# mandt-lab/shallow-ntc

Measured on AMD Instinct MI355X. Metric: decode Mpixels/s + (bpp, PSNR) on Kodak, two_layer_syn, higher is better.
Workload: dtype f32

## Files before the change

include/sntc.h:

```cpp
#ifndef SNTC_H_
#define SNTC_H_

#include <stddef.h>
#include <stdint.h>

#ifdef __cplusplus
extern "C" {
#endif

#define SNTC_VERSION 100

enum {
  SNTC_OK = 0,
  SNTC_ERR_BAD_SHAPE = 1,
  SNTC_ERR_UNSUPPORTED = 2,
  SNTC_ERR_HIP = 3,
  SNTC_ERR_NONFINITE = 4,
  SNTC_ERR_NO_DEVICE = 5
};

const char* sntc_last_error(void);
int sntc_version(void);
int sntc_device_count(void);
int sntc_device_arch(int device, char* buf, size_t buflen);

enum {
  SNTC_CONV2D = 0,
  SNTC_CONV2D_TRANSPOSE = 1,
  SNTC_SIGNAL_DOWN = 2,
  SNTC_SIGNAL_UP = 3
};
enum {
  SNTC_ACT_NONE = 0, SNTC_ACT_RELU = 1, SNTC_ACT_LEAKY_RELU = 2 , SNTC_ACT_SIGMOID = 3
};
enum {
  SNTC_PRO_NONE = 0, SNTC_PRO_ABS = 1, SNTC_PRO_SQUARE = 2
};
enum {
  SNTC_EPI_STORE = 0,
  SNTC_EPI_ADD = 1,
  SNTC_EPI_GATE = 2,
  SNTC_EPI_RES_DIV = 3,
  SNTC_EPI_RES_MUL = 4,
  SNTC_EPI_RES_DIV_SQRT = 5,
  SNTC_EPI_RES_MUL_SQRT = 6,
  SNTC_EPI_MASK_RELU = 7,
  SNTC_EPI_MASK_LEAKY = 8
};

typedef struct sntc_conv_desc {
  int32_t kind;
  int32_t kh, kw;
  int32_t stride;
  int32_t cin, cout;
  int32_t act;
  int32_t prologue;
  int32_t epilogue;
  int32_t reserved[7];
} sntc_conv_desc;

typedef struct sntc_conv_plan sntc_conv_plan;

int sntc_conv_plan_create(const sntc_conv_desc* desc, const float* weight, const float* bias,
                          void* stream, sntc_conv_plan** plan);
void sntc_conv_plan_destroy(sntc_conv_plan* plan);
int sntc_conv_plan_update(sntc_conv_plan* plan, const float* weight, const float* bias, void* stream);
typedef struct sntc_plan_group sntc_plan_group;
int sntc_plan_group_create(sntc_conv_plan* const* plans, const float* const* weights, const float* const* biases, int count,
                           void* stream, sntc_plan_group** group);
int sntc_plan_group_update(const sntc_plan_group* group, void* stream);
void sntc_plan_group_destroy(sntc_plan_group* group);
int sntc_conv_out_shape(const sntc_conv_plan* plan, int h, int w, int* ho, int* wo);
int64_t sntc_conv_flops(const sntc_conv_plan* plan, int n, int h, int w);
int sntc_conv_forward(const sntc_conv_plan* plan, const float* x, int n, int h, int w, float* y,
                      const float* res, const float* aux, void* workspace, size_t workspace_bytes, void* stream);
int64_t sntc_conv_workspace_bytes(const sntc_conv_plan* plan, int n, int h, int w);
int sntc_conv_fusable(const sntc_conv_plan* first, const sntc_conv_plan* second);
int64_t sntc_conv_fused_workspace_bytes(const sntc_conv_plan* first, int n, int h, int w);
int sntc_conv_forward_fused(const sntc_conv_plan* first, const sntc_conv_plan* second, const float* x, int n, int h, int w, float* y,
                            const float* res, const float* aux, void* workspace, size_t workspace_bytes, void* stream);
typedef struct sntc_resblock_plan sntc_resblock_plan;
int sntc_resblock_supported(int c);
int sntc_resblock_plan_create(int c, const float* w0, const float* b0, const float* w1, const float* b1,
                              const float* w2, const float* b2, int precision, void* stream, sntc_resblock_plan** plan);
int sntc_resblock_plan_update(sntc_resblock_plan* plan, const float* w0, const float* b0, const float* w1, const float* b1,
                              const float* w2, const float* b2, void* stream);
void sntc_resblock_plan_destroy(sntc_resblock_plan* plan);
int64_t sntc_resblock_flops(const sntc_resblock_plan* plan, int n, int h, int w);
int sntc_resblock_forward(const sntc_resblock_plan* plan, const float* x, int n, int h, int w, float* y, void* stream);
int sntc_resblock_plan_set_workgroups(sntc_resblock_plan* plan, int max_workgroups);
typedef struct sntc_rgbconv_plan sntc_rgbconv_plan;
int sntc_rgbconv_supported(int kind, int k, int stride, int cin, int cout, int act);
int sntc_rgbconv_plan_create(int kind, int k, int stride, int cin, int cout, const float* w, const float* bias, int act,
                             void* stream, sntc_rgbconv_plan** plan);
int sntc_rgbconv_plan_update(sntc_rgbconv_plan* plan, const float* w, const float* bias, void* stream);
void sntc_rgbconv_plan_destroy(sntc_rgbconv_plan* plan);
int64_t sntc_rgbconv_flops(const sntc_rgbconv_plan* plan, int n, int h, int w);
int sntc_rgbconv_forward(const sntc_rgbconv_plan* plan, const float* x, int n, int h, int w, float* y, void* stream);
int sntc_rgbconv_plan_set_workgroups(sntc_rgbconv_plan* plan, int max_workgroups);
typedef struct sntc_upsmall_plan sntc_upsmall_plan;
int sntc_upsmall_supported(int kind, int k, int stride, int cin, int cout);
int sntc_upsmall_plan_create(int kind, int k, int stride, int cin, int cout, const float* w, const float* bias, void* stream,
                             sntc_upsmall_plan** plan);
int sntc_upsmall_plan_update(sntc_upsmall_plan* plan, const float* w, const float* bias, void* stream);
void sntc_upsmall_plan_destroy(sntc_upsmall_plan* plan);
int64_t sntc_upsmall_flops(const sntc_upsmall_plan* plan, int n, int h, int w);
int sntc_upsmall_forward(const sntc_upsmall_plan* plan, const float* x, int n, int h, int w, float* y, void* stream);
typedef struct sntc_syn_plan sntc_syn_plan;
typedef struct sntc_syn_batch {
  const float* y_hat;
  float* hidden;
  int32_t n, h, w;
  int32_t reserved;
} sntc_syn_batch;
int sntc_syn_supported(int k, int stride, int cin, int ch, int has_res);
int sntc_syn_plan_create(int k, int stride, int cin, int ch, int has_res, int act_kind, const float* w1, const float* b1,
                         const float* beta, const float* gamma, void* stream, sntc_syn_plan** plan);
int sntc_syn_plan_update(sntc_syn_plan* plan, const float* w1, const float* b1, const float* beta, const float* gamma, void* stream);
void sntc_syn_plan_destroy(sntc_syn_plan* plan);
int64_t sntc_syn_flops(const sntc_syn_plan* plan, int64_t latent_pixels);
int64_t sntc_syn_workspace_bytes(const sntc_syn_plan* plan);
int sntc_syn_forward(const sntc_syn_plan* plan, const sntc_syn_batch* batches, int nbatches, void* workspace, size_t workspace_bytes,
                     void* stream);
int sntc_syn_plan_set_workgroups(sntc_syn_plan* plan, int max_workgroups);
int sntc_syn_plan_units(const sntc_syn_plan* plan, int* out, int capacity);
int sntc_syn_describe(int k, int stride, int cin, int ch, int has_res, int* out, int capacity);
int sntc_syn_selfcheck(int k, int stride, int cin, int ch, int has_res, int h, int w, unsigned seed, double* max_err);
int sntc_conv_plan_set_tile(sntc_conv_plan* plan, int variant);
int sntc_conv_plan_set_schedule(sntc_conv_plan* plan, int flags);
int sntc_split3(const float* x, int64_t npix, int c, void* out, void* stream);
int sntc_dequant_split3(const int32_t* symbols, const float* hyper, int64_t npix, int c, void* out, float* y_hat,
                        void* stream);
int sntc_conv_status(int* flags, void* stream);
int sntc_conv_status_inject(int flags, void* stream);
int sntc_conv_set_stream_k(int enabled);
int sntc_conv_get_stream_k(void);
int sntc_conv_launch_info(const sntc_conv_plan* plan, int n, int h, int w, int* variant, int* nblocks);
int sntc_conv_launch_order(const sntc_conv_plan* plan, int n, int h, int w, int* column_major);
int64_t sntc_conv_tune_workspace_bytes(const sntc_conv_plan* plan, int n, int h, int w);
int sntc_conv_plan_tune(sntc_conv_plan* plan, const float* x, int n, int h, int w, float* y, const float* res,
                        const float* aux, void* workspace, size_t workspace_bytes, int reps, int* variant, int* stream_k,
                        void* stream);
int sntc_conv_plan_candidates(const sntc_conv_plan* plan, int n, int h, int w, int* variants, int* stream_k, int capacity);
int sntc_conv_plan_set_choice(sntc_conv_plan* plan, int n, int h, int w, int variant, int stream_k);
int sntc_conv_plan_clear_tuning(sntc_conv_plan* plan);
int sntc_conv_plan_drop_choice(sntc_conv_plan* plan, int n, int h, int w, int ncols);

int sntc_conv_columns_supported(const sntc_conv_plan* plan, int ncols);
int sntc_conv_forward_columns(const sntc_conv_plan* plan, const float* x, int n, int h, int w, float* y, const float* res,
                              const float* aux, void* workspace, size_t workspace_bytes, void* stream, int ncols);
int64_t sntc_conv_columns_flops(const sntc_conv_plan* plan, int n, int h, int w, int ncols);
int64_t sntc_conv_columns_workspace_bytes(const sntc_conv_plan* plan, int n, int h, int w, int ncols);
int sntc_conv_columns_launch_info(const sntc_conv_plan* plan, int n, int h, int w, int ncols, int* variant, int* nblocks,
                                  int* column_major);
int64_t sntc_conv_columns_tune_workspace_bytes(const sntc_conv_plan* plan, int n, int h, int w, int ncols);
int sntc_conv_columns_tune(sntc_conv_plan* plan, const float* x, int n, int h, int w, int ncols, float* y, void* workspace,
                           size_t workspace_bytes, int reps, int* variant, int* stream_k, void* stream);
int sntc_conv_columns_candidates(const sntc_conv_plan* plan, int n, int h, int w, int ncols, int* variants, int* stream_k,
                                 int capacity);
int sntc_conv_columns_set_choice(sntc_conv_plan* plan, int n, int h, int w, int ncols, int variant, int stream_k);

int sntc_gdn_small(const float* x, int64_t npix, int c, const float* beta, const float* gamma,
                   int inverse, int alpha, int epsilon_is_half, float* y, void* stream);

int sntc_two_layer_tail(const float* t, int n, int hh, int wh, int ch, int has_res, int act_kind,
                        const float* beta, const float* gamma, const float* w2, const float* b2,
                        int k2, int s2, int cout, float* x_hat, void* stream);
int sntc_two_layer_tail_pixels(const float* t, int n, int hh, int wh, int ch, int has_res, int act_kind,
                               const float* beta, const float* gamma, const float* w2, const float* b2, int k2, int s2,
                               int cout, int h, int w, const float* ref, uint8_t* pixels, uint64_t* sse, void* stream);

int sntc_pad_reflect(const float* x, int n, int h, int w, int c, int hp, int wp, float* y, void* stream);
int sntc_pad_zero(const float* x, int n, int h, int w, int c, int top, int left, int hp, int wp, float* y, void* stream);
int sntc_crop(const float* x, int n, int hp, int wp, int c, int h, int w, float* y, void* stream);
int sntc_depth_to_space(const float* x, int n, int h, int w, int c, int block, float* y, void* stream);
int sntc_concat_channels(const float* a, int ca, const float* b, int cb, int64_t npix, float* y, void* stream);
int sntc_pixels_sse(const float* x, const float* x_hat, int n, int h, int w, int c, int hs, int ws,
                    uint8_t* pixels_out, unsigned long long* sse_out, void* stream);
int sntc_block_sse(const float* x, const uint8_t* pixels, int n, int h, int w, int c, int block, uint32_t* out, void* stream);
int sntc_float_sse(const float* x, const float* x_hat, int n, int h, int w, int c, int hs, int ws,
                   double* sse_out, void* stream);

typedef struct sntc_prior sntc_prior;
int sntc_prior_create(int channels, int nlayers, const int* widths, const float* matrices,
                      const float* biases, const float* factors, void* stream, sntc_prior** prior);
void sntc_prior_destroy(sntc_prior* prior);

int sntc_entropy_factorized(const sntc_prior* prior, const float* z, int n, int64_t hw, float* z_hat,
                            double* bits, int values_only, void* stream);

int sntc_entropy_scale_normal(const float* y, const float* hyper, int n, int64_t hw, int c,
                              float* y_hat, int32_t* symbols, double* bits, int values_only,
                              void* stream);
int sntc_dequant_scale_normal(const int32_t* symbols, const float* hyper, int n, int64_t hw, int c,
                              float* y_hat, void* stream);
int sntc_dequant_mean(const int32_t* symbols, const float* mu, int n, int64_t hw, int c, int mu_stride, float* y_hat,
                      void* stream);

int64_t sntc_rans_cap_words(int64_t elems_per_image, int segments);
int sntc_rans_encode(const int32_t* values, const uint16_t* table_ids, int nimages, int64_t elems_per_image, int segments,
                     int lanes, const uint16_t* cdf, const uint32_t* meta, int ntables, int total_entries, int64_t cap_words,
                     uint16_t* scratch, int32_t* len_words, void* stream);
int sntc_rans_compact(const uint16_t* scratch, int64_t cap_words, const int32_t* len_words, const int64_t* offsets,
                      int nstreams, uint16_t* payload, void* stream);
int64_t sntc_rans_lut_budget(int ntables, int total_entries);
int sntc_rans_decode(const uint16_t* payload, const int64_t* offsets, const uint16_t* table_ids, int nimages,
                     int64_t elems_per_image, int segments, int lanes, const uint16_t* cdf, const uint32_t* meta, int ntables,
                     int total_entries, const uint32_t* dec, const uint16_t* lut, const uint32_t* lut_meta, int lut_entries,
                     int32_t* values, int32_t* bad_streams, void* stream);
int sntc_rans_encode_channels(const float* y, int nimages, int64_t elems_per_image, int channels, int segments, int lanes,
                              const uint16_t* cdf, const uint32_t* meta, int total_entries, int64_t cap_words, uint16_t* scratch,
                              int32_t* len_words, float* y_hat, void* stream);
int sntc_rans_decode_channels(const uint16_t* payload, const int64_t* offsets, int nimages, int64_t elems_per_image, int channels,
                              int segments, int lanes, const uint16_t* cdf, const uint32_t* meta, int total_entries,
                              const uint32_t* dec, const uint16_t* lut, const uint32_t* lut_meta, int lut_entries, float* y_hat,
                              int32_t* bad_streams, void* stream);
int sntc_rans_cost(const int32_t* values, const uint16_t* table_ids, int nimages, int64_t elems_per_image, const uint32_t* meta,
                   int ntables, int total_entries, const uint32_t* cost_q, uint64_t* cost, void* stream);
int sntc_scale_table_ids(const float* hyper, int64_t npix, int c, uint16_t* table_ids, void* stream);
int sntc_channel_table_ids(int64_t npix, int c, uint16_t* table_ids, void* stream);
int sntc_round_to_int(const float* x, int64_t total, int32_t* out, void* stream);
int sntc_int_to_float(const int32_t* x, int64_t total, float* out, void* stream);

int sntc_step_symbols(const float* y, const float* mu, int n, int64_t hw, int c, int mu_stride, const uint16_t* base_ids,
                      const float* inv_step, const int32_t* shift, int32_t* symbols, uint16_t* table_ids, void* stream);
int sntc_step_table_ids(const uint16_t* base_ids, int n, int64_t elems_per_image, const int32_t* shift, uint16_t* table_ids,
                        void* stream);
int sntc_dequant_step(const int32_t* symbols, const float* mu, int n, int64_t hw, int c, int mu_stride, const float* step,
                      float* y_hat, void* stream);
int sntc_step_ladder_cost(const float* y, const float* mu, int n, int64_t hw, int c, int mu_stride, const uint16_t* base_ids,
                          const float* inv_step, const int32_t* shift, int nsteps, const uint32_t* meta, int ntables,
                          int total_entries, const uint32_t* cost_q, uint64_t* cost, void* stream);

int sntc_step_map_symbols(const float* y, const float* mu, int n, int64_t hw, int c, int mu_stride, const uint16_t* base_ids,
                          const int8_t* kmap, const float* lut, int32_t* symbols, uint16_t* table_ids, void* stream);
int sntc_step_map_table_ids(const uint16_t* base_ids, int n, int64_t hw, int c, const int8_t* kmap, uint16_t* table_ids,
                            void* stream);
int sntc_dequant_step_map(const int32_t* symbols, const float* mu, int n, int64_t hw, int c, int mu_stride, const int8_t* kmap,
                          const float* lut, float* y_hat, void* stream);
int sntc_step_map_ladder_cost(const float* y, const float* mu, int n, int64_t hw, int c, int mu_stride, const uint16_t* base_ids,
                              const int8_t* offsets, const float* lut, const int32_t* base, int nsteps, const uint32_t* meta,
                              int ntables, int total_entries, const uint32_t* cost_q, uint64_t* cost, void* stream);

int sntc_step_ladder_dequant(const float* y, const float* mu, int n, int64_t hw, int c, int mu_stride, const float* inv_step,
                             const float* step, int nsteps, float* y_hat, void* stream);
int sntc_step_map_ladder_dequant(const float* y, const float* mu, int n, int64_t hw, int c, int mu_stride, const int8_t* offsets,
                                 const float* lut, const int32_t* base, int nsteps, float* y_hat, void* stream);

int sntc_ssim_scale(const float* a, const float* b, int n, int h, int w, int c, float max_val, double* ssim_sum,
                    double* cs_sum, void* stream);
int sntc_avgpool2_symmetric(const float* x, int n, int h, int w, int c, float* y, void* stream);
int sntc_pixels_float(const float* x_hat, int n, int h, int w, int c, int hs, int ws, float* out, void* stream);

int sntc_msssim_inputs(const float* x, const float* x_hat, int n, int h, int w, int c, int hs, int ws, float* a, float* b,
                       double* sse, void* stream);
int sntc_msssim_finish(const double* sums, const double* counts, const double* weights, int scales, int n, int c, double weight,
                       double* q, float* coef, void* stream);
int sntc_ssim_scale_grad(const float* a, const float* b, int n, int h, int w, int c, float max_val, const float* coef, int use_lum,
                         const float* g_coarse, int hs, int ws, float out_scale, float* g, void* stream);
int sntc_avgpool2_symmetric_grad(const float* g_coarse, int n, int h, int w, int c, float* g_fine, void* stream);

int sntc_sga_factorized_fwd(const sntc_prior* prior, const float* z_loc, int n, int64_t hw, float tau,
                            const float* noise, uint64_t seed, uint64_t step, float* z_tilde, float* sprime,
                            float* dbits_dz, double* bits, void* stream);
int sntc_sga_normal_fwd(const float* y_loc, const float* hyper, int n, int64_t hw, int c, float tau,
                        const float* noise, uint64_t seed, uint64_t step, float* y_tilde, float* sprime,
                        float* dbits_dv, float* dbits_draw, double* bits, void* stream);
int sntc_sga_normal_bwd(const float* g_ytilde, const float* sprime, const float* dbits_dv, const float* dbits_draw,
                        float weight, int64_t npix, int c, float* g_yloc, float* g_hyper, void* stream);
int sntc_sga_normal_step_fwd(const float* y_loc, const float* hyper, int n, int64_t hw, int c, float tau, const float* noise,
                             uint64_t seed, uint64_t step, const float* quant_step, const float* inv_step, const int32_t* shift,
                             float* y_tilde, float* sprime, float* dbits_dv, float* dbits_draw, double* bits, void* stream);
int sntc_sga_normal_step_bwd(const float* g_ytilde, const float* sprime, const float* dbits_dv, const float* dbits_draw,
                             float weight, int n, int64_t hw, int c, const float* quant_step, const float* inv_step,
                             const float* dweight, float* g_yloc, float* g_hyper, void* stream);
int sntc_sga_normal_step_map_fwd(const float* y_loc, const float* hyper, int n, int64_t hw, int c, float tau, const float* noise,
                                 uint64_t seed, uint64_t step, const int8_t* kmap, const float* lut, float* y_tilde, float* sprime,
                                 float* dbits_dv, float* dbits_draw, double* bits, void* stream);
int sntc_sga_normal_step_map_bwd(const float* g_ytilde, const float* sprime, const float* dbits_dv, const float* dbits_draw,
                                 float weight, int n, int64_t hw, int c, const int8_t* kmap, const float* lut, float* g_yloc,
                                 float* g_hyper, void* stream);
int sntc_uq_sample(const float* loc, const float* offset, int64_t npix, int c, int offset_stride, int mode, float param,
                   const float* noise, uint64_t seed, uint64_t step, float* out, void* stream);
int sntc_sga_chain(const float* g, const float* dbits, const float* sprime, float weight, int64_t total, float* out,
                   void* stream);
int sntc_distortion_grad(const float* x, const float* x_hat, int n, int h, int w, int c, int hs, int ws, float scale,
                         float* g_xhat, double* sse, void* stream);
int sntc_distortion_grad_weighted(const float* x, const float* x_hat, int n, int h, int w, int c, int hs, int ws, float scale,
                                  const float* weights, int hb, int wb, int block, float* g_xhat, double* sse, double* wsse,
                                  void* stream);
int sntc_two_layer_out_adjoint(const float* g_xhat, int n, int hh, int wh, int ch, const float* w2, int k2, int s2, int cout,
                               float* g_h, void* stream);
int sntc_two_layer_tail_bwd(const float* t, const float* g_h, int64_t npix, int ch, int has_res, int act_kind,
                            const float* beta, const float* gamma, int cp, float* g_t, float* abs_x, float* g_x,
                            void* stream);
int sntc_adam_step(float* param, const float* grad, float* m, float* v, int64_t n, float lr, float beta1, float beta2,
                   float eps, int64_t t, float grad_scale, void* stream);

int64_t sntc_conv_wgrad_workspace_bytes(int kind, int kh, int kw, int stride, int cin, int cout, int n, int h, int w);
int sntc_conv_wgrad(int kind, int kh, int kw, int stride, int cin, int cout, const float* x, const float* g_out, int n,
                    int h, int w, float* dw, int accumulate, void* workspace, int64_t workspace_bytes, void* stream);
int64_t sntc_bias_grad_workspace_bytes(int64_t npix, int c);
int sntc_bias_grad(const float* g, int64_t npix, int c, float* db, int accumulate, void* workspace, int64_t workspace_bytes,
                   void* stream);
int sntc_act_backward(const float* g, const float* y, int64_t total, int act, float* g_pre, void* stream);
int sntc_gate_forward(const float* x, const float* t, const float* s, int64_t total, float* out, void* stream);
int sntc_gate_backward(const float* g, const float* t, const float* s, int64_t total, float* g_t, float* g_spre, void* stream);
int sntc_axpy(float* a, const float* b, float alpha, int64_t total, void* stream);
int sntc_noise_add(const float* x, int64_t total, const float* noise, uint64_t seed, uint64_t step, float* out, void* stream);
int sntc_sumsq(const float* x, int64_t total, double* out, void* stream);
int sntc_two_layer_hidden(const float* t, int64_t npix, int ch, int has_res, int act_kind, const float* beta,
                          const float* gamma, float* h, void* stream);
int sntc_gdn_reparam_forward(const float* raw, int64_t total, float bound, float pedestal, float* eff, void* stream);
int sntc_gdn_reparam_backward(const float* raw, const float* g_eff, int64_t total, float bound, float* g_raw, void* stream);
int sntc_noisy_normal(const float* y_tilde, const float* hyper, int n, int64_t hw, int c, float* dbits_dv,
                      float* dbits_draw, double* bits, void* stream);
int sntc_noisy_factorized(const sntc_prior* prior, const float* z_tilde, int n, int64_t hw, float* dbits_dz,
                          float* grad_record, double* bits, void* stream);
int sntc_prior_record_floats(const sntc_prior* prior);
int sntc_prior_update(sntc_prior* prior, const float* matrices, const float* biases, const float* factors, void* stream);
int sntc_prior_param_grad(const sntc_prior* prior, const float* matrices, const float* factors, const float* grad_record,
                          float weight, float* g_matrices, float* g_biases, float* g_factors, void* stream);

int sntc_gdn_apply(const float* x, const float* norm, int64_t total, int inverse, float* y, void* stream);
int sntc_gdn_backward_prep(const float* g, const float* x, const float* norm, int64_t total, int inverse, float* q, float* abs_x,
                           void* stream);
int sntc_gdn_backward_finish(const float* g, const float* x, const float* norm, const float* t, int64_t total, int inverse,
                             float* dx, void* stream);
int sntc_small_matmul(const float* a, const float* b, int rows, int k, int64_t cols, int transpose_a, float* out, void* stream);
int sntc_transpose_last2(const float* src, int taps, int a, int b, float* dst, void* stream);

#ifdef __cplusplus
}
#endif
#endif
```

shallow-ntc_amd/_capi.py:

```python
from __future__ import annotations

import ctypes as C
import os
from pathlib import Path

_PKG = Path(__file__).resolve().parent
LIB_PATH = Path(os.environ.get("SNTC_LIB", _PKG / "lib" / "libsntc_hip.so"))

OK, ERR_BAD_SHAPE, ERR_UNSUPPORTED, ERR_HIP, ERR_NONFINITE, ERR_NO_DEVICE = range(6)

CONV2D, CONV2D_TRANSPOSE, SIGNAL_DOWN, SIGNAL_UP = range(4)
ACT_NONE, ACT_RELU, ACT_LEAKY_RELU, ACT_SIGMOID = range(4)
PRO_NONE, PRO_ABS, PRO_SQUARE = range(3)
EPI_STORE, EPI_ADD, EPI_GATE, EPI_RES_DIV, EPI_RES_MUL, EPI_RES_DIV_SQRT, EPI_RES_MUL_SQRT, EPI_MASK_RELU, EPI_MASK_LEAKY = range(9)


class SntcError(RuntimeError):
    def __init__(self, code, msg):
        super().__init__(f"sntc error {code}: {msg}")
        self.code = code


class NonFiniteError(SntcError, ValueError):
    """Mirrors tf.debugging.check_numerics' InvalidArgumentError (reference mshyper/models.py:308-309,356)."""


class ConvDesc(C.Structure):
    _fields_ = [("kind", C.c_int32), ("kh", C.c_int32), ("kw", C.c_int32), ("stride", C.c_int32),
                ("cin", C.c_int32), ("cout", C.c_int32), ("act", C.c_int32), ("prologue", C.c_int32),
                ("epilogue", C.c_int32), ("reserved", C.c_int32 * 7)]


class SynBatch(C.Structure):
    _fields_ = [("y_hat", C.c_void_p), ("hidden", C.c_void_p), ("n", C.c_int32), ("h", C.c_int32), ("w", C.c_int32),
                ("reserved", C.c_int32)]


_P = C.c_void_p
SIGNATURES = {
    "sntc_last_error": (C.c_char_p, []),
    "sntc_version": (C.c_int, []),
    "sntc_device_count": (C.c_int, []),
    "sntc_device_arch": (C.c_int, [C.c_int, C.c_char_p, C.c_size_t]),
    "sntc_conv_plan_create": (C.c_int, [C.POINTER(ConvDesc), _P, _P, _P, C.POINTER(_P)]),
    "sntc_conv_plan_destroy": (None, [_P]),
    "sntc_conv_plan_update": (C.c_int, [_P, _P, _P, _P]),
    "sntc_plan_group_create": (C.c_int, [_P, _P, _P, C.c_int, _P, _P]),
    "sntc_plan_group_update": (C.c_int, [_P, _P]),
    "sntc_plan_group_destroy": (None, [_P]),
    "sntc_conv_out_shape": (C.c_int, [_P, C.c_int, C.c_int, C.POINTER(C.c_int), C.POINTER(C.c_int)]),
    "sntc_conv_flops": (C.c_int64, [_P, C.c_int, C.c_int, C.c_int]),
    "sntc_conv_forward": (C.c_int, [_P, _P, C.c_int, C.c_int, C.c_int, _P, _P, _P, _P, C.c_size_t, _P]),
    "sntc_conv_workspace_bytes": (C.c_int64, [_P, C.c_int, C.c_int, C.c_int]),
    "sntc_conv_fusable": (C.c_int, [_P, _P]),
    "sntc_conv_fused_workspace_bytes": (C.c_int64, [_P, C.c_int, C.c_int, C.c_int]),
    "sntc_conv_forward_fused": (C.c_int, [_P, _P, _P, C.c_int, C.c_int, C.c_int, _P, _P, _P, _P, C.c_size_t, _P]),
    "sntc_resblock_supported": (C.c_int, [C.c_int]),
    "sntc_resblock_plan_create": (C.c_int, [C.c_int, _P, _P, _P, _P, _P, _P, C.c_int, _P, C.POINTER(_P)]),
    "sntc_resblock_plan_update": (C.c_int, [_P, _P, _P, _P, _P, _P, _P, _P]),
    "sntc_resblock_plan_destroy": (None, [_P]),
    "sntc_resblock_flops": (C.c_int64, [_P, C.c_int, C.c_int, C.c_int]),
    "sntc_resblock_forward": (C.c_int, [_P, _P, C.c_int, C.c_int, C.c_int, _P, _P]),
    "sntc_resblock_plan_set_workgroups": (C.c_int, [_P, C.c_int]),
    "sntc_upsmall_supported": (C.c_int, [C.c_int, C.c_int, C.c_int, C.c_int, C.c_int]),
    "sntc_upsmall_plan_create": (C.c_int, [C.c_int, C.c_int, C.c_int, C.c_int, C.c_int, _P, _P, _P, C.POINTER(_P)]),
    "sntc_upsmall_plan_update": (C.c_int, [_P, _P, _P, _P]),
    "sntc_upsmall_plan_destroy": (None, [_P]),
    "sntc_upsmall_flops": (C.c_int64, [_P, C.c_int, C.c_int, C.c_int]),
    "sntc_upsmall_forward": (C.c_int, [_P, _P, C.c_int, C.c_int, C.c_int, _P, _P]),
    "sntc_rgbconv_supported": (C.c_int, [C.c_int, C.c_int, C.c_int, C.c_int, C.c_int, C.c_int]),
    "sntc_rgbconv_plan_create": (C.c_int, [C.c_int, C.c_int, C.c_int, C.c_int, C.c_int, _P, _P, C.c_int, _P, C.POINTER(_P)]),
    "sntc_rgbconv_plan_update": (C.c_int, [_P, _P, _P, _P]),
    "sntc_rgbconv_plan_destroy": (None, [_P]),
    "sntc_rgbconv_flops": (C.c_int64, [_P, C.c_int, C.c_int, C.c_int]),
    "sntc_rgbconv_forward": (C.c_int, [_P, _P, C.c_int, C.c_int, C.c_int, _P, _P]),
    "sntc_rgbconv_plan_set_workgroups": (C.c_int, [_P, C.c_int]),
    "sntc_syn_supported": (C.c_int, [C.c_int, C.c_int, C.c_int, C.c_int, C.c_int]),
    "sntc_syn_plan_create": (C.c_int, [C.c_int, C.c_int, C.c_int, C.c_int, C.c_int, C.c_int, _P, _P, _P, _P, _P, C.POINTER(_P)]),
    "sntc_syn_plan_update": (C.c_int, [_P, _P, _P, _P, _P, _P]),
    "sntc_syn_plan_destroy": (None, [_P]),
    "sntc_syn_flops": (C.c_int64, [_P, C.c_int64]),
    "sntc_syn_workspace_bytes": (C.c_int64, [_P]),
    "sntc_syn_forward": (C.c_int, [_P, _P, C.c_int, _P, C.c_size_t, _P]),
    "sntc_syn_plan_set_workgroups": (C.c_int, [_P, C.c_int]),
    "sntc_syn_plan_units": (C.c_int, [_P, C.POINTER(C.c_int), C.c_int]),
    "sntc_syn_describe": (C.c_int, [C.c_int, C.c_int, C.c_int, C.c_int, C.c_int, C.POINTER(C.c_int), C.c_int]),
    "sntc_syn_selfcheck": (C.c_int, [C.c_int, C.c_int, C.c_int, C.c_int, C.c_int, C.c_int, C.c_int, C.c_uint, C.POINTER(C.c_double)]),
    "sntc_conv_plan_set_tile": (C.c_int, [C.c_void_p, C.c_int]),
    "sntc_conv_plan_set_schedule": (C.c_int, [C.c_void_p, C.c_int]),
    "sntc_split3": (C.c_int, [_P, C.c_int64, C.c_int, _P, _P]),
    "sntc_dequant_split3": (C.c_int, [_P, _P, C.c_int64, C.c_int, _P, _P, _P]),
    "sntc_conv_status": (C.c_int, [C.POINTER(C.c_int), _P]),
    "sntc_conv_status_inject": (C.c_int, [C.c_int, _P]),
    "sntc_conv_set_stream_k": (C.c_int, [C.c_int]),
    "sntc_conv_get_stream_k": (C.c_int, []),
    "sntc_conv_launch_info": (C.c_int, [_P, C.c_int, C.c_int, C.c_int, C.POINTER(C.c_int), C.POINTER(C.c_int)]),
    "sntc_conv_launch_order": (C.c_int, [_P, C.c_int, C.c_int, C.c_int, C.POINTER(C.c_int)]),
    "sntc_conv_tune_workspace_bytes": (C.c_int64, [_P, C.c_int, C.c_int, C.c_int]),
    "sntc_conv_plan_tune": (C.c_int, [_P, _P, C.c_int, C.c_int, C.c_int, _P, _P, _P, _P, C.c_size_t, C.c_int, C.POINTER(C.c_int),
                                      C.POINTER(C.c_int), _P]),
    "sntc_conv_plan_clear_tuning": (C.c_int, [_P]),
    "sntc_conv_plan_candidates": (C.c_int, [_P, C.c_int, C.c_int, C.c_int, C.POINTER(C.c_int), C.POINTER(C.c_int), C.c_int]),
    "sntc_conv_plan_set_choice": (C.c_int, [_P, C.c_int, C.c_int, C.c_int, C.c_int, C.c_int]),
    "sntc_conv_plan_drop_choice": (C.c_int, [_P, C.c_int, C.c_int, C.c_int, C.c_int]),
    "sntc_conv_columns_supported": (C.c_int, [_P, C.c_int]),
    "sntc_conv_forward_columns": (C.c_int, [_P, _P, C.c_int, C.c_int, C.c_int, _P, _P, _P, _P, C.c_size_t, _P, C.c_int]),
    "sntc_conv_columns_flops": (C.c_int64, [_P, C.c_int, C.c_int, C.c_int, C.c_int]),
    "sntc_conv_columns_workspace_bytes": (C.c_int64, [_P, C.c_int, C.c_int, C.c_int, C.c_int]),
    "sntc_conv_columns_launch_info": (C.c_int, [_P, C.c_int, C.c_int, C.c_int, C.c_int, C.POINTER(C.c_int), C.POINTER(C.c_int),
                                                C.POINTER(C.c_int)]),
    "sntc_conv_columns_tune_workspace_bytes": (C.c_int64, [_P, C.c_int, C.c_int, C.c_int, C.c_int]),
    "sntc_conv_columns_tune": (C.c_int, [_P, _P, C.c_int, C.c_int, C.c_int, C.c_int, _P, _P, C.c_size_t, C.c_int, C.POINTER(C.c_int),
                                         C.POINTER(C.c_int), _P]),
    "sntc_conv_columns_candidates": (C.c_int, [_P, C.c_int, C.c_int, C.c_int, C.c_int, C.POINTER(C.c_int), C.POINTER(C.c_int), C.c_int]),
    "sntc_conv_columns_set_choice": (C.c_int, [_P, C.c_int, C.c_int, C.c_int, C.c_int, C.c_int, C.c_int]),
    "sntc_gdn_small": (C.c_int, [_P, C.c_int64, C.c_int, _P, _P, C.c_int, C.c_int, C.c_int, _P, _P]),
    "sntc_two_layer_tail": (C.c_int, [_P, C.c_int, C.c_int, C.c_int, C.c_int, C.c_int, C.c_int, _P, _P, _P, _P,
                                      C.c_int, C.c_int, C.c_int, _P, _P]),
    "sntc_two_layer_tail_pixels": (C.c_int, [_P, C.c_int, C.c_int, C.c_int, C.c_int, C.c_int, C.c_int, _P, _P, _P, _P,
                                             C.c_int, C.c_int, C.c_int, C.c_int, C.c_int, _P, _P, _P, _P]),
    "sntc_pad_reflect": (C.c_int, [_P, C.c_int, C.c_int, C.c_int, C.c_int, C.c_int, C.c_int, _P, _P]),
    "sntc_pad_zero": (C.c_int, [_P, C.c_int, C.c_int, C.c_int, C.c_int, C.c_int, C.c_int, C.c_int, C.c_int, _P, _P]),
    "sntc_crop": (C.c_int, [_P, C.c_int, C.c_int, C.c_int, C.c_int, C.c_int, C.c_int, _P, _P]),
    "sntc_depth_to_space": (C.c_int, [_P, C.c_int, C.c_int, C.c_int, C.c_int, C.c_int, _P, _P]),
    "sntc_concat_channels": (C.c_int, [_P, C.c_int, _P, C.c_int, C.c_int64, _P, _P]),
    "sntc_pixels_sse": (C.c_int, [_P, _P, C.c_int, C.c_int, C.c_int, C.c_int, C.c_int, C.c_int, _P, _P, _P]),
    "sntc_float_sse": (C.c_int, [_P, _P, C.c_int, C.c_int, C.c_int, C.c_int, C.c_int, C.c_int, _P, _P]),
    "sntc_prior_create": (C.c_int, [C.c_int, C.c_int, C.POINTER(C.c_int), C.POINTER(C.c_float),
                                    C.POINTER(C.c_float), C.POINTER(C.c_float), _P, C.POINTER(_P)]),
    "sntc_prior_destroy": (None, [_P]),
    "sntc_entropy_factorized": (C.c_int, [_P, _P, C.c_int, C.c_int64, _P, _P, C.c_int, _P]),
    "sntc_entropy_scale_normal": (C.c_int, [_P, _P, C.c_int, C.c_int64, C.c_int, _P, _P, _P, C.c_int, _P]),
    "sntc_dequant_scale_normal": (C.c_int, [_P, _P, C.c_int, C.c_int64, C.c_int, _P, _P]),
    "sntc_dequant_mean": (C.c_int, [_P, _P, C.c_int, C.c_int64, C.c_int, C.c_int, _P, _P]),
    "sntc_rans_cap_words": (C.c_int64, [C.c_int64, C.c_int]),
    "sntc_rans_encode": (C.c_int, [_P, _P, C.c_int, C.c_int64, C.c_int, C.c_int, _P, _P, C.c_int, C.c_int, C.c_int64, _P, _P, _P]),
    "sntc_rans_compact": (C.c_int, [_P, C.c_int64, _P, _P, C.c_int, _P, _P]),
    "sntc_rans_lut_budget": (C.c_int64, [C.c_int, C.c_int]),
    "sntc_rans_decode": (C.c_int, [_P, _P, _P, C.c_int, C.c_int64, C.c_int, C.c_int, _P, _P, C.c_int, C.c_int, _P, _P, _P, C.c_int, _P, _P, _P]),
    "sntc_rans_encode_channels": (C.c_int, [_P, C.c_int, C.c_int64, C.c_int, C.c_int, C.c_int, _P, _P, C.c_int, C.c_int64, _P, _P, _P, _P]),
    "sntc_rans_decode_channels": (C.c_int, [_P, _P, C.c_int, C.c_int64, C.c_int, C.c_int, C.c_int, _P, _P, C.c_int, _P, _P, _P, C.c_int, _P, _P, _P]),
    "sntc_rans_cost": (C.c_int, [_P, _P, C.c_int, C.c_int64, _P, C.c_int, C.c_int, _P, _P, _P]),
    "sntc_scale_table_ids": (C.c_int, [_P, C.c_int64, C.c_int, _P, _P]),
    "sntc_channel_table_ids": (C.c_int, [C.c_int64, C.c_int, _P, _P]),
    "sntc_round_to_int": (C.c_int, [_P, C.c_int64, _P, _P]),
    "sntc_int_to_float": (C.c_int, [_P, C.c_int64, _P, _P]),
    "sntc_step_symbols": (C.c_int, [_P, _P, C.c_int, C.c_int64, C.c_int, C.c_int, _P, _P, _P, _P, _P, _P]),
    "sntc_step_table_ids": (C.c_int, [_P, C.c_int, C.c_int64, _P, _P, _P]),
    "sntc_dequant_step": (C.c_int, [_P, _P, C.c_int, C.c_int64, C.c_int, C.c_int, _P, _P, _P]),
    "sntc_step_ladder_cost": (C.c_int, [_P, _P, C.c_int, C.c_int64, C.c_int, C.c_int, _P, _P, _P, C.c_int, _P, C.c_int, C.c_int,
                                        _P, _P, _P]),
    "sntc_step_map_symbols": (C.c_int, [_P, _P, C.c_int, C.c_int64, C.c_int, C.c_int, _P, _P, _P, _P, _P, _P]),
    "sntc_step_map_table_ids": (C.c_int, [_P, C.c_int, C.c_int64, C.c_int, _P, _P, _P]),
    "sntc_dequant_step_map": (C.c_int, [_P, _P, C.c_int, C.c_int64, C.c_int, C.c_int, _P, _P, _P, _P]),
    "sntc_step_map_ladder_cost": (C.c_int, [_P, _P, C.c_int, C.c_int64, C.c_int, C.c_int, _P, _P, _P, _P, C.c_int, _P, C.c_int,
                                            C.c_int, _P, _P, _P]),
    "sntc_step_ladder_dequant": (C.c_int, [_P, _P, C.c_int, C.c_int64, C.c_int, C.c_int, _P, _P, C.c_int, _P, _P]),
    "sntc_step_map_ladder_dequant": (C.c_int, [_P, _P, C.c_int, C.c_int64, C.c_int, C.c_int, _P, _P, _P, C.c_int, _P, _P]),
    "sntc_ssim_scale": (C.c_int, [_P, _P, C.c_int, C.c_int, C.c_int, C.c_int, C.c_float, _P, _P, _P]),
    "sntc_avgpool2_symmetric": (C.c_int, [_P, C.c_int, C.c_int, C.c_int, C.c_int, _P, _P]),
    "sntc_pixels_float": (C.c_int, [_P, C.c_int, C.c_int, C.c_int, C.c_int, C.c_int, C.c_int, _P, _P]),
    "sntc_msssim_inputs": (C.c_int, [_P, _P, C.c_int, C.c_int, C.c_int, C.c_int, C.c_int, C.c_int, _P, _P, _P, _P]),
    "sntc_msssim_finish": (C.c_int, [_P, C.POINTER(C.c_double), C.POINTER(C.c_double), C.c_int, C.c_int, C.c_int, C.c_double,
                                     _P, _P, _P]),
    "sntc_ssim_scale_grad": (C.c_int, [_P, _P, C.c_int, C.c_int, C.c_int, C.c_int, C.c_float, _P, C.c_int, _P, C.c_int, C.c_int,
                                       C.c_float, _P, _P]),
    "sntc_avgpool2_symmetric_grad": (C.c_int, [_P, C.c_int, C.c_int, C.c_int, C.c_int, _P, _P]),
    "sntc_sga_factorized_fwd": (C.c_int, [_P, _P, C.c_int, C.c_int64, C.c_float, _P, C.c_uint64, C.c_uint64, _P, _P, _P, _P, _P]),
    "sntc_sga_normal_fwd": (C.c_int, [_P, _P, C.c_int, C.c_int64, C.c_int, C.c_float, _P, C.c_uint64, C.c_uint64, _P, _P, _P,
                                      _P, _P, _P]),
    "sntc_sga_normal_bwd": (C.c_int, [_P, _P, _P, _P, C.c_float, C.c_int64, C.c_int, _P, _P, _P]),
    "sntc_sga_normal_step_fwd": (C.c_int, [_P, _P, C.c_int, C.c_int64, C.c_int, C.c_float, _P, C.c_uint64, C.c_uint64, _P, _P, _P,
                                           _P, _P, _P, _P, _P, _P]),
    "sntc_sga_normal_step_bwd": (C.c_int, [_P, _P, _P, _P, C.c_float, C.c_int, C.c_int64, C.c_int, _P, _P, _P, _P, _P, _P]),
    "sntc_uq_sample": (C.c_int, [_P, _P, C.c_int64, C.c_int, C.c_int, C.c_int, C.c_float, _P, C.c_uint64, C.c_uint64, _P, _P]),
    "sntc_sga_chain": (C.c_int, [_P, _P, _P, C.c_float, C.c_int64, _P, _P]),
    "sntc_sga_normal_step_map_fwd": (C.c_int, [_P, _P, C.c_int, C.c_int64, C.c_int, C.c_float, _P, C.c_uint64, C.c_uint64, _P, _P, _P,
                                               _P, _P, _P, _P, _P]),
    "sntc_sga_normal_step_map_bwd": (C.c_int, [_P, _P, _P, _P, C.c_float, C.c_int, C.c_int64, C.c_int, _P, _P, _P, _P, _P]),
    "sntc_distortion_grad_weighted": (C.c_int, [_P, _P, C.c_int, C.c_int, C.c_int, C.c_int, C.c_int, C.c_int, C.c_float, _P, C.c_int,
                                                C.c_int, C.c_int, _P, _P, _P, _P]),
    "sntc_block_sse": (C.c_int, [_P, _P, C.c_int, C.c_int, C.c_int, C.c_int, C.c_int, _P, _P]),
    "sntc_distortion_grad": (C.c_int, [_P, _P, C.c_int, C.c_int, C.c_int, C.c_int, C.c_int, C.c_int, C.c_float, _P, _P, _P]),
    "sntc_two_layer_tail_bwd": (C.c_int, [_P, _P, C.c_int64, C.c_int, C.c_int, C.c_int, _P, _P, C.c_int, _P, _P, _P, _P]),
    "sntc_two_layer_out_adjoint": (C.c_int, [_P, C.c_int, C.c_int, C.c_int, C.c_int, _P, C.c_int, C.c_int, C.c_int, _P, _P]),
    "sntc_adam_step": (C.c_int, [_P, _P, _P, _P, C.c_int64, C.c_float, C.c_float, C.c_float, C.c_float, C.c_int64, C.c_float, _P]),
    "sntc_conv_wgrad_workspace_bytes": (C.c_int64, [C.c_int] * 9),
    "sntc_conv_wgrad": (C.c_int, [C.c_int] * 6 + [_P, _P, C.c_int, C.c_int, C.c_int, _P, C.c_int, _P, C.c_int64, _P]),
    "sntc_bias_grad_workspace_bytes": (C.c_int64, [C.c_int64, C.c_int]),
    "sntc_bias_grad": (C.c_int, [_P, C.c_int64, C.c_int, _P, C.c_int, _P, C.c_int64, _P]),
    "sntc_act_backward": (C.c_int, [_P, _P, C.c_int64, C.c_int, _P, _P]),
    "sntc_gate_forward": (C.c_int, [_P, _P, _P, C.c_int64, _P, _P]),
    "sntc_gate_backward": (C.c_int, [_P, _P, _P, C.c_int64, _P, _P, _P]),
    "sntc_axpy": (C.c_int, [_P, _P, C.c_float, C.c_int64, _P]),
    "sntc_noise_add": (C.c_int, [_P, C.c_int64, _P, C.c_uint64, C.c_uint64, _P, _P]),
    "sntc_sumsq": (C.c_int, [_P, C.c_int64, _P, _P]),
    "sntc_two_layer_hidden": (C.c_int, [_P, C.c_int64, C.c_int, C.c_int, C.c_int, _P, _P, _P, _P]),
    "sntc_gdn_reparam_forward": (C.c_int, [_P, C.c_int64, C.c_float, C.c_float, _P, _P]),
    "sntc_gdn_reparam_backward": (C.c_int, [_P, _P, C.c_int64, C.c_float, _P, _P]),
    "sntc_noisy_normal": (C.c_int, [_P, _P, C.c_int, C.c_int64, C.c_int, _P, _P, _P, _P]),
    "sntc_noisy_factorized": (C.c_int, [_P, _P, C.c_int, C.c_int64, _P, _P, _P, _P]),
    "sntc_gdn_apply": (C.c_int, [_P, _P, C.c_int64, C.c_int, _P, _P]),
    "sntc_gdn_backward_prep": (C.c_int, [_P, _P, _P, C.c_int64, C.c_int, _P, _P, _P]),
    "sntc_gdn_backward_finish": (C.c_int, [_P, _P, _P, _P, C.c_int64, C.c_int, _P, _P]),
    "sntc_small_matmul": (C.c_int, [_P, _P, C.c_int, C.c_int, C.c_int64, C.c_int, _P, _P]),
    "sntc_transpose_last2": (C.c_int, [_P, C.c_int, C.c_int, C.c_int, _P, _P]),
    "sntc_prior_record_floats": (C.c_int, [_P]),
    "sntc_prior_update": (C.c_int, [_P, _P, _P, _P, _P]),
    "sntc_prior_param_grad": (C.c_int, [_P, _P, _P, _P, C.c_float, _P, _P, _P, _P]),
}

_lib = None


def load():
    global _lib
    if _lib is not None:
        return _lib
    if not LIB_PATH.exists():
        raise ImportError(
            f"{LIB_PATH} is missing: build it with `python -c 'import __graft_entry__ as g; g.build()'` "
            f"or `make -C shallow-ntc_amd/csrc`.  There is no CPU fallback for the hot path.")
    import torch
    lib = C.CDLL(str(LIB_PATH))
    for name, (res, args) in SIGNATURES.items():
        fn = getattr(lib, name)
        fn.restype = res
        fn.argtypes = args
    _lib = lib
    if os.environ.get("SNTC_STATIC_SCHEDULES", "") not in ("", "0"):
        lib.sntc_conv_set_stream_k(0)
    return lib


def last_error() -> str:
    return load().sntc_last_error().decode("utf-8", "replace")


def check(rc: int):
    if rc != OK:
        msg = last_error()
        raise (NonFiniteError if rc == ERR_NONFINITE else SntcError)(rc, msg)


def call(name, *args):
    check(getattr(load(), name)(*args))


def device_count() -> int:
    return load().sntc_device_count()


def require_gpu():
    if device_count() < 1:
        raise SntcError(ERR_NO_DEVICE, "no HIP device visible: the shallow-ntc hot path only runs on MI355X (gfx950)")


def device_arch(device=0) -> str:
    buf = C.create_string_buffer(256)
    check(load().sntc_device_arch(device, buf, 256))
    return buf.value.decode()
```

shallow-ntc_amd/csrc/conv_plan.hip:

```cpp
#include <algorithm>
#include <cstdio>
#include <cstdlib>
#include <array>
#include <atomic>
#include <map>
#include <mutex>
#include <cstdlib>
#include <vector>
#include "sntc_internal.h"

namespace sntc {

struct PackDesc {
  const float* w;
  float* wp;
  const int* taps;
  const unsigned* cols;
  int T, Cin, Cout, K, Ncol, kw, s, pt, pl, phase_mode, slab_major, out_major, bf3, rowpack;
};

__device__ __forceinline__ void pack_element(const PackDesc& d, size_t idx) {
  const int col = (int)(idx / d.K);
  const int k = (int)(idx - (size_t)col * d.K);
  float v = 0.0f;
// ... 174 lines not shown
  const int k = d.kh, s = d.stride;
  struct HostGrp { std::vector<int> taps; std::vector<unsigned> cols; int q0y = 0, q0x = 0; bool uniform = true; };
  std::vector<HostGrp> groups;
  auto enc = [](int oyo, int oxo, int ch) { return ((unsigned)(oyo + 128) << 24) | ((unsigned)(oxo + 128) << 16) | (unsigned)ch; };

  if (!p->phase_mode) {
    HostGrp hg;
    for (int ky = 0; ky < d.kh; ++ky)
      for (int kx = 0; kx < (p->rowpack ? 1 : d.kw); ++kx) hg.taps.push_back((ky << 16) | kx);
    for (int ch = 0; ch < d.cout; ++ch) hg.cols.push_back(enc(0, 0, ch));
    groups.push_back(std::move(hg));
  } else {
    auto classes = [&](int kk, std::vector<std::pair<int, std::vector<int>>>& out) {
      for (int phi = 0; phi < s; ++phi) {
        const int cnt = (kk - phi + s - 1) / s;
        if (cnt <= 0) return false;
        bool found = false;
        for (auto& c : out)
          if (c.first == cnt) { c.second.push_back(phi); found = true; }
        if (!found) out.push_back({cnt, {phi}});
      }
      std::sort(out.begin(), out.end(), [](const auto& a, const auto& b) { return a.first > b.first; });
      return true;
    };
    std::vector<std::pair<int, std::vector<int>>> cy, cx;
    if (!classes(d.kh, cy) || !classes(d.kw, cx))
      return fail(SNTC_ERR_UNSUPPORTED, "transposed convolution with kernel < stride is not supported");
    for (auto& a : cy)
      for (auto& b : cx) {
        HostGrp hg;
        for (int jy = 0; jy < a.first; ++jy)
          for (int jx = 0; jx < b.first; ++jx) hg.taps.push_back((jy << 16) | jx);
        for (int py : a.second)
          for (int px : b.second)
            for (int ch = 0; ch < d.cout; ++ch) hg.cols.push_back(enc(py - p->pt, px - p->pl, ch));
        auto q0 = [&](int phi, int pad) { return phi < pad ? 1 : 0; };
        hg.q0y = q0(a.second[0], p->pt);
        hg.q0x = q0(b.second[0], p->pl);
        for (int py : a.second) hg.uniform &= q0(py, p->pt) == hg.q0y;
        for (int px : b.second) hg.uniform &= q0(px, p->pl) == hg.q0x;
        groups.push_back(std::move(hg));
      }
    std::stable_sort(groups.begin(), groups.end(),
                     [](const HostGrp& a, const HostGrp& b) { return a.taps.size() > b.taps.size(); });
  }
  if ((int)groups.size() > kMaxGroups) return fail(SNTC_ERR_UNSUPPORTED, "too many phase groups");
  p->ngroups = (int)groups.size();
  p->exact_grid = p->phase_mode && p->pt < s && p->pl < s;
  for (auto& hg : groups) p->exact_grid = p->exact_grid && hg.uniform;
  for (int gi = 0; gi < p->ngroups; ++gi) {
    auto& hg = groups[gi];
    auto& G = p->g[gi];
    if (p->exact_grid) { G.q0y = hg.q0y; G.q0x = hg.q0x; }
    G.T = (int)hg.taps.size();
    G.Ncol = (int)hg.cols.size();
    G.tw = 1;
    for (int t = 0; t < G.T; ++t) G.tw = std::max(G.tw, (hg.taps[t] & 0xffff) + 1);
    for (int t = 0; t < G.T; ++t)
      if (hg.taps[t] != (((t / G.tw) << 16) | (t % G.tw))) return fail(SNTC_ERR_UNSUPPORTED, "tap table is not a dense row-major grid");
    G.K = p->rowpack ? G.T * kStage : ((G.T * d.cin + kStage - 1) / kStage) * kStage;
    if ((int64_t)G.Ncol * G.K * 4 >= (1LL << 31)) return fail(SNTC_ERR_UNSUPPORTED, "packed weights of one phase group must be < 2 GiB");
    SNTC_HIP(hipMalloc(&G.taps, sizeof(int) * std::max(1, G.T)));
    SNTC_HIP(hipMalloc(&G.cols, sizeof(unsigned) * G.Ncol));
    SNTC_HIP(hipMalloc(&G.wp, (p->bf3 ? 6 : sizeof(float)) * (size_t)G.Ncol * std::max(kStage, G.K)));
    SNTC_HIP(hipMemcpyAsync(G.taps, hg.taps.data(), sizeof(int) * G.T, hipMemcpyHostToDevice, stream));
    SNTC_HIP(hipMemcpyAsync(G.cols, hg.cols.data(), sizeof(unsigned) * G.Ncol, hipMemcpyHostToDevice, stream));
    SNTC_HIP(hipStreamSynchronize(stream));
    const size_t total = (size_t)G.Ncol * G.K;
    const int blocks = (int)std::min<size_t>((total + 255) / 256, 4096);
    if (total > 0)
      hipLaunchKernelGGL(pack_weights_kernel, dim3(blocks), dim3(256), 0, stream, weight, G.wp, G.taps, G.cols,
                         G.T, d.cin, d.cout, G.K, G.Ncol, d.kind, d.kw, s, p->pt, p->pl, p->phase_mode ? 1 : 0, p->vec ? 1 : 0, p->out_major ? 1 : 0, p->bf3 ? 1 : 0, p->rowpack ? 1 : 0);
    SNTC_HIP(hipGetLastError());
  }
  if (bias) {
    SNTC_HIP(hipMalloc(&p->bias, sizeof(float) * d.cout));
    SNTC_HIP(hipMemcpyAsync(p->bias, bias, sizeof(float) * d.cout, hipMemcpyDeviceToDevice, stream));
  }
  (void)k;
  return pack_fused_second(p, stream);
}

extern "C" int sntc_conv_plan_create(const sntc_conv_desc* desc, const float* weight, const float* bias,
                                     void* stream, sntc_conv_plan** plan) {
  if (!desc || !weight || !plan) return fail(SNTC_ERR_BAD_SHAPE, "sntc_conv_plan_create: null argument");
  const sntc_conv_desc& d = *desc;
  if (d.kind < SNTC_CONV2D || d.kind > SNTC_SIGNAL_UP) return fail(SNTC_ERR_UNSUPPORTED, "unknown conv kind");
  if (d.kh < 1 || d.kw < 1 || d.kh > 64 || d.kw > 64 || d.stride < 1 || d.stride > 64 || d.cin < 1 || d.cout < 1 ||
      d.cout > 65535)
    return fail(SNTC_ERR_BAD_SHAPE, "sntc_conv_plan_create: bad kernel / stride / channel sizes");
  if (d.act < SNTC_ACT_NONE || d.act > SNTC_ACT_SIGMOID || d.prologue < 0 || d.prologue > SNTC_PRO_SQUARE ||
      d.epilogue < 0 || d.epilogue > SNTC_EPI_MASK_LEAKY)
    return fail(SNTC_ERR_UNSUPPORTED, "unknown activation / prologue / epilogue");
  int rc = gg_init();
  if (rc) return rc;
  auto* p = new sntc_conv_plan();
  p->d = d;
  SNTC_HIP(hipGetDevice(&p->device));
  p->up = (d.kind == SNTC_CONV2D_TRANSPOSE || d.kind == SNTC_SIGNAL_UP);
  p->phase_mode = p->up && d.stride > 1;
  if (d.kind == SNTC_CONV2D_TRANSPOSE) {
    p->pt = std::max(d.kh - d.stride, 0) / 2;
    p->pl = std::max(d.kw - d.stride, 0) / 2;
  } else if (d.kind == SNTC_SIGNAL_UP) {
    p->pt = (d.kh - 1) / 2;
    p->pl = (d.kw - 1) / 2;
  } else if (d.kind == SNTC_SIGNAL_DOWN) {
    p->pt = d.kh / 2;
    p->pl = d.kw / 2;
  }
  p->rowpack = d.reserved[2] == 1;
  if (p->rowpack && (d.kind != SNTC_CONV2D || d.kw * d.cin > kStage || d.prologue != SNTC_PRO_NONE || d.reserved[1] != 0)) {
    delete p;
    return fail(SNTC_ERR_UNSUPPORTED, "row-packed plans: Keras Conv2D with kw * Cin <= 16 (the RGB first layer), fp32, no prologue");
  }
  p->vec = p->rowpack || (d.cin % kStage) == 0;
  p->out_major = (d.kind == SNTC_CONV2D_TRANSPOSE) != (d.reserved[0] != 0);
  p->bf3 = d.reserved[1] != 0;
  p->s3 = d.reserved[1] == 2;
  if (p->bf3 && (!p->vec || d.prologue != SNTC_PRO_NONE)) {
    delete p;
    return fail(SNTC_ERR_UNSUPPORTED, "bf16 x 3 plans need Cin % 16 == 0 and no prologue");
  }
  if (p->s3 && ((d.cout & 3) || (d.epilogue != SNTC_EPI_STORE && d.epilogue != SNTC_EPI_ADD && d.epilogue != SNTC_EPI_GATE &&
                                d.epilogue != SNTC_EPI_MASK_RELU && d.epilogue != SNTC_EPI_MASK_LEAKY))) {
    delete p;
    return fail(SNTC_ERR_UNSUPPORTED, "pre-split bf16 x 3 plans need Cout % 4 == 0 and a store / add / gate / mask epilogue");
  }
  rc = build_plan(p, weight, bias, (hipStream_t)stream);
  if (rc) {
    sntc_conv_plan_destroy(p);
    return rc;
  }
  *plan = p;
  return SNTC_OK;
}

extern "C" int sntc_conv_plan_update(sntc_conv_plan* p, const float* weight, const float* bias, void* stream) {
  if (!p || !weight) return fail(SNTC_ERR_BAD_SHAPE, "sntc_conv_plan_update: null argument");
  if ((bias != nullptr) != (p->bias != nullptr)) return fail(SNTC_ERR_BAD_SHAPE, "sntc_conv_plan_update: bias presence differs from the plan");
  hipStream_t s = (hipStream_t)stream;
  const sntc_conv_desc& d = p->d;
  for (int gi = 0; gi < p->ngroups; ++gi) {
    auto& G = p->g[gi];
    const size_t total = (size_t)G.Ncol * G.K;
    const int blocks = (int)std::min<size_t>((total + 255) / 256, 4096);
    if (total > 0)
      hipLaunchKernelGGL(pack_weights_kernel, dim3(blocks), dim3(256), 0, s, weight, G.wp, G.taps, G.cols, G.T, d.cin, d.cout, G.K,
                         G.Ncol, d.kind, d.kw, d.stride, p->pt, p->pl, p->phase_mode ? 1 : 0, p->vec ? 1 : 0, p->out_major ? 1 : 0, p->bf3 ? 1 : 0, p->rowpack ? 1 : 0);
    SNTC_HIP(hipGetLastError());
  }
  if (bias) SNTC_HIP(hipMemcpyAsync(p->bias, bias, sizeof(float) * d.cout, hipMemcpyDeviceToDevice, s));
  return pack_fused_second(p, s);
}

struct sntc_plan_group {
  PackJob* jobs = nullptr;
  int* blk_job = nullptr;
  long long* blk_first = nullptr;
  int nblocks = 0;
  int nblocks2 = 0;
};

extern "C" void sntc_plan_group_destroy(sntc_plan_group* g) {
  if (!g) return;
  if (g->jobs) (void)hipFree(g->jobs);
  if (g->blk_job) (void)hipFree(g->blk_job);
  if (g->blk_first) (void)hipFree(g->blk_first);
  delete g;
}

extern "C" int sntc_plan_group_create(sntc_conv_plan* const* plans, const float* const* weights, const float* const* biases,
                                      int count, void* stream, sntc_plan_group** out) {
  if (!plans || !weights || !biases || !out || count < 1) return fail(SNTC_ERR_BAD_SHAPE, "sntc_plan_group_create: null argument");
  std::vector<PackJob> jobs, jobs2;
  for (int i = 0; i < count; ++i) {
    sntc_conv_plan* p = plans[i];
    if (!p || !weights[i]) return fail(SNTC_ERR_BAD_SHAPE, "sntc_plan_group_create: null plan or weight array");
    if ((biases[i] != nullptr) != (p->bias != nullptr))
      return fail(SNTC_ERR_BAD_SHAPE, "sntc_plan_group_create: bias presence differs from the plan");
    const sntc_conv_desc& d = p->d;
    for (int gi = 0; gi < p->ngroups; ++gi) {
      auto& G = p->g[gi];
      PackJob j{};
      j.d = PackDesc{weights[i], G.wp, G.taps, G.cols, G.T, d.cin, d.cout, G.K, G.Ncol, d.kw, d.stride, p->pt, p->pl,
                     p->phase_mode ? 1 : 0, p->vec ? 1 : 0, p->out_major ? 1 : 0, p->bf3 ? 1 : 0, p->rowpack ? 1 : 0};
      j.kind = 0;
      if ((size_t)G.Ncol * G.K > 0) jobs.push_back(j);
    }
    if (biases[i]) {
      PackJob j{};
      j.d.w = biases[i]; j.d.wp = p->bias; j.d.Ncol = d.cout;
      j.kind = 1;
      jobs.push_back(j);
    }
    if (fusable_second(p) && p->w2f) {
      PackJob j{};
      j.d.w = p->g[0].wp; j.d.wp = p->w2f; j.d.K = p->g[0].K; j.d.Ncol = p->g[0].Ncol;
      j.kind = 2;
      jobs2.push_back(j);
    }
  }
  std::vector<int> blk_job;
  std::vector<long long> blk_first;
  auto add_blocks = [&](const std::vector<PackJob>& js, int base) {
    for (size_t j = 0; j < js.size(); ++j) {
      const size_t total = js[j].kind == 0 ? (size_t)js[j].d.Ncol * js[j].d.K : js[j].kind == 1 ? (size_t)js[j].d.Ncol : (size_t)(2 * 3 * 12 * 64 * 4);
      for (size_t f = 0; f < total; f += kPackChunk) { blk_job.push_back(base + (int)j); blk_first.push_back((long long)f); }
    }
  };
  add_blocks(jobs, 0);
  const int nb1 = (int)blk_job.size();
  add_blocks(jobs2, (int)jobs.size());
  const int nb2 = (int)blk_job.size() - nb1;
  jobs.insert(jobs.end(), jobs2.begin(), jobs2.end());
  auto* g = new sntc_plan_group();
  g->nblocks = nb1;
  g->nblocks2 = nb2;
  hipStream_t s = (hipStream_t)stream;
  hipError_t e = hipMalloc(&g->jobs, sizeof(PackJob) * jobs.size());
  if (e == hipSuccess) e = hipMalloc(&g->blk_job, sizeof(int) * blk_job.size());
  if (e == hipSuccess) e = hipMalloc(&g->blk_first, sizeof(long long) * blk_first.size());
  if (e == hipSuccess) e = hipMemcpyAsync(g->jobs, jobs.data(), sizeof(PackJob) * jobs.size(), hipMemcpyHostToDevice, s);
  if (e == hipSuccess) e = hipMemcpyAsync(g->blk_job, blk_job.data(), sizeof(int) * blk_job.size(), hipMemcpyHostToDevice, s);
  if (e == hipSuccess) e = hipMemcpyAsync(g->blk_first, blk_first.data(), sizeof(long long) * blk_first.size(), hipMemcpyHostToDevice, s);
  if (e == hipSuccess) e = hipStreamSynchronize(s);
  if (e != hipSuccess) { sntc_plan_group_destroy(g); return hip_fail(e, "sntc_plan_group_create"); }
  *out = g;
  return SNTC_OK;
}

extern "C" int sntc_plan_group_update(const sntc_plan_group* g, void* stream) {
  if (!g) return fail(SNTC_ERR_BAD_SHAPE, "sntc_plan_group_update: null group");
  hipStream_t s = (hipStream_t)stream;
  if (g->nblocks > 0) hipLaunchKernelGGL(pack_group_kernel, dim3(g->nblocks), dim3(256), 0, s, g->jobs, g->blk_job, g->blk_first);
  if (g->nblocks2 > 0)
    hipLaunchKernelGGL(pack_group_kernel, dim3(g->nblocks2), dim3(256), 0, s, g->jobs, g->blk_job + g->nblocks, g->blk_first + g->nblocks);
  SNTC_HIP(hipGetLastError());
  return SNTC_OK;
}

struct Geo {
  int Ho, Wo, Qh, Qw, sA, tstep, offy, offx, sO;
};

static int geometry(const sntc_conv_plan* p, int h, int w, Geo* g) {
  const sntc_conv_desc& d = p->d;
  const int s = d.stride;
  if (h < 1 || w < 1) return fail(SNTC_ERR_BAD_SHAPE, "empty image");
  if (p->rowpack) {
    if (h < d.kh || w < d.kw) return fail(SNTC_ERR_BAD_SHAPE, "row-packed plan: padded input smaller than the kernel");
    const int ho = (h - d.kh) / s + 1, wo = (w - d.kw) / s + 1;
    *g = Geo{ho, wo, ho, wo, s, 1, 0, 0, 1};
    return SNTC_OK;
  }
  if (!p->up) {
    g->Ho = (h + s - 1) / s;
    g->Wo = (w + s - 1) / s;
    int pt, pl;
    if (d.kind == SNTC_CONV2D) {
      pt = std::max((g->Ho - 1) * s + d.kh - h, 0) / 2;
      pl = std::max((g->Wo - 1) * s + d.kw - w, 0) / 2;
    } else {
      pt = p->pt;
      pl = p->pl;
    }
    *g = Geo{g->Ho, g->Wo, g->Ho, g->Wo, s, 1, -pt, -pl, 1};
  } else if (!p->phase_mode) {
    *g = Geo{h, w, h, w, 1, -1, p->pt, p->pl, 1};
  } else {
    const int ho = h * s, wo = w * s;
    if (p->exact_grid)
      *g = Geo{ho, wo, h, w, 1, -1, 0, 0, s};
    else
      *g = Geo{ho, wo, (ho - 1 + p->pt) / s + 1, (wo - 1 + p->pl) / s + 1, 1, -1, 0, 0, s};
  }
  return SNTC_OK;
}

extern "C" int sntc_conv_out_shape(const sntc_conv_plan* p, int h, int w, int* ho, int* wo) {
  if (!p || !ho || !wo) return fail(SNTC_ERR_BAD_SHAPE, "sntc_conv_out_shape: null argument");
  Geo g;
  int rc = geometry(p, h, w, &g);
  if (rc) return rc;
  *ho = g.Ho;
  *wo = g.Wo;
  return SNTC_OK;
}

static int64_t conv_flops(const sntc_conv_plan* p, int n, int h, int w, int ncols) {
  if (!p) return 0;
  Geo g;
  if (geometry(p, h, w, &g)) return 0;
  const sntc_conv_desc& d = p->d;
  const int64_t px = p->up ? (int64_t)h * w : (int64_t)g.Ho * g.Wo;
  return 2 * (int64_t)n * px * d.kh * d.kw * d.cin * (ncols > 0 ? ncols : d.cout);
}

extern "C" int64_t sntc_conv_flops(const sntc_conv_plan* p, int n, int h, int w) { return conv_flops(p, n, h, w, 0); }

struct Sched {
  const GGInstance* inst = nullptr;
  int ksplit = 1;
  bool sk = false;
  int workers = 0;
  int64_t units = 0;
  int64_t blocks = 0;
};

static int max_steps(const sntc_conv_plan* p) {
  int s = 0;
  for (int gi = 0; gi < p->ngroups; ++gi) s = std::max(s, p->g[gi].K / kStage);
  return s;
}

static int pick_ksplit(const sntc_conv_plan* p, const Geo& g) {
  int steps_min = 1 << 30, steps_max = 0;
  int64_t bpi = 0;
  const int64_t mt = ((int64_t)g.Qh * g.Qw + 127) / 128;
  for (int gi = 0; gi < p->ngroups; ++gi) {
    const int steps = p->g[gi].K / 32;
    steps_min = std::min(steps_min, steps);
    steps_max = std::max(steps_max, steps);
    bpi += mt * ((p->g[gi].Ncol + 63) / 64);
  }
#ifndef SNTC_KSPLIT_BPI_MAX
#define SNTC_KSPLIT_BPI_MAX 32
#endif
  if (steps_max < 64 || bpi > SNTC_KSPLIT_BPI_MAX) return 1;
  const int want = (int)((128 + bpi - 1) / bpi);
  return std::max(1, std::min({8, want, std::max(1, steps_min / 8)}));
}

static const char* columns_error(const sntc_conv_plan* p, int ncols) {
  if (!p) return "null plan";
  if (p->ngroups != 1 || p->phase_mode) return "column-limited launches: single-group plans whose columns are the output channels";
  if (p->bf3 || p->s3 || p->rowpack) return "column-limited launches: plain fp32 plans only (not bf16 x 3, not row-packed)";
  if (p->d.epilogue != SNTC_EPI_STORE) return "column-limited launches: plain store epilogue only";
  if (ncols <= 0 || ncols > p->d.cout || (ncols & 3)) return "column-limited launches: 0 < ncols <= cout and ncols % 4 == 0";
  return nullptr;
}

static inline int launch_cols(const sntc_conv_plan* p, int gi, int ncols) { return ncols > 0 ? ncols : p->g[gi].Ncol; }

struct Work {
  int ntm = 0;
  int ntn[kMaxGroups] = {};
  int tile0[kMaxGroups] = {};
  long long unit0[kMaxGroups] = {};
  int tps = 0;
  long long ups = 0;
  int64_t tiles = 0, units = 0;
  double padded_macs = 0;
};

static Work work_of(const sntc_conv_plan* p, const GGInstance& inst, int64_t M, int ncols) {
  Work wk;
  const int bm = inst.bm, bn = inst.bn;
  wk.ntm = (int)((M + bm - 1) / bm);
  for (int gi = 0; gi < p->ngroups; ++gi) {
    const int steps = p->g[gi].K / kStage;
    wk.ntn[gi] = (launch_cols(p, gi, ncols) + bn - 1) / bn;
    wk.tile0[gi] = wk.tps;
    wk.unit0[gi] = wk.ups;
    wk.tps += wk.ntn[gi];
    wk.ups += (long long)wk.ntn[gi] * steps;
    wk.padded_macs += (double)p->g[gi].K * (double)((int64_t)wk.ntn[gi] * bn) * (double)((int64_t)wk.ntm * bm);
  }
  wk.tiles = (int64_t)wk.tps * wk.ntm;
  wk.units = (int64_t)wk.ups * wk.ntm;
  return wk;
}

constexpr int kDeepBlocksPerCU = 2;
constexpr double kDeepCost = 0.6;

static std::atomic<int> g_stream_k_enabled{1};

static Sched schedule_s3(const sntc_conv_plan* p, const Geo& g, int64_t n, const TuneChoice* force) {
  Sched best;
  const int64_t M = n * g.Qh * g.Qw;
  const int msteps = max_steps(p);
  double best_cost = 1e300;
  for (int v : {11, 12, 13}) {
    if (p->tile >= 11 && v != p->tile) continue;
    if (force && v != force->variant) continue;
    const GGInstance* inst = gg_find(v, kLoadVec, kStageDma, kFormPresplit);
    if (!inst) continue;
    const int cus = std::max(8, gg_resident(*inst));
    const Work wk = work_of(p, *inst, M, 0);
    const int64_t tiles = wk.tiles, units = wk.units;
    const double macs = wk.padded_macs;
    Sched s;
    s.inst = inst;
    s.ksplit = 1;
    s.units = units;
    const int64_t fit = msteps > 0 ? units / msteps : 0;
    const int workers = (int)(std::min<int64_t>(cus, fit) & ~7LL);
    const bool can_sk = g_stream_k_enabled.load(std::memory_order_relaxed) && units < (1LL << 31) && workers >= 8 && 2 * workers >= cus;
    s.sk = force ? (force->sk != 0 && can_sk) : (can_sk && !p->no_stream_k && (units >= 64 * tiles || p->force_stream_k));
    s.workers = s.sk ? workers : 0;
    s.blocks = s.sk ? workers : tiles;
    double cost = macs;
    if (s.sk) {
      cost *= (double)cus / workers;
    } else {
      const double rounds = (double)tiles / cus;
      cost *= rounds < 1.0 ? 1.0 / rounds : std::ceil(rounds) / rounds;
    }
    cost /= (v == 11 ? 1.0 : v == 13 ? 0.97 : 0.92);
    if (cost < best_cost) { best_cost = cost; best = s; }
  }
  bool halo = best.inst && !p->no_halo && g.sA == 1;
  for (int gi = 0; halo && gi < p->ngroups; ++gi) {
    const int th = p->g[gi].T / p->g[gi].tw;
    halo = p->g[gi].T <= 32 && best.inst->bm + (th - 1) * g.Qw + p->g[gi].tw - 1 + (p->g[gi].T > 1 ? 1 : 0) <= bf3p_patch_rows_max();
  }
  if (halo) best.inst = gg_find(best.inst->variant, kLoadVec, kStageDma, kFormPresplitHalo);
  return best;
}

static const GGInstance* column_major(const sntc_conv_plan* p, const Sched& sc, int ncols) {
  const GGInstance* strip = sc.inst;
  if (!sc.sk || strip->load != kLoadVec || strip->stage != kStageRing || strip->form != kFormPlain || p->ngroups != 1 || p->colm == 0 ||
      (p->colm != 1 && (size_t)launch_cols(p, 0, ncols) * p->g[0].K * sizeof(float) <= ((size_t)4 << 20)))
    return nullptr;
  const GGInstance* twin = gg_find(strip->variant, kLoadVec, kStageRing, kFormColm);
  return twin && gg_resident(*twin) >= gg_resident(*strip) ? twin : nullptr;
}

static Sched schedule(const sntc_conv_plan* p, const Geo& g, int64_t n, bool fused = false, const TuneChoice* force = nullptr,
                      int ncols = 0) {
  if (p->s3) return schedule_s3(p, g, n, force);
  Sched best;
  const int64_t M = n * g.Qh * g.Qw;
  const int ksplit = fused ? 1 : pick_ksplit(p, g);
  const int msteps = max_steps(p);
  const bool pro = p->d.prologue != SNTC_PRO_NONE;
  const GGLoad load = !p->vec ? kLoadGather : pro ? kLoadVecPro : kLoadVec;
  const GGForm form = fused ? kFormFuse2 : p->bf3 ? kFormBf3 : kFormPlain;
  double best_cost = 1e300;
  for (int v = 1; v <= kNumVariants; ++v) {
    if (!fused && p->tile != 0 && v != p->tile) continue;
    if (p->tile == 0 && (v == 6 || v == 7 || v == 10)) continue;
    if (force && v != force->variant) continue;
    const GGInstance* ring = gg_find(v, load, kStageRing, form);
    if (!ring) continue;
    const GGInstance* dma = !fused && plan_dma(p) ? gg_find(v, load, kStageDma, kFormPlain) : nullptr;
    const Work wk = work_of(p, *ring, M, ncols);
    const int64_t tiles = wk.tiles, units = wk.units;
    const double macs = wk.padded_macs;
    Sched s;
    s.inst = dma ? dma : ring;
    const int resident = std::max(1, gg_resident(*s.inst));
    s.ksplit = ksplit;
    s.units = units;
    const int64_t fit = msteps > 0 ? units / msteps : 0;
    const int workers = (int)(std::min<int64_t>(resident, fit) & ~7LL);
    const bool short_tiles = (units < 64 * tiles || tiles * ksplit >= 4 * (int64_t)resident) && !p->force_stream_k;
    const bool can_sk = ksplit == 1 && g_stream_k_enabled.load(std::memory_order_relaxed) && units < (1LL << 31) && workers >= 8 &&
                        2 * workers >= resident;
    s.sk = force ? (force->sk != 0 && can_sk) : (can_sk && !p->no_stream_k && !short_tiles);
    s.workers = s.sk ? workers : 0;
    s.blocks = s.sk ? workers : tiles * ksplit;
    double cost = macs;
    const bool deep_ok = !fused && !s.sk && p->dma != 0 && p->vec && !p->rowpack && !pro && !p->bf3 &&
                         tiles * ksplit <= (int64_t)kDeepBlocksPerCU * gg_num_cus();
    const GGInstance* deep = deep_ok ? gg_find(v, kLoadVec, kStageDeep, kFormPlain) : nullptr;
    if (deep) s.inst = deep;
    if (s.sk) {
      cost *= (double)resident / workers;
    } else if (deep) {
      cost *= std::max(1.0, (double)gg_num_cus() / (double)(tiles * ksplit)) * kDeepCost;
    } else {
      const double rounds = (double)(tiles * ksplit) / resident;
      cost *= rounds < 1.0 ? 1.0 / rounds : std::ceil(rounds) / rounds;
      if (tiles * ksplit < 768) cost *= 1.0 + 0.5 * (double)(768 - tiles * ksplit) / 768.0;
    }
    static const double kRate[kNumVariants + 1] = {0, 0.86, 0.93, 1.00, 1.00, 0.97, 0.90, 0.85, 0.90, 1.02, 0.40};
    cost /= kRate[v];
#ifdef SNTC_DIAG
    if (getenv("SNTC_SCHED_DBG"))
      fprintf(stderr, "[sched] M=%lld v=%d sk=%d workers=%d blocks=%lld tiles=%lld units=%lld resident=%d deep=%d cost=%.4g (macs %.4g)\n", (long long)M, v,
              (int)s.sk, s.workers, (long long)s.blocks, (long long)tiles, (long long)units, resident, deep ? 1 : 0, cost, macs);
#endif
    if (cost < best_cost) { best_cost = cost; best = s; }
  }
  if (const GGInstance* twin = column_major(p, best, ncols)) best.inst = twin;
  return best;
}

static Sched plan_schedule(const sntc_conv_plan* p, const Geo& g, int n, int h, int w, bool fused = false, int ncols = 0) {
  if (!fused && p->tile == 0 && !p->no_stream_k && !p->force_stream_k) {
    TuneChoice c;
    bool have = false;
    {
      std::lock_guard<std::mutex> lk(p->tune_mu);
      auto it = p->tuned.find({n, h, w, ncols});
      if (it != p->tuned.end()) { c = it->second; have = true; }
    }
    if (have && c.sk != 0 && !g_stream_k_enabled.load(std::memory_order_relaxed)) have = false;
    if (have) {
      const Sched s = schedule(p, g, n, false, &c, ncols);
      if (s.inst) return s;
    }
  }
  return schedule(p, g, n, fused, nullptr, ncols);
}

static int64_t workspace_floats(const sntc_conv_plan* p, int64_t M, const Sched& s, int ncols = 0) {
  if (s.sk)
    return (int64_t)s.workers * (int64_t)s.inst->slab_floats + s.workers;
  if (s.ksplit <= 1) return 0;
  int64_t cols = 0;
  for (int gi = 0; gi < p->ngroups; ++gi) cols += launch_cols(p, gi, ncols);
  return (int64_t)s.ksplit * M * cols;
}

static int64_t conv_workspace_bytes(const sntc_conv_plan* p, int n, int h, int w, int ncols) {
  if (!p) return 0;
  Geo g;
  if (geometry(p, h, w, &g)) return 0;
  return 4 * workspace_floats(p, (int64_t)n * g.Qh * g.Qw, plan_schedule(p, g, n, h, w, false, ncols), ncols);
}

extern "C" int64_t sntc_conv_workspace_bytes(const sntc_conv_plan* p, int n, int h, int w) { return conv_workspace_bytes(p, n, h, w, 0); }

static int conv_launch_info(const sntc_conv_plan* p, int n, int h, int w, int ncols, int* variant, int* nblocks, int* column_major_out) {
  Geo g;
  int rc = geometry(p, h, w, &g);
  if (rc) return rc;
  const Sched s = plan_schedule(p, g, n, h, w, false, ncols);
  if (variant) *variant = s.inst ? s.inst->variant : 0;
  if (nblocks) *nblocks = (int)s.blocks;
  if (column_major_out) *column_major_out = s.inst && s.inst->form == kFormColm ? 1 : 0;
  return SNTC_OK;
}

extern "C" int sntc_conv_launch_order(const sntc_conv_plan* p, int n, int h, int w, int* column_major_out) {
  if (!p || !column_major_out) return fail(SNTC_ERR_BAD_SHAPE, "sntc_conv_launch_order: null argument");
  return conv_launch_info(p, n, h, w, 0, nullptr, nullptr, column_major_out);
}

extern "C" int sntc_conv_launch_info(const sntc_conv_plan* p, int n, int h, int w, int* variant, int* nblocks) {
  if (!p || !variant || !nblocks) return fail(SNTC_ERR_BAD_SHAPE, "sntc_conv_launch_info: null argument");
  return conv_launch_info(p, n, h, w, 0, variant, nblocks, nullptr);
}

static int conv_forward_impl(const sntc_conv_plan* p, const sntc_conv_plan* p2, const float* x, int n, int h, int w, float* y,
                             const float* res, const float* aux, void* workspace, size_t workspace_bytes, void* stream,
                             const TuneChoice* force = nullptr, int ncols = 0) {
  if (!p || !x || !y) return fail(SNTC_ERR_BAD_SHAPE, "sntc_conv_forward: null argument");
  if (ncols != 0) {
    if (const char* why = columns_error(p, ncols)) return fail(SNTC_ERR_UNSUPPORTED, why);
    if (p2) return fail(SNTC_ERR_UNSUPPORTED, "column-limited launches: not the fused pair");
  }
  if (n < 1) return fail(SNTC_ERR_BAD_SHAPE, "sntc_conv_forward: empty batch");
  const sntc_conv_desc& d = p->d;
  const int epilogue = p2 ? p2->d.epilogue : d.epilogue;
  if (epilogue != SNTC_EPI_STORE && !res) return fail(SNTC_ERR_BAD_SHAPE, "epilogue needs `res`");
  if (epilogue == SNTC_EPI_GATE && !aux) return fail(SNTC_ERR_BAD_SHAPE, "gate epilogue needs `aux`");
  Geo g;
  int rc = geometry(p, h, w, &g);
  if (rc) return rc;
  const int64_t M = (int64_t)n * g.Qh * g.Qw;
  const int64_t x_bytes = (int64_t)n * h * w * d.cin * (p->s3 ? 6 : 4);
  if (M > 0x7fffffffLL || x_bytes >= (1LL << 31))
    return fail(SNTC_ERR_BAD_SHAPE, "sntc_conv_forward: input tensor must be < 2 GiB (32-bit buffer offsets); split the batch");
  if (p2 && M * p2->d.cout >= (1LL << 32)) return fail(SNTC_ERR_BAD_SHAPE, "sntc_conv_forward_fused: output too large; split the batch");
  const Sched sc = force ? schedule(p, g, n, false, force, ncols) : plan_schedule(p, g, n, h, w, p2 != nullptr, ncols);
  if (!sc.inst) return fail(SNTC_ERR_UNSUPPORTED, "sntc_conv_forward: no compiled instance for this plan and tile variant");
  const int64_t ws_floats = workspace_floats(p, M, sc, ncols);
  if (ws_floats > 0 && (!workspace || workspace_bytes < (size_t)ws_floats * 4))
    return fail(SNTC_ERR_BAD_SHAPE, "sntc_conv_forward: this call needs sntc_conv_workspace_bytes() of workspace "
                                    "(split-K slabs / stream-K hand-off)");
  const GGInstance& inst = *sc.inst;
  const Work wk = work_of(p, inst, M, ncols);
  if (sc.sk && wk.units != sc.units) return fail(SNTC_ERR_HIP, "sntc_conv_forward: schedule and launch disagree about the work units");
  GGArgs a{};
  a.ksplit = sc.ksplit;
  a.slab = static_cast<float*>(workspace);
  a.x = x; a.y = y; a.bias = p->bias; a.res = res; a.aux = aux;
  a.x_bytes = (unsigned)x_bytes;
  a.N = n; a.H = h; a.W = w; a.Cin = d.cin;
  a.Qh = g.Qh; a.Qw = g.Qw; a.M = (int)M;
  a.Ho = g.Ho; a.Wo = g.Wo; a.Cout = ncols > 0 ? ncols : d.cout;
  a.sA = g.sA; a.tstep = g.tstep; a.offy = g.offy; a.offx = g.offx; a.sO = g.sO;
  a.act = d.act; a.epi = epilogue; a.pro = d.prologue;
  a.ntm = wk.ntm;
  a.ngroups = p->ngroups;
  if (p2) { a.w2f = p2->w2f; a.bias2 = p2->bias; a.Cout2 = p2->d.cout; }
  a.status = gg_status_word();
  if (!a.status) return fail(SNTC_ERR_HIP, "sntc_conv_forward: the device tables of the current device are not initialised");
  a.sk = sc.sk ? 1 : 0;
  a.nworkers = sc.workers;
  a.units = wk.units;
  if (sc.sk) {
    a.sk_slab = static_cast<float*>(workspace);
    a.sk_flags = reinterpret_cast<int*>(a.sk_slab + (size_t)sc.workers * inst.slab_floats);
    a.slab = nullptr;
    if (int zrc = zero_async(a.sk_flags, sizeof(int) * sc.workers, (hipStream_t)stream)) return zrc;
  }
  int nb = 0;
  size_t slab_off = 0;
  for (int gi = 0; gi < p->ngroups; ++gi) {
    GGGroup& G = a.g[gi];
    G.wp = p->g[gi].wp; G.taps = p->g[gi].taps; G.cols = reinterpret_cast<const int*>(p->g[gi].cols);
    G.T = p->g[gi].T; G.K = p->g[gi].K; G.Ncol = launch_cols(p, gi, ncols); G.tw = p->g[gi].tw;
    G.ntn = wk.ntn[gi];
    G.steps = G.K / kStage;
    G.blk0 = nb;
    G.tile0 = wk.tile0[gi];
    G.unit0 = wk.unit0[gi];
    nb += G.ntn * a.ntm * sc.ksplit;
    G.slab_off = slab_off;
    G.q0y = p->g[gi].q0y; G.q0x = p->g[gi].q0x;
    slab_off += (size_t)sc.ksplit * M * G.Ncol;
  }
  a.tps = wk.tps;
  a.ups = (int)wk.ups;
  if (p->s3) a.order = p->dma == 0 ? 0 : 1;
  rc = gg_launch(inst, a, sc.sk ? sc.workers : nb, (hipStream_t)stream);
  if (rc || sc.sk || sc.ksplit <= 1) return rc;
  return gg_reduce_launch(a, (hipStream_t)stream);
}

extern "C" int sntc_conv_forward(const sntc_conv_plan* p, const float* x, int n, int h, int w, float* y,
                                 const float* res, const float* aux, void* workspace, size_t workspace_bytes,
                                 void* stream) {
  return conv_forward_impl(p, nullptr, x, n, h, w, y, res, aux, workspace, workspace_bytes, stream);
}

static void tune_candidates(const sntc_conv_plan* p, const Geo& g, int n, std::vector<std::pair<TuneChoice, Sched>>* out, int ncols = 0) {
  for (int v = 1; v <= kMaxVariant; ++v) {
    if (!base_instance(p, v)) continue;
    for (int sk = 1; sk >= 0; --sk) {
      TuneChoice c;
      c.variant = v;
      c.sk = sk;
      const Sched s = schedule(p, g, n, false, &c, ncols);
      if (!s.inst || s.inst->variant != v || (sk && !s.sk)) continue;
      out->push_back({c, s});
    }
  }
}

static int64_t conv_tune_workspace_bytes(const sntc_conv_plan* p, int n, int h, int w, int ncols) {
  if (!p) return 0;
  Geo g;
  if (geometry(p, h, w, &g)) return 0;
  std::vector<std::pair<TuneChoice, Sched>> cand;
  tune_candidates(p, g, n, &cand, ncols);
  int64_t m = 0;
  for (auto& c : cand) m = std::max(m, workspace_floats(p, (int64_t)n * g.Qh * g.Qw, c.second, ncols));
  return 4 * m;
}

extern "C" int64_t sntc_conv_tune_workspace_bytes(const sntc_conv_plan* p, int n, int h, int w) {
  return conv_tune_workspace_bytes(p, n, h, w, 0);
}

static int conv_plan_tune(sntc_conv_plan* p, const float* x, int n, int h, int w, int ncols, float* y, const float* res,
                          const float* aux, void* workspace, size_t workspace_bytes, int reps, int* variant,
                          int* stream_k, void* stream) {
  if (!p || !x || !y) return fail(SNTC_ERR_BAD_SHAPE, "sntc_conv_plan_tune: null argument");
  if (ncols != 0)
    if (const char* why = columns_error(p, ncols)) return fail(SNTC_ERR_UNSUPPORTED, why);
  Geo g;
  int rc = geometry(p, h, w, &g);
  if (rc) return rc;
  reps = std::max(1, std::min(reps, 100));
  std::vector<std::pair<TuneChoice, Sched>> cand;
  tune_candidates(p, g, n, &cand, ncols);
  if (cand.empty()) return fail(SNTC_ERR_UNSUPPORTED, "sntc_conv_plan_tune: no candidate");
  hipEvent_t e0, e1;
  SNTC_HIP(hipEventCreate(&e0));
  SNTC_HIP(hipEventCreate(&e1));
  float best_ms = 1e30f;
  TuneChoice best;
  for (auto& c : cand) {
    if ((size_t)(4 * workspace_floats(p, (int64_t)n * g.Qh * g.Qw, c.second, ncols)) > workspace_bytes) continue;
    rc = conv_forward_impl(p, nullptr, x, n, h, w, y, res, aux, workspace, workspace_bytes, stream, &c.first, ncols);
    if (rc) break;
    (void)hipEventRecord(e0, (hipStream_t)stream);
    for (int r = 0; r < reps && !rc; ++r)
      rc = conv_forward_impl(p, nullptr, x, n, h, w, y, res, aux, workspace, workspace_bytes, stream, &c.first, ncols);
    (void)hipEventRecord(e1, (hipStream_t)stream);
    if (rc) break;
    float ms = 0.f;
    if (hipEventSynchronize(e1) != hipSuccess || hipEventElapsedTime(&ms, e0, e1) != hipSuccess) { rc = fail(SNTC_ERR_HIP, "sntc_conv_plan_tune: timing failed"); break; }
    if (ms < best_ms) { best_ms = ms; best = c.first; }
  }
  (void)hipEventDestroy(e0);
  (void)hipEventDestroy(e1);
  if (rc) return rc;
  if (best.variant == 0) return fail(SNTC_ERR_BAD_SHAPE, "sntc_conv_plan_tune: workspace smaller than sntc_conv_tune_workspace_bytes()");
  {
    std::lock_guard<std::mutex> lk(p->tune_mu);
    p->tuned[{n, h, w, ncols}] = best;
  }
  if (variant) *variant = best.variant;
  if (stream_k) *stream_k = best.sk;
  return SNTC_OK;
}

extern "C" int sntc_conv_plan_tune(sntc_conv_plan* p, const float* x, int n, int h, int w, float* y, const float* res,
                                   const float* aux, void* workspace, size_t workspace_bytes, int reps, int* variant,
                                   int* stream_k, void* stream) {
  return conv_plan_tune(p, x, n, h, w, 0, y, res, aux, workspace, workspace_bytes, reps, variant, stream_k, stream);
}

static int conv_plan_set_choice(sntc_conv_plan* p, int n, int h, int w, int ncols, int variant, int stream_k) {
  if (!p) return fail(SNTC_ERR_BAD_SHAPE, "sntc_conv_plan_set_choice: null plan");
  if (ncols != 0)
    if (const char* why = columns_error(p, ncols)) return fail(SNTC_ERR_UNSUPPORTED, why);
  Geo g;
  int rc = geometry(p, h, w, &g);
  if (rc) return rc;
  TuneChoice c;
  c.variant = variant;
  c.sk = stream_k ? 1 : 0;
  const Sched s = schedule(p, g, n, false, &c, ncols);
  if (!s.inst || s.inst->variant != variant || (stream_k && !s.sk))
    return fail(SNTC_ERR_UNSUPPORTED, "sntc_conv_plan_set_choice: not a candidate of this plan for this call shape");
  std::lock_guard<std::mutex> lk(p->tune_mu);
  p->tuned[{n, h, w, ncols}] = c;
  return SNTC_OK;
}

extern "C" int sntc_conv_plan_set_choice(sntc_conv_plan* p, int n, int h, int w, int variant, int stream_k) {
  return conv_plan_set_choice(p, n, h, w, 0, variant, stream_k);
}

static int conv_plan_candidates(const sntc_conv_plan* p, int n, int h, int w, int ncols, int* variants, int* stream_k, int capacity) {
  if (!p || !variants || !stream_k || capacity < 1) return fail(SNTC_ERR_BAD_SHAPE, "sntc_conv_plan_candidates: bad argument");
  if (ncols != 0 && columns_error(p, ncols)) { (void)fail(SNTC_ERR_UNSUPPORTED, columns_error(p, ncols)); return -1; }
  Geo g;
  if (geometry(p, h, w, &g)) return -1;
  std::vector<std::pair<TuneChoice, Sched>> cand;
  tune_candidates(p, g, n, &cand, ncols);
  int k = 0;
  for (auto& c : cand)
    if (k < capacity) { variants[k] = c.first.variant; stream_k[k] = c.first.sk; ++k; }
  return k;
}

extern "C" int sntc_conv_plan_candidates(const sntc_conv_plan* p, int n, int h, int w, int* variants, int* stream_k, int capacity) {
  return conv_plan_candidates(p, n, h, w, 0, variants, stream_k, capacity);
}

extern "C" int sntc_conv_columns_supported(const sntc_conv_plan* p, int ncols) { return columns_error(p, ncols) ? 0 : 1; }

extern "C" int sntc_conv_forward_columns(const sntc_conv_plan* p, const float* x, int n, int h, int w, float* y, const float* res,
                                         const float* aux, void* workspace, size_t workspace_bytes, void* stream, int ncols) {
  if (const char* why = columns_error(p, ncols)) return fail(SNTC_ERR_UNSUPPORTED, why);
  return conv_forward_impl(p, nullptr, x, n, h, w, y, res, aux, workspace, workspace_bytes, stream, nullptr, ncols);
}

extern "C" int64_t sntc_conv_columns_flops(const sntc_conv_plan* p, int n, int h, int w, int ncols) {
  return columns_error(p, ncols) ? 0 : conv_flops(p, n, h, w, ncols);
}

extern "C" int64_t sntc_conv_columns_workspace_bytes(const sntc_conv_plan* p, int n, int h, int w, int ncols) {
  return columns_error(p, ncols) ? 0 : conv_workspace_bytes(p, n, h, w, ncols);
}

extern "C" int sntc_conv_columns_launch_info(const sntc_conv_plan* p, int n, int h, int w, int ncols, int* variant, int* nblocks,
                                             int* column_major_out) {
  if (const char* why = columns_error(p, ncols)) return fail(SNTC_ERR_UNSUPPORTED, why);
  return conv_launch_info(p, n, h, w, ncols, variant, nblocks, column_major_out);
}

extern "C" int64_t sntc_conv_columns_tune_workspace_bytes(const sntc_conv_plan* p, int n, int h, int w, int ncols) {
  return columns_error(p, ncols) ? 0 : conv_tune_workspace_bytes(p, n, h, w, ncols);
}

extern "C" int sntc_conv_columns_tune(sntc_conv_plan* p, const float* x, int n, int h, int w, int ncols, float* y, void* workspace,
                                      size_t workspace_bytes, int reps, int* variant, int* stream_k, void* stream) {
  if (const char* why = columns_error(p, ncols)) return fail(SNTC_ERR_UNSUPPORTED, why);
  return conv_plan_tune(p, x, n, h, w, ncols, y, nullptr, nullptr, workspace, workspace_bytes, reps, variant, stream_k, stream);
}

extern "C" int sntc_conv_columns_candidates(const sntc_conv_plan* p, int n, int h, int w, int ncols, int* variants, int* stream_k,
                                            int capacity) {
  if (columns_error(p, ncols)) { (void)fail(SNTC_ERR_UNSUPPORTED, columns_error(p, ncols)); return -1; }
  return conv_plan_candidates(p, n, h, w, ncols, variants, stream_k, capacity);
}

extern "C" int sntc_conv_columns_set_choice(sntc_conv_plan* p, int n, int h, int w, int ncols, int variant, int stream_k) {
  if (const char* why = columns_error(p, ncols)) return fail(SNTC_ERR_UNSUPPORTED, why);
  return conv_plan_set_choice(p, n, h, w, ncols, variant, stream_k);
}

extern "C" int sntc_conv_plan_drop_choice(sntc_conv_plan* p, int n, int h, int w, int ncols) {
  if (!p) return fail(SNTC_ERR_BAD_SHAPE, "sntc_conv_plan_drop_choice: null plan");
  std::lock_guard<std::mutex> lk(p->tune_mu);
  p->tuned.erase({n, h, w, ncols});
  return SNTC_OK;
}

extern "C" int sntc_conv_plan_clear_tuning(sntc_conv_plan* p) {
  if (!p) return fail(SNTC_ERR_BAD_SHAPE, "sntc_conv_plan_clear_tuning: null plan");
  std::lock_guard<std::mutex> lk(p->tune_mu);
  p->tuned.clear();
  return SNTC_OK;
}

static const char* fused_pair_error(const sntc_conv_plan* p, const sntc_conv_plan* p2) {
  if (!p || !p2) return "null plan";
  const sntc_conv_desc& a = p->d;
  if (p->up || p2->up || p->bf3 || p2->bf3) return "forward convolutions in fp32 only";
  if (!p->vec || a.cout != 96 || a.stride != 1 || a.prologue != SNTC_PRO_NONE || a.epilogue != SNTC_EPI_STORE || p->ngroups != 1)
    return "first plan: stride-1 convolution with Cin % 16 == 0 and 96 output channels, plain store";
  if (!fusable_second(p2) || !p2->w2f) return "second plan: 1x1 convolution 96 -> 192 without activation";
  return nullptr;
}

extern "C" int sntc_conv_fusable(const sntc_conv_plan* p, const sntc_conv_plan* p2) { return fused_pair_error(p, p2) ? 0 : 1; }

extern "C" int64_t sntc_conv_fused_workspace_bytes(const sntc_conv_plan* p, int n, int h, int w) {
  if (!p) return 0;
  Geo g;
  if (geometry(p, h, w, &g)) return 0;
  return 4 * workspace_floats(p, (int64_t)n * g.Qh * g.Qw, schedule(p, g, n, true));
}

extern "C" int sntc_conv_forward_fused(const sntc_conv_plan* p, const sntc_conv_plan* p2, const float* x, int n, int h, int w, float* y,
                                       const float* res, const float* aux, void* workspace, size_t workspace_bytes,
                                       void* stream) {
  if (const char* why = fused_pair_error(p, p2)) return fail(SNTC_ERR_UNSUPPORTED, why);
  return conv_forward_impl(p, p2, x, n, h, w, y, res, aux, workspace, workspace_bytes, stream);
}

extern "C" int sntc_conv_set_stream_k(int enabled) {
  g_stream_k_enabled.store(enabled ? 1 : 0, std::memory_order_relaxed);
  return SNTC_OK;
}

extern "C" int sntc_conv_get_stream_k(void) { return g_stream_k_enabled.load(std::memory_order_relaxed); }

__global__ void status_exchange_kernel(int* word, int* out) { *out = atomicExch(word, 0); }
__global__ void status_or_kernel(int* word, int flags) { atomicOr(word, flags); }

extern "C" int sntc_conv_status(int* flags, void* stream) {
  if (!flags) return fail(SNTC_ERR_BAD_SHAPE, "sntc_conv_status: null argument");
  int rc = gg_init();
  if (rc) return rc;
  int* word = gg_status_word();
  hipStream_t s = (hipStream_t)stream;
  hipLaunchKernelGGL(status_exchange_kernel, dim3(1), dim3(1), 0, s, word, word + 1);
  SNTC_HIP(hipGetLastError());
  SNTC_HIP(hipMemcpyAsync(flags, word + 1, sizeof(int), hipMemcpyDeviceToHost, s));
  SNTC_HIP(hipStreamSynchronize(s));
  return SNTC_OK;
}

extern "C" int sntc_conv_status_inject(int flags, void* stream) {
  int rc = gg_init();
  if (rc) return rc;
  hipLaunchKernelGGL(status_or_kernel, dim3(1), dim3(1), 0, (hipStream_t)stream, gg_status_word(), flags);
  SNTC_HIP(hipGetLastError());
  return SNTC_OK;
}
```

shallow-ntc_amd/csrc/gather_gemm.hip:

```cpp
#include "gather_gemm_kernel.h"

namespace sntc {

#define SNTC_GG_DECL_VEC(TM, TN, WM, WN) extern template __global__ void gg_kernel<TM, TN, WM, WN, true, false>(const GGArgs);
#define SNTC_GG_DECL_PRO(TM, TN, WM, WN)                                                   \
  extern template __global__ void gg_kernel<TM, TN, WM, WN, true, true>(const GGArgs);    \
  extern template __global__ void gg_kernel<TM, TN, WM, WN, false, true>(const GGArgs);
#define SNTC_GG_DECL_DMA(TM, TN, WM, WN) extern template __global__ void gg_kernel<TM, TN, WM, WN, true, false, false, true>(const GGArgs);
SNTC_GG_SHAPES(SNTC_GG_DECL_VEC)
SNTC_GG_SHAPES(SNTC_GG_DECL_PRO)
SNTC_GG_DMA_SHAPES(SNTC_GG_DECL_DMA)
extern template __global__ void gg_kernel<1, 1, 2, 2, true, false, false, true, kDeepRing>(const GGArgs);
extern template __global__ void gg_kernel<1, 3, 4, 1, true, false, false, false, 0, true>(const GGArgs);
extern template __global__ void gg_kernel<2, 2, 2, 2, true, false, false, false, 0, false, true>(const GGArgs);
extern template __global__ void gg_kernel<1, 2, 4, 1, true, false, true>(const GGArgs);
extern template __global__ void gg_kernel<1, 4, 4, 1, true, false, true>(const GGArgs);

__global__ void __launch_bounds__(256) gg_reduce_kernel(const GGArgs a) {
  const GGGroup G = a.g[blockIdx.y];
  const size_t total = (size_t)a.M * G.Ncol;
  const int per = a.Qh * a.Qw;
  for (size_t i = blockIdx.x * (size_t)blockDim.x + threadIdx.x; i < total; i += (size_t)gridDim.x * blockDim.x) {
    const int m = (int)(i / G.Ncol);
    const int col = (int)(i - (size_t)m * G.Ncol);
    float v = 0.0f;
    for (int sp = 0; sp < a.ksplit; ++sp) v += a.slab[G.slab_off + (size_t)sp * total + i];
    const unsigned ce = G.cols[col];
    const int ch = ce & 0xffff;
    const int n = m / per;
    const int rem = m - n * per;
    const int qy = rem / a.Qw + G.q0y, qx = rem - (rem / a.Qw) * a.Qw + G.q0x;
    const int oy = qy * a.sO + (int)((ce >> 24) & 0xff) - 128;
    const int ox = qx * a.sO + (int)((ce >> 16) & 0xff) - 128;
    if ((unsigned)oy >= (unsigned)a.Ho || (unsigned)ox >= (unsigned)a.Wo) continue;
    const size_t idx = (((size_t)n * a.Ho + oy) * a.Wo + ox) * a.Cout + ch;
    v = apply_act(v + (a.bias ? a.bias[ch] : 0.0f), a.act);
    a.y[idx] = apply_epilogue1(v, a.epi, a.res, a.aux, idx);
  }
}

int gg_reduce_launch(const GGArgs& args, hipStream_t stream) {
  size_t most = 0;
  for (int gi = 0; gi < args.ngroups; ++gi) most = std::max(most, (size_t)args.M * args.g[gi].Ncol);
  int blocks = (int)std::min<size_t>((most + 255) / 256, 2048);
  hipLaunchKernelGGL(gg_reduce_kernel, dim3(blocks, args.ngroups), dim3(256), 0, stream, args);
  hipError_t e = hipGetLastError();
  if (e != hipSuccess) return hip_fail(e, "split-K reduce launch");
  return SNTC_OK;
}

static GGInstance row(int v, GGLoad load, GGStage stage, GGForm form, int TM, int TN, int WM, int WN, const void* fn) {
  GGInstance r{v, load, stage, form, 32 * TM * WM, 32 * TN * WN, 64 * WM * WN, 0, (size_t)TM * TN * 16 * 64 * WM * WN, fn};
  const size_t rinfo = 2 * r.bm * sizeof(int4);
  if (form == kFormPresplitHalo)
    r.lds = (size_t)2 * kBf3PatchRounds * 512 * 16 + (size_t)(v == 12 ? kBf3DeepRing : 3) * r.bn * 96 + rinfo;
  else if (form == kFormBf3 || form == kFormPresplit)
    r.lds = (size_t)3 * (r.bm + r.bn) * 96 + rinfo;
  else
    r.lds = (size_t)(stage == kStageDeep ? kDeepRing : stage == kStageDma ? 4 : 3) * (r.bm + r.bn) * kStage * sizeof(float) + rinfo;
  return r;
}

#define GG(v, load, stage, form, TM, TN, WM, WN, ...) \
  row(v, load, stage, form, TM, TN, WM, WN, reinterpret_cast<const void*>(&gg_kernel<TM, TN, WM, WN, __VA_ARGS__>))
#define GG_LOADERS(v, TM, TN, WM, WN)                                        \
  GG(v, kLoadVec, kStageRing, kFormPlain, TM, TN, WM, WN, true, false),      \
  GG(v, kLoadVecPro, kStageRing, kFormPlain, TM, TN, WM, WN, true, true),    \
  GG(v, kLoadGather, kStageRing, kFormPlain, TM, TN, WM, WN, false, true)
#define GG_DMA(v, TM, TN, WM, WN) GG(v, kLoadVec, kStageDma, kFormPlain, TM, TN, WM, WN, true, false, false, true)
#define BF3P(v, TN, form) row(v, kLoadVec, kStageDma, form, 2, TN, 4, 2, bf3p_kernel(v, form == kFormPresplitHalo))

static const GGInstance kInstances[] = {
    GG_LOADERS(1, 1, 1, 4, 1), GG_LOADERS(2, 1, 2, 4, 1), GG_LOADERS(3, 1, 3, 4, 1), GG_LOADERS(4, 1, 4, 4, 1), GG_LOADERS(5, 1, 5, 4, 1),
    GG_LOADERS(6, 1, 6, 4, 1), GG_LOADERS(7, 1, 7, 4, 1), GG_LOADERS(8, 1, 1, 2, 2), GG_LOADERS(9, 2, 2, 2, 2), GG_LOADERS(10, 2, 4, 4, 1),
    GG_DMA(1, 1, 1, 4, 1), GG_DMA(2, 1, 2, 4, 1), GG_DMA(3, 1, 3, 4, 1), GG_DMA(4, 1, 4, 4, 1), GG_DMA(5, 1, 5, 4, 1),
    GG_DMA(8, 1, 1, 2, 2), GG_DMA(9, 2, 2, 2, 2),
    GG(8, kLoadVec, kStageDeep, kFormPlain, 1, 1, 2, 2, true, false, false, true, kDeepRing),
    GG(3, kLoadVec, kStageRing, kFormFuse2, 1, 3, 4, 1, true, false, false, false, 0, true),
    GG(9, kLoadVec, kStageRing, kFormColm, 2, 2, 2, 2, true, false, false, false, 0, false, true),
    GG(2, kLoadVec, kStageRing, kFormBf3, 1, 2, 4, 1, true, false, true),
    GG(4, kLoadVec, kStageRing, kFormBf3, 1, 4, 4, 1, true, false, true),
    BF3P(11, 4, kFormPresplit), BF3P(11, 4, kFormPresplitHalo), BF3P(12, 2, kFormPresplit), BF3P(12, 2, kFormPresplitHalo),
    BF3P(13, 3, kFormPresplit), BF3P(13, 3, kFormPresplitHalo),
};
#undef GG
#undef GG_LOADERS
#undef GG_DMA
#undef BF3P
constexpr int kNumInstances = sizeof(kInstances) / sizeof(kInstances[0]);

const GGInstance* gg_find(int variant, GGLoad load, GGStage stage, GGForm form) {
  for (const GGInstance& r : kInstances)
    if (r.variant == variant && r.load == load && r.stage == stage && r.form == form) return &r;
  return nullptr;
}

static bool presplit(const GGInstance& r) { return r.form == kFormPresplit || r.form == kFormPresplitHalo; }

constexpr int kMaxDevices = 16;
struct DeviceTables {
  std::once_flag once;
  int rc = SNTC_OK;
  int num_cus = 0;
  int resident[kNumInstances] = {};
  int* status = nullptr;
};
static DeviceTables g_dev[kMaxDevices];

static int fill_tables(DeviceTables& T, int dev) {
  hipDeviceProp_t prop;
  SNTC_HIP(hipGetDeviceProperties(&prop, dev));
  T.num_cus = prop.multiProcessorCount;
  for (int i = 0; i < kNumInstances; ++i) {
    const GGInstance& r = kInstances[i];
    SNTC_HIP(hipFuncSetAttribute(r.fn, hipFuncAttributeMaxDynamicSharedMemorySize, (int)r.lds));
    if (presplit(r)) {
      T.resident[i] = T.num_cus;
      continue;
    }
    int per_cu = 0;
    SNTC_HIP(hipOccupancyMaxActiveBlocksPerMultiprocessor(&per_cu, r.fn, r.threads, r.lds));
    per_cu = std::max(1, std::min({per_cu, 8, (int)(163840 / r.lds)}));
    T.resident[i] = per_cu * T.num_cus;
  }
  SNTC_HIP(hipMalloc(&T.status, 2 * sizeof(int)));
  SNTC_HIP(hipMemset(T.status, 0, 2 * sizeof(int)));
  return SNTC_OK;
}

static DeviceTables* current_tables() {
  int dev = 0;
  if (hipGetDevice(&dev) != hipSuccess || dev < 0 || dev >= kMaxDevices) return nullptr;
  DeviceTables& T = g_dev[dev];
  std::call_once(T.once, [&] { T.rc = fill_tables(T, dev); });
  return T.rc == SNTC_OK ? &T : nullptr;
}

int gg_init() {
  int dev = 0;
  SNTC_HIP(hipGetDevice(&dev));
  if (dev < 0 || dev >= kMaxDevices) return fail(SNTC_ERR_UNSUPPORTED, "device index beyond the residency tables");
  DeviceTables& T = g_dev[dev];
  std::call_once(T.once, [&] { T.rc = fill_tables(T, dev); });
  return T.rc;
}

int gg_resident(const GGInstance& inst) {
  const DeviceTables* T = current_tables();
  return T ? T->resident[&inst - kInstances] : 0;
}

int gg_num_cus() {
  const DeviceTables* T = current_tables();
  return T ? T->num_cus : 0;
}

int* gg_status_word() {
  const DeviceTables* T = current_tables();
  return T ? T->status : nullptr;
}

int gg_launch(const GGInstance& inst, const GGArgs& args, int nblocks, hipStream_t stream) {
  GGArgs a = args;
  a.dma = inst.stage;
  a.bf3 = inst.form == kFormBf3 || presplit(inst) ? 1 : 0;
  a.halo = inst.form == kFormPresplitHalo ? 1 : 0;
  if (!presplit(inst)) a.order = inst.form == kFormColm ? 0 : 1;
#ifdef SNTC_DIAG
  if (const char* e = getenv("SNTC_GG_DBG")) a.dbg = atoi(e);
#endif
  void* params[] = {&a};
  hipError_t e = hipLaunchKernel(inst.fn, dim3(nblocks), dim3(inst.threads), params, inst.lds, stream);
  if (e != hipSuccess) return hip_fail(e, "gather-GEMM launch");
  return SNTC_OK;
}

}
```

shallow-ntc_amd/csrc/gather_gemm_kernel.h:

```cpp
#pragma once
#include <algorithm>
#include <cstdlib>
#include <mutex>
#include <type_traits>
#include "sntc_internal.h"

namespace sntc {

typedef float f32x4 __attribute__((ext_vector_type(4)));
typedef float f32x16 __attribute__((ext_vector_type(16)));
typedef unsigned u32x4 __attribute__((ext_vector_type(4)));

constexpr unsigned kOutOfRange = 0x80000000u;
constexpr int kSpinLimit = 1 << 22;

__device__ __forceinline__ float apply_act(float v, int act) {
  switch (act) {
    case SNTC_ACT_RELU: return fmaxf(v, 0.0f);
    case SNTC_ACT_LEAKY_RELU: return v >= 0.0f ? v : 0.2f * v;
    case SNTC_ACT_SIGMOID: return 1.0f / (1.0f + expf(-v));
    default: return v;
  }
}

template <int HI, int LO, class F>
__device__ __forceinline__ bool first_of_desc(F&& f) {
  if constexpr (HI < LO) {
    return false;
  } else {
    if (f(std::integral_constant<int, HI>{})) return true;
    return first_of_desc<HI - 1, LO>(f);
  }
}

__device__ __forceinline__ f32x4 buf_load(__amdgpu_buffer_rsrc_t rsrc, unsigned voff, unsigned soff) {
  const u32x4 v = __builtin_amdgcn_raw_buffer_load_b128(rsrc, (int)voff, (int)soff, 0);
  return __builtin_bit_cast(f32x4, v);
}

__device__ __forceinline__ void buf_store(__amdgpu_buffer_rsrc_t rsrc, f32x4 v, unsigned voff, unsigned soff) {
  __builtin_amdgcn_raw_buffer_store_b128(__builtin_bit_cast(u32x4, v), rsrc, (int)voff, (int)soff, 0);
}

__device__ __forceinline__ float buf_load1(__amdgpu_buffer_rsrc_t rsrc, unsigned voff) {
  return __builtin_bit_cast(float, __builtin_amdgcn_raw_buffer_load_b32(rsrc, (int)voff, 0, 0));
}

__device__ __forceinline__ f32x4 apply_epilogue(f32x4 v, int epi, const f32x4 rs, const float* aux, size_t idx) {
  switch (epi) {
    case SNTC_EPI_ADD: return v + rs;
    case SNTC_EPI_GATE: return rs + *reinterpret_cast<const f32x4*>(aux + idx) * v;
    case SNTC_EPI_RES_DIV: return rs / v;
    case SNTC_EPI_RES_MUL: return rs * v;
    case SNTC_EPI_RES_DIV_SQRT:
#pragma unroll
      for (int e = 0; e < 4; ++e) v[e] = rs[e] / sqrtf(v[e]);
      return v;
    case SNTC_EPI_RES_MUL_SQRT:
#pragma unroll
      for (int e = 0; e < 4; ++e) v[e] = rs[e] * sqrtf(v[e]);
      return v;
    case SNTC_EPI_MASK_RELU:
#pragma unroll
      for (int e = 0; e < 4; ++e) v[e] = rs[e] > 0.0f ? v[e] : 0.0f;
      return v;
    case SNTC_EPI_MASK_LEAKY:
#pragma unroll
      for (int e = 0; e < 4; ++e) v[e] = rs[e] >= 0.0f ? v[e] : 0.2f * v[e];
      return v;
    default: return v;
  }
}

__device__ __forceinline__ float apply_epilogue1(float v, int epi, const float* res, const float* aux, size_t idx) {
  switch (epi) {
    case SNTC_EPI_ADD: return v + res[idx];
    case SNTC_EPI_GATE: return res[idx] + aux[idx] * v;
    case SNTC_EPI_RES_DIV: return res[idx] / v;
    case SNTC_EPI_RES_MUL: return res[idx] * v;
    case SNTC_EPI_RES_DIV_SQRT: return res[idx] / sqrtf(v);
    case SNTC_EPI_RES_MUL_SQRT: return res[idx] * sqrtf(v);
    case SNTC_EPI_MASK_RELU: return res[idx] > 0.0f ? v : 0.0f;
    case SNTC_EPI_MASK_LEAKY: return res[idx] >= 0.0f ? v : 0.2f * v;
    default: return v;
  }
}

typedef const GGArgs __attribute__((address_space(4))) KArgs;
__device__ __forceinline__ KArgs& fresh_args() {
  KArgs* kp = (KArgs*)__builtin_amdgcn_kernarg_segment_ptr();
  asm volatile("" : "+s"(kp));
  return *kp;
}

struct Piece {
  int gi, mt, nt, k0, k1;
  int consume;
  int publish;
  int split;
};

constexpr int gg_waves(int tiles) { return tiles == 1 ? 4 : (tiles <= 3 ? 3 : 2); }

typedef __bf16 bf16x8 __attribute__((ext_vector_type(8)));
typedef __bf16 bf16x4 __attribute__((ext_vector_type(4)));

__device__ __forceinline__ void split3(float x, __bf16* hi, __bf16* mid, __bf16* lo) {
  const __bf16 h = (__bf16)x;
  const float r1 = x - (float)h;
  const __bf16 m = (__bf16)r1;
  const float r2 = r1 - (float)m;
  *hi = h; *mid = m; *lo = (__bf16)r2;
}

template <int TM, int TN, int WM, int WN, bool VEC, bool PRO, bool BF3 = false, bool DMA = false, int DEEP = 0, bool FUSE2 = false,
          bool COLM = false>
__global__ void __launch_bounds__(256, FUSE2 ? 2 : gg_waves(TM * TN)) gg_kernel(const GGArgs a) {
  static_assert(!BF3 || (VEC && !PRO), "the bf16 x 3 experiment covers the vector path without prologue");
  static_assert(!DMA || (VEC && !PRO && !BF3), "direct-to-LDS staging: vector path, no prologue (nothing can touch the data on the way)");
  static_assert(!FUSE2 || (TM == 1 && TN == 3 && WM == 4 && WN == 1 && VEC && !PRO && !BF3 && !DMA),
                "FUSE2: 3x3 (N = 96) -> 1x1 (96 -> 192) of a ResidualBlock, the 128 x 96 register-staged instance only");
  static_assert(DEEP == 0 || (DMA && (DEEP & (DEEP - 1)) == 0 && DEEP >= 4), "DEEP: ring slots of the direct-to-LDS pipeline, a power of two");
  constexpr int RING = DMA ? (DEEP ? DEEP : 4) : 3;
  constexpr int BM = WM * TM * 32;
  constexpr int BN = WN * TN * 32;
  constexpr int SLOT = BF3 ? (BM + BN) * 24 : (BM + BN) * kStage;
  constexpr int A_CH = BM / 64;
  constexpr int B_CH = BF3 ? (BN * 6 + 255) / 256 : (BN + 63) / 64;
  constexpr int A_SC = BM / 16;
  constexpr int EPW = 32 * (TN >= 2 ? 64 : 32);
  constexpr bool DBUF = !BF3 && TM * TN <= 8 && TN <= 5;
  constexpr bool RBUF = DBUF && TM * TN <= 3 && !FUSE2;
  static_assert(RING * SLOT >= 4 * EPW + (DMA ? SLOT : 0), "epilogue staging (and one prefetched stage) must fit in the stage ring");
  extern __shared__ __attribute__((aligned(16))) char smem[];
  float* ring = reinterpret_cast<float*>(smem);
  int4* rinfo_all = reinterpret_cast<int4*>(ring + RING * SLOT);

  const int tid = threadIdx.x;
  const int lane = tid & 63;
  const int wave = tid >> 6;
  const int wm = wave / WN;
  const int wn = wave % WN;
  const int l31 = lane & 31;
  const int h = lane >> 5;

  int sk_head_t = -1, sk_head_k1 = 0;
  int sk_tail_t = -1, sk_tail_k0 = 0;
  int sk_cur = 0, sk_last = -1;
  int sk_phase = 0;
  int wl = 0;
  if (a.sk) {
    const int w = blockIdx.x;
    wl = (w & 7) * (a.nworkers >> 3) + (w >> 3);
    const int u_lo = (int)(a.units * wl / a.nworkers);
    const int u_hi = (int)(a.units * (wl + 1) / a.nworkers);
    auto locate = [&](int u, int* t, int* k, int* steps) {
      if constexpr (COLM) {
        const int st = a.g[0].steps;
        const int per = a.ntm * st;
        const int nt = u / per;
        const int r2 = u - nt * per;
        const int mt = r2 / st;
        *t = nt * a.ntm + mt;
        *k = r2 - mt * st;
        *steps = st;
      } else {
        const int mt = u / a.ups;
        const int r = u - mt * a.ups;
        int gi = 0;
#pragma unroll
        for (int i = 1; i < kMaxGroups; ++i)
          if (i < a.ngroups && r >= (int)a.g[i].unit0) gi = i;
        const int r2 = r - (int)a.g[gi].unit0;
        const int nt = r2 / a.g[gi].steps;
        *t = mt * a.tps + a.g[gi].tile0 + nt;
        *k = r2 - nt * a.g[gi].steps;
        *steps = a.g[gi].steps;
      }
    };
    if (u_hi > u_lo) {
      int tF, kF, sF, tL, kL, sL;
      locate(u_lo, &tF, &kF, &sF);
      locate(u_hi - 1, &tL, &kL, &sL);
      sk_cur = tF;
      sk_last = tL;
      if (kF > 0) { sk_tail_t = tF; sk_tail_k0 = kF; sk_cur = tF + 1; }
      if (kL + 1 < sL) { sk_head_t = tL; sk_head_k1 = kL + 1; sk_last = tL - 1; }
    } else {
      sk_phase = 3;
    }
  }

  auto tile_of = [&](int t, Piece* p) {
    KArgs& a = fresh_args();
    if constexpr (COLM) {
      const int nt = t / a.ntm;
      p->gi = 0;
      p->mt = t - nt * a.ntm;
      p->nt = nt;
    } else {
      const int mt = t / a.tps;
      const int r = t - mt * a.tps;
      int gi = 0;
#pragma unroll
      for (int i = 1; i < kMaxGroups; ++i)
        if (i < a.ngroups && r >= a.g[i].tile0) gi = i;
      p->gi = gi;
      p->mt = mt;
      p->nt = r - a.g[gi].tile0;
    }
  };

  auto next_piece = [&](Piece* p) -> bool {
    KArgs& a = fresh_args();
    if (!a.sk) return false;
    if (sk_phase == 0) {
      sk_phase = 1;
      if (sk_head_t >= 0) {
        tile_of(sk_head_t, p);
        p->k0 = 0; p->k1 = sk_head_k1; p->consume = -1; p->publish = 1; p->split = 0;
        return true;
      }
    }
    if (sk_phase == 1) {
      if (sk_cur <= sk_last) {
        tile_of(sk_cur++, p);
        p->k0 = 0; p->k1 = a.g[p->gi].steps; p->consume = -1; p->publish = 0; p->split = 0;
        return true;
      }
      sk_phase = 2;
    }
    if (sk_phase == 2) {
      sk_phase = 3;
      if (sk_tail_t >= 0) {
        tile_of(sk_tail_t, p);
        p->k0 = sk_tail_k0; p->k1 = a.g[p->gi].steps; p->consume = wl - 1; p->publish = 0; p->split = 0;
        return true;
      }
    }
    return false;
  };

  Piece P;
  bool have;
  if (a.sk) {
    have = next_piece(&P);
  } else {
    int gi = 0;
#pragma unroll
    for (int i = 1; i < kMaxGroups; ++i)
      if (i < a.ngroups && (int)blockIdx.x >= a.g[i].blk0) gi = i;
    const int lb0 = blockIdx.x - a.g[gi].blk0;
    const int split = lb0 % a.ksplit;
    const int lb = lb0 / a.ksplit;
    const int ntn = a.g[gi].ntn;
    const int full = a.ntm & ~7;
    if (lb < full * ntn) {
      const int l = lb >> 3;
      P.mt = (l / ntn) * 8 + (lb & 7);
      P.nt = l % ntn;
    } else {
      const int r = lb - full * ntn, rem = a.ntm - full;
      P.mt = full + r % rem;
      P.nt = r / rem;
    }
    const int steps = a.g[gi].steps;
    P.gi = gi;
    P.k0 = (int)(((long long)split * steps) / a.ksplit);
    P.k1 = (int)(((long long)(split + 1) * steps) / a.ksplit);
    P.consume = -1; P.publish = 0; P.split = split;
    have = true;
  }
  if (!have) return;

  const __amdgpu_buffer_rsrc_t xs =
      __builtin_amdgcn_make_buffer_rsrc(const_cast<float*>(a.x), 0, (int)a.x_bytes, 0x00020000);
  const int r0 = tid >> 2;
  const int c = DMA ? ((tid & 3) ^ ((r0 >> 2) & 3)) : (tid & 3);
  const int wsw = (c ^ ((r0 >> 2) & 3)) << 2;
  const int kk = tid & 15;
  const int rs = tid >> 4;
  const int gsw = (((kk >> 2) ^ ((rs >> 2) & 3)) << 2) + (kk & 3);
  constexpr int NROW = VEC ? A_CH : A_SC;

  int a_iy0[NROW], a_ix0[NROW];
  unsigned a_img[NROW];
  unsigned a_off[NROW];
  unsigned b_off[B_CH];
  int ld_stage = 0, ld_t = 0, ld_cc = 0;
  int ld_ty = 0, ld_tx = 0;
  int g_t = 0, g_ch = 0, g_ty = 0, g_tx = 0;
  int g_T = a.g[P.gi].T, g_tw = a.g[P.gi].tw;
  __amdgpu_buffer_rsrc_t ws =
      __builtin_amdgcn_make_buffer_rsrc(const_cast<float*>(a.g[P.gi].wp), 0, a.g[P.gi].Ncol * a.g[P.gi].K * (BF3 ? 6 : 4), 0x00020000);
  int m0 = 0, n0 = 0;

  auto set_tap = [&](int ty, int tx) {
#pragma unroll
    for (int i = 0; i < NROW; ++i) {
      const int iy = a_iy0[i] + ty * a.tstep;
      const int ix = a_ix0[i] + tx * a.tstep;
      const bool ok = (unsigned)iy < (unsigned)a.H && (unsigned)ix < (unsigned)a.W;
      const unsigned pix = ((unsigned)(iy * a.W + ix) * (unsigned)a.Cin * 4u) & 0x7fffffffu;
      a_off[i] = (a_img[i] + pix) | (ok ? 0u : kOutOfRange);
    }
  };

  auto write_rinfo = [&](const Piece& p, int rb) {
    KArgs& a = fresh_args();
    int4* rinfo = rinfo_all + rb * BM;
    const int mbase = p.mt * BM;
    const int q0y = a.g[p.gi].q0y, q0x = a.g[p.gi].q0x;
    for (int r = tid; r < BM; r += 256) {
      const int m = mbase + r;
      int4 ri = make_int4(0, 0, 0, 0);
      if (m < a.M) {
        const int per = a.Qh * a.Qw;
        const int n = m / per;
        const int rem = m - n * per;
        const int qy = rem / a.Qw;
        ri = make_int4(n, qy + q0y, rem - qy * a.Qw + q0x, 1);
      }
      rinfo[r] = ri;
    }
  };

  auto init_loader = [&](const Piece& p, int rb) {
    KArgs& a = fresh_args();
    const int4* rinfo = rinfo_all + rb * BM;
    const auto& G = a.g[p.gi];
    g_T = G.T;
    g_tw = G.tw;
    ws = __builtin_amdgcn_make_buffer_rsrc(const_cast<float*>(G.wp), 0, G.Ncol * G.K * (BF3 ? 6 : 4), 0x00020000);
    m0 = p.mt * BM;
    n0 = p.nt * BN;
#pragma unroll
    for (int i = 0; i < NROW; ++i) {
      const int4 ri = rinfo[VEC ? r0 + 64 * i : rs + 16 * i];
      a_iy0[i] = ri.y * a.sA + a.offy;
      a_ix0[i] = ri.z * a.sA + a.offx;
      a_img[i] = ri.w ? (unsigned)ri.x * (unsigned)(a.H * a.W) * (unsigned)a.Cin * 4u + (VEC ? (unsigned)c * 16u : 0u)
                      : kOutOfRange;
    }
#pragma unroll
    for (int i = 0; i < B_CH; ++i) {
      if (BF3) {
        const int q = tid + 256 * i;
        const int brow = min(n0 + q / 6, G.Ncol - 1);
        b_off[i] = (unsigned)brow * (unsigned)(G.K / kStage) * 96u + (unsigned)(q % 6) * 16u;
      } else {
        const int brow = min(n0 + r0 + 64 * i, G.Ncol - 1);
        b_off[i] = (unsigned)brow * (unsigned)G.K * 4u + (unsigned)c * 16u;
      }
    }
    ld_stage = p.k0;
    if (VEC) {
      ld_cc = p.k0 / g_T;
      ld_t = p.k0 - ld_cc * g_T;
      ld_ty = ld_t / g_tw;
      ld_tx = ld_t - ld_ty * g_tw;
      set_tap(ld_ty, ld_tx);
    } else {
      const int k = p.k0 * kStage + kk;
      g_t = k / a.Cin;
      g_ch = k - g_t * a.Cin;
      g_ty = g_t / g_tw;
      g_tx = g_t - g_ty * g_tw;
    }
  };

  struct Regs {
    f32x4 a[VEC ? A_CH : 1];
    float s[VEC ? 1 : A_SC];
    f32x4 b[B_CH];
  };

  auto advance_stage = [&]() {
    ++ld_stage;
    if (VEC) {
      const int row_end = (ld_tx + 1 == g_tw) ? 1 : 0;
      const int tap_end = (ld_t + 1 == g_T) ? 1 : 0;
      ld_tx = row_end ? 0 : ld_tx + 1;
      ld_ty = tap_end ? 0 : ld_ty + row_end;
      ld_t = tap_end ? 0 : ld_t + 1;
      ld_cc += tap_end;
      set_tap(ld_ty, ld_tx);
    }
  };

  auto load_regs = [&](Regs& R) {
    if (VEC) {
      const unsigned soff = (unsigned)ld_cc * 64u;
#pragma unroll
      for (int i = 0; i < A_CH; ++i) R.a[i] = buf_load(xs, a_off[i], soff);
    } else {
      const bool kok = g_t < g_T;
      const int ty = g_ty * a.tstep, tx = g_tx * a.tstep;
#pragma unroll
      for (int i = 0; i < A_SC; ++i) {
        const int iy = a_iy0[i] + ty;
        const int ix = a_ix0[i] + tx;
        const bool ok = kok && (unsigned)iy < (unsigned)a.H && (unsigned)ix < (unsigned)a.W && !(a_img[i] & kOutOfRange);
        const unsigned off = a_img[i] + ((unsigned)(iy * a.W + ix) * (unsigned)a.Cin + (unsigned)g_ch) * 4u;
        R.s[i] = buf_load1(xs, ok ? off : kOutOfRange);
      }
      g_ch += kStage;
      while (g_ch >= a.Cin) {
        g_ch -= a.Cin;
        ++g_t;
        if (++g_tx == g_tw) { g_tx = 0; ++g_ty; }
      }
    }
    const unsigned wsoff = (unsigned)ld_stage * (BF3 ? 96u : 64u);
#pragma unroll
    for (int i = 0; i < B_CH; ++i)
      if (BF3 ? ((BN * 6) % 256 == 0 || tid + 256 * i < BN * 6) : (BN % 64 == 0 || r0 + 64 * i < BN))
        R.b[i] = buf_load(ws, b_off[i], wsoff);
    advance_stage();
  };

  const int my_nb = [&]() {
    int nb = 0;
#pragma unroll
    for (int i = 0; i < B_CH; ++i) nb += ((tid >> 6) * 16 + 64 * i < BN) ? 1 : 0;
    return nb;
  }();
  const int wave_u = __builtin_amdgcn_readfirstlane(tid >> 6);
  auto dma_stage = [&](int slot) {
    typedef __attribute__((address_space(3))) void lds_void;
    float* Ab = ring + __builtin_amdgcn_readfirstlane(slot) * SLOT + wave_u * 16 * kStage;
    const unsigned soff = (unsigned)__builtin_amdgcn_readfirstlane(ld_cc) * 64u;
#pragma unroll
    for (int i = 0; i < A_CH; ++i)
      __builtin_amdgcn_raw_ptr_buffer_load_lds(xs, (lds_void*)(Ab + 64 * i * kStage), 16, (int)a_off[i], (int)soff, 0, 0);
    float* Bb = Ab + BM * kStage;
    const unsigned wsoff = (unsigned)__builtin_amdgcn_readfirstlane(ld_stage) * 64u;
#pragma unroll
    for (int i = 0; i < B_CH; ++i)
      if (BN % 64 == 0 || wave_u * 16 + 64 * i < BN)
        __builtin_amdgcn_raw_ptr_buffer_load_lds(ws, (lds_void*)(Bb + 64 * i * kStage), 16, (int)b_off[i], (int)wsoff, 0, 0);
    advance_stage();
  };
  auto dma_wait = [&](auto K) {
    constexpr int k = decltype(K)::value < 0 ? 0 : decltype(K)::value;
    if (k == 0) {
      asm volatile("s_waitcnt vmcnt(0)" ::: "memory");
    } else if (my_nb == B_CH) {
      asm volatile("s_waitcnt vmcnt(%0)" ::"n"(k * (A_CH + B_CH)) : "memory");
    } else {
      asm volatile("s_waitcnt vmcnt(%0)" ::"n"(k * (A_CH + B_CH - 1)) : "memory");
    }
  };
  auto write_lds = [&](const Regs& R, int slot) {
    float* Ab = ring + slot * SLOT;
    if (BF3) {
      char* Ap = reinterpret_cast<char*>(Ab);
      char* Bp = Ap + 3 * BM * 32;
#pragma unroll
      for (int i = 0; i < A_CH; ++i) {
        const int r = r0 + 64 * i;
        bf16x4 hi, mid, lo;
#pragma unroll
        for (int e = 0; e < 4; ++e) {
          __bf16 x0, x1, x2;
          split3(R.a[i][e], &x0, &x1, &x2);
          hi[e] = x0; mid[e] = x1; lo[e] = x2;
        }
        const int off = r * 32 + (((c >> 1) ^ ((r >> 3) & 1)) << 4) + ((c & 1) << 3);
        *reinterpret_cast<bf16x4*>(Ap + off) = hi;
        *reinterpret_cast<bf16x4*>(Ap + BM * 32 + off) = mid;
        *reinterpret_cast<bf16x4*>(Ap + 2 * BM * 32 + off) = lo;
      }
#pragma unroll
      for (int i = 0; i < B_CH; ++i) {
        const int q = tid + 256 * i;
        if ((BN * 6) % 256 == 0 || q < BN * 6) {
          const int r = q / 6, part = q % 6, plane = part >> 1, half = part & 1;
          *reinterpret_cast<f32x4*>(Bp + plane * BN * 32 + r * 32 + ((half ^ ((r >> 3) & 1)) << 4)) = R.b[i];
        }
      }
      return;
    }
    float* Bb = Ab + BM * kStage;
    if (VEC) {
#pragma unroll
      for (int i = 0; i < A_CH; ++i) {
        f32x4 v = R.a[i];
        if (PRO) {
          if (a.pro == SNTC_PRO_ABS) {
            v[0] = fabsf(v[0]); v[1] = fabsf(v[1]); v[2] = fabsf(v[2]); v[3] = fabsf(v[3]);
          } else if (a.pro == SNTC_PRO_SQUARE) {
            v = v * v;
          }
        }
        *reinterpret_cast<f32x4*>(Ab + (r0 + 64 * i) * kStage + wsw) = v;
      }
    } else {
#pragma unroll
      for (int i = 0; i < A_SC; ++i) {
        float v = R.s[i];
        if (PRO) {
          if (a.pro == SNTC_PRO_ABS) v = fabsf(v);
          else if (a.pro == SNTC_PRO_SQUARE) v = v * v;
        }
        Ab[(rs + 16 * i) * kStage + gsw] = v;
      }
    }
#pragma unroll
    for (int i = 0; i < B_CH; ++i)
      if (BN % 64 == 0 || r0 + 64 * i < BN)
        *reinterpret_cast<f32x4*>(Bb + (r0 + 64 * i) * kStage + wsw) = R.b[i];
  };

  const int swz = (l31 >> 2) & 3;
  const int fa_row = (wm * TM * 32 + l31) * kStage;
  const int fb_row = (BM + wn * TN * 32 + l31) * kStage;
  const int foff0 = ((0 + h) ^ swz) << 2, foff1 = ((2 + h) ^ swz) << 2;

  struct Frag {
    f32x4 a[TM];
    f32x4 b[TN];
  };
  auto read_frag = [&](Frag& F, int slot, int g) {
    const float* base = ring + slot * SLOT;
    const int off = g ? foff1 : foff0;
#pragma unroll
    for (int i = 0; i < TM; ++i) F.a[i] = *reinterpret_cast<const f32x4*>(base + fa_row + i * 32 * kStage + off);
#pragma unroll
    for (int j = 0; j < TN; ++j) F.b[j] = *reinterpret_cast<const f32x4*>(base + fb_row + j * 32 * kStage + off);
  };

  struct Frag3 {
    bf16x8 a[BF3 ? 3 : 1][TM];
    bf16x8 b[BF3 ? 3 : 1][TN];
  };
  auto read_frag3 = [&](Frag3& F, int slot) {
    const char* base = reinterpret_cast<const char*>(ring + slot * SLOT);
    const int hoff = (h ^ ((l31 >> 3) & 1)) << 4;
#pragma unroll
    for (int p = 0; p < (BF3 ? 3 : 1); ++p) {
#pragma unroll
      for (int i = 0; i < TM; ++i)
        F.a[p][i] = *reinterpret_cast<const bf16x8*>(base + p * BM * 32 + (wm * TM * 32 + i * 32 + l31) * 32 + hoff);
#pragma unroll
      for (int j = 0; j < TN; ++j)
        F.b[p][j] = *reinterpret_cast<const bf16x8*>(base + 3 * BM * 32 + p * BN * 32 + (wn * TN * 32 + j * 32 + l31) * 32 + hoff);
    }
  };

  f32x16 acc[TM][TN];
  auto mfma3 = [&](const Frag3& F) {
    constexpr int PA[6] = {2, 0, 1, 1, 0, 0};
    constexpr int PB[6] = {0, 2, 1, 0, 1, 0};
#pragma unroll
    for (int t = 0; t < (BF3 ? 6 : 0); ++t)
#pragma unroll
      for (int i = 0; i < TM; ++i)
#pragma unroll
        for (int j = 0; j < TN; ++j)
          acc[i][j] = __builtin_amdgcn_mfma_f32_32x32x16_bf16(F.a[BF3 ? PA[t] : 0][i], F.b[BF3 ? PB[t] : 0][j], acc[i][j], 0, 0, 0);
  };
  auto mfma_group = [&](const Frag& F) {
    if (SNTC_DBG(a, 64)) return;
#pragma unroll
    for (int e = 0; e < 4; ++e)
#pragma unroll
      for (int i = 0; i < TM; ++i)
#pragma unroll
        for (int j = 0; j < TN; ++j)
          acc[i][j] = FUSE2 ? __builtin_amdgcn_mfma_f32_32x32x2f32(F.b[j][e], F.a[i][e], acc[i][j], 0, 0, 0)
                            : __builtin_amdgcn_mfma_f32_32x32x2f32(F.a[i][e], F.b[j][e], acc[i][j], 0, 0, 0);
  };

  int rb = 0;
  Regs R0, R1;
  write_rinfo(P, rb);
  __syncthreads();
  init_loader(P, rb);
  int dma_issued = 0;
  if (DMA) {
    const int n = P.k1 - P.k0;
    for (; dma_issued < RING - 1 && dma_issued < n; ++dma_issued) dma_stage(dma_issued);
  } else {
    const int n = P.k1 - P.k0;
    if (n > 0) load_regs(R0);
    if (RBUF && n > 1) load_regs(R1);
  }

  while (true) {
    const int n = P.k1 - P.k0;
    if (P.consume >= 0) {
      if (tid == 0) {
        int spins = 0;
        while (__hip_atomic_load(a.sk_flags + P.consume, __ATOMIC_RELAXED, __HIP_MEMORY_SCOPE_AGENT) == 0) {
          __builtin_amdgcn_s_sleep(8);
          if (++spins > kSpinLimit) {
            __hip_atomic_fetch_or(fresh_args().status, 1, __ATOMIC_RELAXED, __HIP_MEMORY_SCOPE_AGENT);
            break;
          }
        }
        __builtin_amdgcn_fence(__ATOMIC_ACQUIRE, "agent");
        asm volatile("s_waitcnt vmcnt(0)" ::: "memory");
      }
      __syncthreads();
      const __amdgpu_buffer_rsrc_t sr = __builtin_amdgcn_make_buffer_rsrc(
          a.sk_slab + (size_t)P.consume * (TM * TN * 16 * 256), 0, TM * TN * 16 * 256 * 4, 0x00020000);
#pragma unroll
      for (int i = 0; i < TM; ++i)
#pragma unroll
        for (int j = 0; j < TN; ++j)
#pragma unroll
          for (int q = 0; q < 4; ++q) {
            const f32x4 v = buf_load(sr, (unsigned)tid * 16u, (unsigned)((i * TN + j) * 4 + q) * 4096u);
            acc[i][j][4 * q] = v[0]; acc[i][j][4 * q + 1] = v[1]; acc[i][j][4 * q + 2] = v[2]; acc[i][j][4 * q + 3] = v[3];
          }
    } else {
#pragma unroll
      for (int i = 0; i < TM; ++i)
#pragma unroll
        for (int j = 0; j < TN; ++j)
#pragma unroll
          for (int e = 0; e < 16; ++e) acc[i][j][e] = 0.0f;
    }

    Frag F0, F1;
    if (DMA) {
      for (; dma_issued < RING - 1 && dma_issued < n; ++dma_issued) dma_stage(dma_issued);
      using Yes = std::integral_constant<bool, true>;
      using No = std::integral_constant<bool, false>;
      auto wait_first = [&](auto I) {
        constexpr int i = decltype(I)::value;
        if constexpr (i > 2) {
          if (n >= i) { dma_wait(std::integral_constant<int, i - 2>{}); return true; }
        }
        return false;
      };
      if (!first_of_desc<RING - 1, 3>(wait_first)) dma_wait(std::integral_constant<int, 0>{});
      __builtin_amdgcn_s_barrier();
      __builtin_amdgcn_sched_barrier(0);
      if (n > 0) read_frag(F0, 0, 0);
      auto dstep = [&](int j, auto LD, auto PF, auto REM) {
        if (decltype(LD)::value) dma_stage((j + RING - 1) & (RING - 1));
        read_frag(F1, j & (RING - 1), 1);
        mfma_group(F0);
        if (decltype(PF)::value) read_frag(F0, (j + 1) & (RING - 1), 0);
        mfma_group(F1);
        if (decltype(LD)::value) {
          constexpr int NW = A_CH + B_CH, NR = TM + TN, NM = 4 * TM * TN;
          __builtin_amdgcn_sched_group_barrier(0x008, 1, 0);
          __builtin_amdgcn_sched_group_barrier(0x020, NW, 0);
          __builtin_amdgcn_sched_group_barrier(0x008, 1, 0);
          __builtin_amdgcn_sched_group_barrier(0x100, NR, 0);
          __builtin_amdgcn_sched_group_barrier(0x008, NM - 2, 0);
          __builtin_amdgcn_sched_group_barrier(0x008, 1, 0);
          __builtin_amdgcn_sched_group_barrier(0x100, NR, 0);
          __builtin_amdgcn_sched_group_barrier(0x008, NM - 1, 0);
        }
        __builtin_amdgcn_sched_barrier(0);
        if constexpr (decltype(LD)::value) dma_wait(std::integral_constant<int, RING - 3>{});
        else dma_wait(std::integral_constant<int, decltype(REM)::value - 3>{});
        asm volatile("s_waitcnt lgkmcnt(0)" ::: "memory");
        __builtin_amdgcn_s_barrier();
        __builtin_amdgcn_sched_barrier(0);
      };
      int j = 0;
      for (; j + RING - 1 < n; ++j) dstep(j, Yes{}, Yes{}, std::integral_constant<int, -1>{});
      auto tail = [&](auto REM) {
        constexpr int rem = decltype(REM)::value;
        if (n - j == rem) {
          if constexpr (rem > 1) dstep(j, No{}, Yes{}, REM);
          else dstep(j, No{}, No{}, REM);
          ++j;
        }
      };
      first_of_desc<RING - 1, 1>([&](auto REM) { tail(REM); return false; });
      dma_issued = 0;
    } else {
    int s_cur = 0, s_n1 = 1, s_n2 = 2;
    if (n > 0) write_lds(R0, 0);
    if (RBUF) {
      if (n > 1) write_lds(R1, 1);
    } else if (n > 1) {
      load_regs(R0);
      write_lds(R0, 1);
    }
    if (n > 2) load_regs(R0);
    __syncthreads();
    if (DBUF && n > 0) read_frag(F0, 0, 0);

    auto step = [&](auto WR, auto LD, auto PF) {
      if (decltype(WR)::value && !SNTC_DBG(a, 2)) write_lds(R0, s_n2);
      if (decltype(LD)::value && !SNTC_DBG(a, 1)) load_regs(R0);
      if (BF3) {
        Frag3 F3;
        read_frag3(F3, s_cur);
        mfma3(F3);
      } else if (DBUF) {
        if (!SNTC_DBG(a, 8)) read_frag(F1, s_cur, 1);
        mfma_group(F0);
        if (decltype(PF)::value && !SNTC_DBG(a, 8)) read_frag(F0, s_n1, 0);
        mfma_group(F1);
      } else {
        read_frag(F0, s_cur, 0);
        mfma_group(F0);
        read_frag(F0, s_cur, 1);
        mfma_group(F0);
      }
      if (DBUF && VEC && decltype(WR)::value && decltype(LD)::value && decltype(PF)::value) {
        constexpr int NW = A_CH + B_CH, NR = TM + TN, NM = 4 * TM * TN;
        __builtin_amdgcn_sched_group_barrier(0x008, 1, 0);
        __builtin_amdgcn_sched_group_barrier(0x200, NW, 0);
        __builtin_amdgcn_sched_group_barrier(0x008, 1, 0);
        __builtin_amdgcn_sched_group_barrier(0x020, NW, 0);
        __builtin_amdgcn_sched_group_barrier(0x008, 1, 0);
        __builtin_amdgcn_sched_group_barrier(0x100, NR, 0);
        __builtin_amdgcn_sched_group_barrier(0x008, NM - 3, 0);
        __builtin_amdgcn_sched_group_barrier(0x008, 1, 0);
        __builtin_amdgcn_sched_group_barrier(0x100, NR, 0);
        __builtin_amdgcn_sched_group_barrier(0x008, NM - 1, 0);
      }
      __builtin_amdgcn_sched_barrier(0);
      if (!SNTC_DBG(a, 4)) __syncthreads();
      __builtin_amdgcn_sched_barrier(0);
      const int t = s_cur; s_cur = s_n1; s_n1 = s_n2; s_n2 = t;
    };
    using Yes = std::integral_constant<bool, true>;
    using No = std::integral_constant<bool, false>;
    for (int j = 0; j + 3 < n; ++j) step(Yes{}, Yes{}, Yes{});
    if (n >= 3) step(Yes{}, No{}, Yes{});
    if (n >= 2) step(No{}, No{}, Yes{});
    if (n >= 1) step(No{}, No{}, No{});
    }

    Piece Q;
    const bool more = next_piece(&Q);
    const int qb = rb ^ 1;
    const int4* rinfo = rinfo_all + rb * BM;
    const int m0d = m0, n0d = n0;
    if (more) {
      write_rinfo(Q, qb);
      __syncthreads();
      init_loader(Q, qb);
      const int nq = Q.k1 - Q.k0;
      if (DMA) {
        constexpr int NPF = (RING * SLOT - 4 * EPW) / SLOT < RING - 1 ? (RING * SLOT - 4 * EPW) / SLOT : RING - 1;
        for (dma_issued = 0; dma_issued < NPF && dma_issued < nq; ++dma_issued) dma_stage(dma_issued);
      } else {
        if (nq > 0) load_regs(R0);
        if (RBUF && nq > 1) load_regs(R1);
      }
    }

    int te = tid;
    asm volatile("" : "+v"(te));
    const int lane = te & 63, wave = te >> 6, l31 = lane & 31, h = lane >> 5;
    const int wm = wave / WN, wn = wave % WN;
    KArgs& a = fresh_args();
    const auto& Gd = a.g[P.gi];
    if (P.publish) {
      const __amdgpu_buffer_rsrc_t sr = __builtin_amdgcn_make_buffer_rsrc(
          a.sk_slab + (size_t)wl * (TM * TN * 16 * 256), 0, TM * TN * 16 * 256 * 4, 0x00020000);
#pragma unroll
      for (int i = 0; i < TM; ++i)
#pragma unroll
        for (int j = 0; j < TN; ++j)
#pragma unroll
          for (int q = 0; q < 4; ++q) {
            const f32x4 v = {acc[i][j][4 * q], acc[i][j][4 * q + 1], acc[i][j][4 * q + 2], acc[i][j][4 * q + 3]};
            buf_store(sr, v, (unsigned)tid * 16u, (unsigned)((i * TN + j) * 4 + q) * 4096u);
          }
      asm volatile("s_waitcnt vmcnt(0)" ::: "memory");
      __syncthreads();
      if (tid == 0) {
        __builtin_amdgcn_fence(__ATOMIC_RELEASE, "agent");
        asm volatile("s_waitcnt vmcnt(0)" ::: "memory");
        __hip_atomic_store(a.sk_flags + wl, 1, __ATOMIC_RELAXED, __HIP_MEMORY_SCOPE_AGENT);
      }
    } else if (a.ksplit > 1) {
      float* slab = a.slab + Gd.slab_off + (size_t)P.split * a.M * Gd.Ncol;
#pragma unroll
      for (int j = 0; j < TN; ++j) {
        const int col = n0d + (wn * TN + j) * 32 + l31;
        if (col >= Gd.Ncol) continue;
#pragma unroll
        for (int i = 0; i < TM; ++i)
#pragma unroll
          for (int r = 0; r < 16; ++r) {
            const int m = m0d + (wm * TM + i) * 32 + (r & 3) + 8 * (r >> 2) + 4 * h;
            if (m < a.M) slab[(size_t)m * Gd.Ncol + col] = acc[i][j][r];
          }
      }
    } else if constexpr (FUSE2) {
#pragma unroll
      for (int j = 0; j < 3; ++j)
#pragma unroll
        for (int q = 0; q < 4; ++q) {
          f32x4 b1 = {0.f, 0.f, 0.f, 0.f};
          if (a.bias) b1 = *reinterpret_cast<const f32x4*>(a.bias + 32 * j + 8 * q + 4 * h);
#pragma unroll
          for (int e = 0; e < 4; ++e) acc[0][j][4 * q + e] = apply_act(acc[0][j][4 * q + e] + b1[e], a.act);
        }
      float* stage = ring + 2 * 3072 + wave * 1024;
      const f32x4* w2src = reinterpret_cast<const f32x4*>(a.w2f);
      f32x4 wreg[3];
#pragma unroll
      for (int u = 0; u < 3; ++u) wreg[u] = w2src[te + 256 * u];
      const int c4 = (lane & 7) << 2;
      const int rsub = lane >> 3;
      const int mrow = m0d + wave * 32 + rsub;
      __syncthreads();
#pragma unroll 1
      for (int ct = 0; ct < (SNTC_DBG(a, 128) ? 0 : 6); ++ct) {
        float* w2s = ring + (ct & 1) * 3072;
#pragma unroll
        for (int u = 0; u < 3; ++u) reinterpret_cast<f32x4*>(w2s)[te + 256 * u] = wreg[u];
        __syncthreads();
        if (ct < 5) {
#pragma unroll
          for (int u = 0; u < 3; ++u) wreg[u] = w2src[(ct + 1) * 768 + te + 256 * u];
        }
        const int ch = 32 * ct + c4;
        f32x4 rv[4];
#pragma unroll
        for (int p = 0; p < 4; ++p) {
          rv[p] = f32x4{0.f, 0.f, 0.f, 0.f};
          if (a.epi != SNTC_EPI_STORE && mrow + 8 * p < a.M)
            rv[p] = *reinterpret_cast<const f32x4*>(a.res + (size_t)(mrow + 8 * p) * a.Cout2 + ch);
        }
        f32x16 acc2;
#pragma unroll
        for (int e = 0; e < 16; ++e) acc2[e] = 0.0f;
#pragma unroll
        for (int j = 0; j < 3; ++j)
#pragma unroll
          for (int q = 0; q < 4; ++q) {
            const f32x4 bq = *reinterpret_cast<const f32x4*>(w2s + ((4 * j + q) * 64 + lane) * 4);
#pragma unroll
            for (int e = 0; e < 4; ++e)
              acc2 = __builtin_amdgcn_mfma_f32_32x32x2f32(acc[0][j][4 * q + e], bq[e], acc2, 0, 0, 0);
          }
#pragma unroll
        for (int r = 0; r < 16; ++r) stage[((r & 3) + 8 * (r >> 2) + 4 * h) * 32 + l31] = acc2[r];
        f32x4 bv = {0.f, 0.f, 0.f, 0.f};
        if (a.bias2) bv = *reinterpret_cast<const f32x4*>(a.bias2 + ch);
#pragma unroll
        for (int p = 0; p < 4; ++p) {
          const int m = mrow + 8 * p;
          if (m >= a.M) continue;
          const size_t idx = (size_t)m * a.Cout2 + ch;
          f32x4 v = *reinterpret_cast<const f32x4*>(stage + (rsub + 8 * p) * 32 + c4) + bv;
          if (a.epi != SNTC_EPI_STORE) v = apply_epilogue(v, a.epi, rv[p], a.aux, idx);
          *reinterpret_cast<f32x4*>(a.y + idx) = v;
        }
      }
    } else if ((a.Cout & 3) == 0) {
      float* stage = ring + (DMA ? RING * SLOT - 4 * EPW : 0) + wave * EPW;
#pragma unroll
      for (int i = 0; i < TM; ++i)
#pragma unroll
      for (int j0 = 0; j0 < TN; j0 += 2) {
        const int ct = (TN - j0) >= 2 ? 2 : 1;
        const int wfl = ct * 32;
#pragma unroll
        for (int jj = 0; jj < 2; ++jj) {
          if (jj < ct) {
#pragma unroll
            for (int r = 0; r < 16; ++r)
              stage[((r & 3) + 8 * (r >> 2) + 4 * h) * wfl + jj * 32 + l31] = acc[i][j0 + jj][r];
          }
        }
        const int lanes_per_row = wfl >> 2;
        const int rows_per_pass = 64 / lanes_per_row;
        const int c4 = (lane % lanes_per_row) << 2;
        const int rsub = lane / lanes_per_row;
        const int col = n0d + (wn * TN + j0) * 32 + c4;
        const bool col_ok = col < Gd.Ncol;
        unsigned ce = 0;
        f32x4 bv = {0.f, 0.f, 0.f, 0.f};
        if (col_ok) {
          ce = Gd.cols[col];
          if (a.bias) bv = *reinterpret_cast<const f32x4*>(a.bias + (ce & 0xffff));
        }
        const int ch = ce & 0xffff;
        const int oyo = (int)((ce >> 24) & 0xff) - 128;
        const int oxo = (int)((ce >> 16) & 0xff) - 128;
        for (int rp = 0; rp < 32; rp += rows_per_pass) {
          const int rloc = rp + rsub;
          const int4 ri = rinfo[(wm * TM + i) * 32 + rloc];
          const int oy = ri.y * a.sO + oyo;
          const int ox = ri.z * a.sO + oxo;
          if (!col_ok || !ri.w || (unsigned)oy >= (unsigned)a.Ho || (unsigned)ox >= (unsigned)a.Wo) continue;
          const size_t idx = (((size_t)ri.x * a.Ho + oy) * a.Wo + ox) * a.Cout + ch;
          f32x4 v = *reinterpret_cast<const f32x4*>(stage + rloc * wfl + c4) + bv;
#pragma unroll
          for (int e = 0; e < 4; ++e) v[e] = apply_act(v[e], a.act);
          if (a.epi != SNTC_EPI_STORE)
            v = apply_epilogue(v, a.epi, SNTC_DBG(a, 32) ? v : *reinterpret_cast<const f32x4*>(a.res + idx), a.aux, idx);
          if (!SNTC_DBG(a, 16) || v[0] == 12345.678f) *reinterpret_cast<f32x4*>(a.y + idx) = v;
        }
      }
    } else {
#pragma unroll
      for (int j = 0; j < TN; ++j) {
        const int col = n0d + (wn * TN + j) * 32 + l31;
        if (col >= Gd.Ncol) continue;
        const unsigned ce = Gd.cols[col];
        const int ch = ce & 0xffff;
        const int oyo = (int)((ce >> 24) & 0xff) - 128;
        const int oxo = (int)((ce >> 16) & 0xff) - 128;
        const float bv = a.bias ? a.bias[ch] : 0.0f;
#pragma unroll
        for (int i = 0; i < TM; ++i)
#pragma unroll
        for (int r = 0; r < 16; ++r) {
          const int row = (wm * TM + i) * 32 + (r & 3) + 8 * (r >> 2) + 4 * h;
          const int4 ri = rinfo[row];
          if (!ri.w) continue;
          const int oy = ri.y * a.sO + oyo;
          const int ox = ri.z * a.sO + oxo;
          if ((unsigned)oy >= (unsigned)a.Ho || (unsigned)ox >= (unsigned)a.Wo) continue;
          const size_t idx = (((size_t)ri.x * a.Ho + oy) * a.Wo + ox) * a.Cout + ch;
          a.y[idx] = apply_epilogue1(apply_act(acc[i][j][r] + bv, a.act), a.epi, a.res, a.aux, idx);
        }
      }
    }
    if (!more) break;
    __syncthreads();
    P = Q;
    rb = qb;
  }
}

#define SNTC_GG_SHAPES(X) X(1, 1, 4, 1) X(1, 2, 4, 1) X(1, 3, 4, 1) X(1, 4, 4, 1) X(1, 5, 4, 1) X(1, 6, 4, 1) X(1, 7, 4, 1) X(1, 1, 2, 2) X(2, 2, 2, 2) X(2, 4, 4, 1)
#define SNTC_GG_DMA_SHAPES(X) X(1, 1, 4, 1) X(1, 2, 4, 1) X(1, 3, 4, 1) X(1, 4, 4, 1) X(1, 5, 4, 1) X(1, 1, 2, 2) X(2, 2, 2, 2)
constexpr int kDeepRing = 8;

}
```

shallow-ntc_amd/csrc/sntc_internal.h:

```cpp
#pragma once
#include <hip/hip_runtime.h>
#include <stdint.h>
#include <string>
#include "../../include/sntc.h"

namespace sntc {

void set_error(const std::string& msg);
int fail(int code, const std::string& msg);
int hip_fail(hipError_t e, const char* what);
int zero_async(void* p, size_t bytes, hipStream_t stream);

#define SNTC_HIP(expr)                                         \
  do {                                                         \
    hipError_t _e = (expr);                                    \
    if (_e != hipSuccess) return ::sntc::hip_fail(_e, #expr);  \
  } while (0)

constexpr int kMaxGroups = 4;

#ifdef SNTC_DIAG
#define SNTC_DBG(a, bit) (((a).dbg & (bit)) != 0)
#else
#define SNTC_DBG(a, bit) false
#endif

struct GGGroup {
  const float* wp;
  const int* taps;
  const int* cols;
  int T;
  int tw;
  int K;
  int Ncol;
  int ntn;
  int blk0;
  size_t slab_off;
  int q0y, q0x;
  int steps;
  int tile0;
  long long unit0;
};

struct GGArgs {
  const float* x;
  float* y;
  const float* bias;
  const float* res;
  const float* aux;
  unsigned x_bytes;
  int N, H, W, Cin;
  int Qh, Qw, M;
  int Ho, Wo, Cout;
  int sA, tstep, offy, offx, sO;
  int act, epi, pro;
  int ntm;
  int ksplit;
  float* slab;
  int sk;
  int nworkers;
  long long units;
  int tps, ups;
  float* sk_slab;
  int* sk_flags;
  int* status;
  const float* w2f;
  const float* bias2;
  int Cout2;
  int dma;
  int bf3;
  int halo;
  int order;
  int dbg;
  int ngroups;
  GGGroup g[kMaxGroups];
};

constexpr int kNumVariants = 10;
constexpr int kMaxVariant = 13;
constexpr int kStage = 16;

enum GGLoad { kLoadVec, kLoadVecPro, kLoadGather };
enum GGStage { kStageRing, kStageDma, kStageDeep };
enum GGForm { kFormPlain, kFormFuse2, kFormColm, kFormBf3, kFormPresplit, kFormPresplitHalo };
struct GGInstance {
  int variant;
  GGLoad load;
  GGStage stage;
  GGForm form;
  int bm, bn, threads;
  size_t lds;
  size_t slab_floats;
  const void* fn;
};
const GGInstance* gg_find(int variant, GGLoad load, GGStage stage, GGForm form);
int gg_init();
int gg_resident(const GGInstance& inst);
int gg_num_cus();
int* gg_status_word();
int gg_launch(const GGInstance& inst, const GGArgs& args, int nblocks, hipStream_t stream);
int gg_reduce_launch(const GGArgs& args, hipStream_t stream);

constexpr int kBf3PatchRounds = 5;
constexpr int kBf3DeepRing = 3;
int bf3p_patch_rows_max();
const void* bf3p_kernel(int variant, bool halo);

constexpr int kMaxW = 4;
constexpr int kMaxL = 5;
struct DFDesc {
  int nl;
  int w[kMaxL + 1];
  int off_m[kMaxL], off_b[kMaxL], off_f[kMaxL];
  int stride;
};

}

struct sntc_prior {
  int channels = 0;
  sntc::DFDesc d{};
  float* rec = nullptr;
};
```

shallow-ntc_amd/ops.py:

```python
from __future__ import annotations

import ctypes as C
import os

import numpy as np
import torch

from . import _capi as capi

ACTS = {None: capi.ACT_NONE, "none": capi.ACT_NONE, "relu": capi.ACT_RELU, "leaky_relu": capi.ACT_LEAKY_RELU,
        "lrelu": capi.ACT_LEAKY_RELU, "sigmoid": capi.ACT_SIGMOID}
KINDS = {"conv": capi.CONV2D, "convT": capi.CONV2D_TRANSPOSE, "sigdown": capi.SIGNAL_DOWN, "sigup": capi.SIGNAL_UP}


WGRAD_STREAM = None
FUSE_RESIDUAL_TAIL = True
MEAN_ONLY_HYPER = True
FUSE_RESIDUAL_BLOCK = not os.environ.get("SNTC_NO_RB_FUSE")
FUSED_BLOCK_MIN_TILES = 256
CONCURRENT_BRANCHES = not os.environ.get("SNTC_NO_BRANCH_STREAMS")
CONCURRENT_BRANCH_MAX_TILES = 1024
MAX_INPUT_BYTES = 1 << 31
PROFILE = None
ROW_PACKED_FIRST_LAYER = not os.environ.get("SNTC_NO_ROWPACK")
# ... 405 lines not shown
        else:
            ws_bytes = int(capi.load().sntc_conv_tune_workspace_bytes(self._h, n, h, w))
            ws = torch.empty((ws_bytes // 4,), dtype=torch.float32, device=x.device) if ws_bytes else None
            capi.call("sntc_conv_plan_tune", self._h, _ptr(x), n, h, w, _ptr(y), _ptr(res), _ptr(aux), _ptr(ws), ws_bytes, int(reps),
                      C.byref(v), C.byref(sk), _stream())
        self._tuned[(n, h, w)] = (v.value, sk.value)
        return v.value, sk.value

    def clear_tuning(self):
        capi.call("sntc_conv_plan_clear_tuning", self._h)
        self._tuned = {}
        for v in self._views.values():
            v._tuned = {}

    def drop_choice(self, n, h, w):
        capi.call("sntc_conv_plan_drop_choice", self._h, int(n), int(h), int(w), self._ncols)
        self._tuned.pop((int(n), int(h), int(w)), None)

    def candidates(self, n, h, w):
        v, s = (C.c_int * 32)(), (C.c_int * 32)()
        if self._ncols:
            k = int(capi.load().sntc_conv_columns_candidates(self._h, int(n), int(h), int(w), self._ncols, v, s, 32))
        else:
            k = int(capi.load().sntc_conv_plan_candidates(self._h, int(n), int(h), int(w), v, s, 32))
        if k < 0:
            raise capi.SntcError(capi.ERR_BAD_SHAPE, capi.last_error())
        return [(v[i], s[i]) for i in range(k)]

    def set_choice(self, n, h, w, variant, stream_k):
        if self._ncols:
            capi.call("sntc_conv_columns_set_choice", self._h, int(n), int(h), int(w), self._ncols, int(variant), int(bool(stream_k)))
        else:
            capi.call("sntc_conv_plan_set_choice", self._h, int(n), int(h), int(w), int(variant), int(bool(stream_k)))
        self._tuned[(int(n), int(h), int(w))] = (int(variant), int(bool(stream_k)))

    def __call__(self, x, res=None, aux=None, out=None):
        if self.s3:
            _check_s3(x, self.cin)
        else:
            _check_nhwc(x, self.cin)
        n, h, w = x.shape[:3]
        ho, wo = self.out_hw(h, w)
        y = out if out is not None else torch.empty((n, ho, wo, self.cout), dtype=torch.float32, device=x.device)
        for t in (res, aux):
            if t is not None and tuple(t.shape) != tuple(y.shape):
                raise ValueError(f"epilogue operand shape {tuple(t.shape)} != output shape {tuple(y.shape)}")
        if x.numel() * x.element_size() >= MAX_INPUT_BYTES and n > 1:
            half = n // 2
            r0 = None if res is None else res[:half]
            r1 = None if res is None else res[half:]
            a0 = None if aux is None else aux[:half]
            a1 = None if aux is None else aux[half:]
            self.__call__(x[:half], r0, a0, out=y[:half])
            self.__call__(x[half:], r1, a1, out=y[half:])
            return y
        if AUTOTUNE and (n, h, w) not in self._tuned:
            self.tune(x, res, aux, reps=AUTOTUNE)
        if LAUNCH_LOG is not None:
            LAUNCH_LOG.append((self, int(n), int(h), int(w)))
        prof = PROFILE
        if prof is not None:
            e0, e1 = torch.cuda.Event(enable_timing=True), torch.cuda.Event(enable_timing=True)
            e0.record()
        if self._ncols:
            ws_bytes = int(capi.load().sntc_conv_columns_workspace_bytes(self._h, n, h, w, self._ncols))
            ws = torch.empty((ws_bytes // 4,), dtype=torch.float32, device=x.device) if ws_bytes else None
            capi.call("sntc_conv_forward_columns", self._h, _ptr(x), n, h, w, _ptr(y), _ptr(res), _ptr(aux), _ptr(ws), ws_bytes, _stream(),
                      self._ncols)
        else:
            ws_bytes = int(capi.load().sntc_conv_workspace_bytes(self._h, n, h, w))
            ws = torch.empty((ws_bytes // 4,), dtype=torch.float32, device=x.device) if ws_bytes else None
            capi.call("sntc_conv_forward", self._h, _ptr(x), n, h, w, _ptr(y), _ptr(res), _ptr(aux), _ptr(ws), ws_bytes, _stream())
        if prof is not None:
            e1.record()
            v, nb = self.launch_info(n, h, w)
            prof.append(dict(e0=e0, e1=e1, flops=(self.parent if self._ncols else self).flops(n, h, w), launched_flops=self.flops(n, h, w),
                             variant=v, nblocks=nb, vec=self.cin % 16 == 0 or self.rowpack,
                             kind=self.kind, k=self.k[0], s=self.stride, cin=self.cin, cout=self.cout, n=n, h=h, w=w,
                             colm=self.launch_order(n, h, w)))
        return y


class ConvPlanColumns(ConvPlan):

    def __init__(self, parent, ncols):
        self.parent, self._ncols = parent, int(ncols)
        self.kind, self.cin, self.cout, self.stride, self.k = parent.kind, parent.cin, int(ncols), parent.stride, parent.k
        self.epilogue, self.bf16x3, self.s3, self.rowpack = parent.epilogue, parent.bf16x3, parent.s3, parent.rowpack
        self._h = parent._h
        self._tuned = {}
        self._views = {}

    def __del__(self):
        pass

    def columns(self, ncols):
        return self.parent.columns(ncols)

    def update(self, weight, bias=None):
        self.parent.update(weight, bias)

    def clear_tuning(self):
        self.parent.clear_tuning()

    def fusable_with(self, second):
        return False

    def fused(self, second, x, res=None, aux=None):
        raise capi.SntcError(capi.ERR_UNSUPPORTED, "a column-limited view cannot be the first half of a fused pair")


def take_conv_status():
    flags = C.c_int(0)
    capi.call("sntc_conv_status", C.byref(flags), _stream())
    return int(flags.value)


def check_conv_status():
    if take_conv_status():
        _latch_stream_k_off()
        raise capi.SntcError(capi.ERR_HIP, "a stream-K hand-off timed out (the device is shared with other streams / processes): "
                                           "the results since the last check are invalid; stream-K is now off, run the step again")


FUSED_TAIL_MIN_ROWS = 24576
LAUNCH_LOG = None
AUTOTUNE = False


class autotune:

    def __init__(self, reps=3):
        self.reps = int(reps)

    def __enter__(self):
        global AUTOTUNE
        self._old = AUTOTUNE
        AUTOTUNE = self.reps
        return self

    def __exit__(self, *exc):
        global AUTOTUNE
        AUTOTUNE = self._old
        return False


def tune_step(step_fn, reps=12, min_gain=0.004, max_launches=16, log=None, burst=1, passes=1):
    global LAUNCH_LOG

    def clock():
        ts = []
        for _ in range(reps):
            e0, e1 = torch.cuda.Event(enable_timing=True), torch.cuda.Event(enable_timing=True)
            e0.record()
            for _ in range(burst):
                step_fn()
            e1.record()
            e1.synchronize()
            ts.append(e0.elapsed_time(e1) / burst)
        ts.sort()
        return ts[len(ts) // 2]

    LAUNCH_LOG = []
    try:
        step_fn()
        torch.cuda.synchronize()
        launches = list(dict.fromkeys(LAUNCH_LOG))
    finally:
        LAUNCH_LOG = None
    launches.sort(key=lambda e: -e[0].flops(e[1], e[2], e[3]))
    for _ in range(3):
        step_fn()
    check_conv_status()
    base = clock()
    if take_conv_status():
        _latch_stream_k_off()
        raise capi.SntcError(capi.ERR_HIP, "tune_step: a stream-K hand-off of the step timed out with the schedules it came with; "
                                           "stream-K is now off, run the step again")
    rollback = []
    for walk in range(max(1, int(passes))):
        changed = False
        for plan, n, h, w in launches[:max_launches]:
            if plan.rowpack:
                continue
            start = plan.launch_info(n, h, w)
            had = plan._tuned.get((n, h, w))

            def restore(plan=plan, n=n, h=h, w=w, had=had):
                if had is not None:
                    plan.set_choice(n, h, w, *had)
                else:
                    plan.drop_choice(n, h, w)

            if walk == 0:
                rollback.append(restore)

            ref = clock()
            if take_conv_status():
                ref = float("inf")
            chosen, t_chosen = None, ref
            for v, sk in plan.candidates(n, h, w):
                plan.set_choice(n, h, w, v, sk)
                if plan.launch_info(n, h, w) == start and (had is None or (v, sk) == tuple(had)):
                    continue
                t = clock()
                if t < t_chosen * (1.0 - min_gain):
                    t = max(t, clock())
                if take_conv_status():
                    continue
                if t < t_chosen * (1.0 - min_gain):
                    chosen, t_chosen = (v, sk), t
            if chosen is not None:
                plan.set_choice(n, h, w, *chosen)
                changed = True
            else:
                restore()
            if log is not None:
                log.append(dict(layer=f"{plan.kind} k{plan.k[0]} s{plan.stride} {plan.cin}->{plan.cout}", shape=[n, h, w], start=list(start),
                                chosen=None if chosen is None else list(chosen), ref_ms=round(ref, 4), step_ms=round(t_chosen, 4), walk=walk))
        if not changed:
            break
    for _ in range(3):
        step_fn()
    if take_conv_status():
        for undo in rollback:
            undo()
        for _ in range(3):
            step_fn()
        if take_conv_status():
            _latch_stream_k_off()
            raise capi.SntcError(capi.ERR_HIP, "tune_step: stream-K hand-offs of the step time out; stream-K is now off, run the step again")
        if log is not None:
            log.append(dict(rolled_back=True))
        return base, base
    after = clock()
    if take_conv_status() or not (after == after and after != float("inf")):
        after = base
    return base, after


def export_tuning():
    out = []
    for idx, ref in enumerate(_PLAN_REGISTRY):
        p = ref()
        if p is None:
            continue
        for (n, h, w), (v, sk) in sorted(p._tuned.items()):
            out.append((idx, p.kind, p.cin, p.cout, int(n), int(h), int(w), int(v), int(sk)))
        for ncols, view in sorted(p._views.items()):
            for (n, h, w), (v, sk) in sorted(view._tuned.items()):
                out.append((idx, p.kind, p.cin, int(ncols), int(n), int(h), int(w), int(v), int(sk)))
    return out


def import_tuning(entries, strict=True):
    applied = 0
    for idx, kind, cin, cout, n, h, w, v, sk in entries:
        if idx >= len(_PLAN_REGISTRY):
            if not strict:
                continue
            raise capi.SntcError(capi.ERR_BAD_SHAPE, f"import_tuning: plan {idx} does not exist here ({len(_PLAN_REGISTRY)} plans "
                                 "were built): the ranks did not build the same plans in the same order")
        p = _PLAN_REGISTRY[idx]()
        if p is None:
            continue
        if (p.kind, p.cin) == (kind, cin) and 0 < cout < p.cout and p.columns_supported(cout):
            p = p.columns(cout)
        if (p.kind, p.cin, p.cout) != (kind, cin, cout):
            if not strict:
                continue
            raise capi.SntcError(capi.ERR_BAD_SHAPE, f"import_tuning: plan {idx} here is {(p.kind, p.cin, p.cout)}, the entry was "
                                 f"measured on {(kind, cin, cout)}: the ranks did not build the same plans in the same order")
        try:
            p.set_choice(n, h, w, v, sk)
            applied += 1
        except capi.SntcError:
            if strict:
                raise
    return applied


STREAM_K_TIMED_OUT = False


def _latch_stream_k_off():
    global STREAM_K_TIMED_OUT
    STREAM_K_TIMED_OUT = True
    capi.call("sntc_conv_set_stream_k", 0)


def set_stream_k(enabled, force=False):
    global STREAM_K_TIMED_OUT
    if enabled and STREAM_K_TIMED_OUT and not force:
        return
    if enabled and force:
        STREAM_K_TIMED_OUT = False
    capi.call("sntc_conv_set_stream_k", int(bool(enabled)))


def stream_k_enabled():
    return bool(capi.load().sntc_conv_get_stream_k())


class static_schedules:

    def __init__(self, active=True):
        self.active = bool(active)

    def __enter__(self):
        self._was = stream_k_enabled()
        if self.active and self._was:
            set_stream_k(False)
        return self

    def __exit__(self, *exc):
        if self.active and self._was:
            set_stream_k(True)
        return False


def gdn_small(x, beta, gamma, inverse=False, alpha=1, epsilon=1.0):
    _check_nhwc(x)
    c = x.shape[-1]
    y = torch.empty_like(x)
    capi.call("sntc_gdn_small", _ptr(x), x.numel() // c, c, _ptr(beta), _ptr(gamma), int(inverse), int(alpha),
              int(epsilon == 0.5), _ptr(y), _stream())
    return y


GDN_SMALL_CHANNELS = (4, 8, 12, 16, 24, 32, 48)
TAIL_CHANNELS = (12, 24, 48)
TAIL_ACTS = {None: 0, "none": 0, "igdn": 1, "igdn1": 1, "gdn": 2, "gdn1": 2, "relu": 3, "leaky_relu": 4, "lrelu": 4}


def _tail_profile(n, hh, wh, ch, cout, k2, s2):
    prof = PROFILE
    if prof is None:
        return None
    e0, e1 = torch.cuda.Event(enable_timing=True), torch.cuda.Event(enable_timing=True)
    e0.record()
    return prof, dict(e0=e0, e1=e1, flops=2 * n * hh * wh * k2 * k2 * ch * cout, variant=0, nblocks=0, vec=True, kind="tail",
                      k=k2, s=s2, cin=ch, cout=cout, n=n, h=hh, w=wh)


def _tail_profile_done(rec):
    if rec is not None:
        rec[1]["e1"].record()
        rec[0].append(rec[1])


def two_layer_tail(t, ch, has_res, act_kind, beta, gamma, w2, b2, k2=5, s2=2):
    _check_nhwc(t, ch * (2 if has_res else 1))
    n, hh, wh, _ = t.shape
    cout = int(w2.shape[2])
    y = torch.empty((n, hh * s2, wh * s2, cout), dtype=torch.float32, device=t.device)
    rec = _tail_profile(n, hh, wh, ch, cout, k2, s2)
    capi.call("sntc_two_layer_tail", _ptr(t), n, hh, wh, ch, int(has_res), act_kind, _ptr(beta), _ptr(gamma),
              _ptr(w2), _ptr(b2), k2, s2, cout, _ptr(y), _stream())
    _tail_profile_done(rec)
    return y


def two_layer_tail_pixels(t, ch, has_res, act_kind, beta, gamma, w2, b2, h, w, reference=None, k2=5, s2=2):
    _check_nhwc(t, ch * (2 if has_res else 1))
    n, hh, wh, _ = t.shape
    cout = int(w2.shape[2])
    px = torch.empty((n, h, w, cout), dtype=torch.uint8, device=t.device)
    sse = None
    if reference is not None:
        _check_nhwc(reference, cout)
        if tuple(reference.shape) != (n, h, w, cout):
            raise ValueError(f"reference {tuple(reference.shape)} does not match the decoded size {(n, h, w, cout)}")
        sse = torch.empty((n,), dtype=torch.int64, device=t.device)
    rec = _tail_profile(n, hh, wh, ch, cout, k2, s2)
    capi.call("sntc_two_layer_tail_pixels", _ptr(t), n, hh, wh, ch, int(has_res), act_kind, _ptr(beta), _ptr(gamma), _ptr(w2),
              _ptr(b2), k2, s2, cout, h, w, _ptr(reference), _ptr(px), _ptr(sse), _stream())
    _tail_profile_done(rec)
    return px, sse


def pad_zero(x, top, left, bottom, right):
    _check_nhwc(x)
    n, h, w, c = x.shape
    y = torch.empty((n, h + top + bottom, w + left + right, c), dtype=torch.float32, device=x.device)
    capi.call("sntc_pad_zero", _ptr(x), n, h, w, c, top, left, h + top + bottom, w + left + right, _ptr(y), _stream())
    return y


class RowPackedConv:

    def __init__(self, weight, bias, stride, act=None):
        self.k, self.stride = int(weight.shape[0]), int(stride)
        self.plan = ConvPlan("conv", weight, bias, stride, act, rowpack=True)
        self.cin, self.cout = self.plan.cin, self.plan.cout

    def _pads(self, size):
        out = -(-size // self.stride)
        total = max((out - 1) * self.stride + self.k - size, 0)
        return total // 2, total - total // 2

    def out_hw(self, h, w):
        return -(-h // self.stride), -(-w // self.stride)

    def flops(self, n, h, w):
        ho, wo = self.out_hw(h, w)
        return 2 * n * ho * wo * self.k * self.k * self.cin * self.cout

    def __call__(self, x, res=None, aux=None):
        _check_nhwc(x, self.cin)
        (pt, pb), (pl, pr) = self._pads(x.shape[1]), self._pads(x.shape[2])
        return self.plan(pad_zero(x, pt, pl, pb, pr), res, aux)


RGB_FIRST_LAYER = not os.environ.get("SNTC_NO_RGBCONV")


class RgbConvPlan:

    @staticmethod
    def supported(k, stride, cin, cout, act=None, kind="conv"):
        return act in ACTS and kind in ("conv", "sigdown") and bool(
            capi.load().sntc_rgbconv_supported(KINDS[kind], int(k), int(stride), int(cin), int(cout), ACTS[act]))

    def __init__(self, weight, bias, stride, act=None, kind="conv"):
        capi.require_gpu()
        self.kind = kind
        self.k, self.stride = int(weight.shape[0]), int(stride)
        self.cin, self.cout = int(weight.shape[2]), int(weight.shape[3])
        if weight.shape[0] != weight.shape[1]:
            raise ValueError(f"first-layer kernel {tuple(weight.shape)} is not square")
        w = weight.contiguous()
        b = None if bias is None else bias.contiguous()
        self._h = C.c_void_p()
        capi.call("sntc_rgbconv_plan_create", KINDS[kind], self.k, self.stride, self.cin, self.cout, _ptr(w), _ptr(b), ACTS[act], _stream(), C.byref(self._h))
        torch.cuda.current_stream().synchronize()

    def __del__(self):
        h = getattr(self, "_h", None)
        if h is not None and h.value:
            try:
                capi.load().sntc_rgbconv_plan_destroy(h)
            except Exception:
                pass
            self._h = None

    def update(self, weight, bias=None):
        capi.call("sntc_rgbconv_plan_update", self._h, _ptr(weight), _ptr(bias), _stream())

    def set_workgroups(self, n):
        capi.call("sntc_rgbconv_plan_set_workgroups", self._h, int(n))

    def out_hw(self, h, w):
        return -(-h // self.stride), -(-w // self.stride)

    def flops(self, n, h, w):
        return int(capi.load().sntc_rgbconv_flops(self._h, n, h, w))

    def __call__(self, x, res=None, aux=None):
        if res is not None or aux is not None:
            raise ValueError("the first-layer kernel has no epilogue operands")
        _check_nhwc(x, self.cin)
        n, h, w, _ = x.shape
        ho, wo = self.out_hw(h, w)
        if n > 1 and max(x.numel(), n * ho * wo * self.cout) * 4 >= MAX_INPUT_BYTES:
            half = n // 2
            return torch.cat([self(x[:half]), self(x[half:])])
        y = torch.empty((n, ho, wo, self.cout), dtype=torch.float32, device=x.device)
        prof = PROFILE
        if prof is not None:
            e0, e1 = torch.cuda.Event(enable_timing=True), torch.cuda.Event(enable_timing=True)
            e0.record()
        capi.call("sntc_rgbconv_forward", self._h, _ptr(x), n, h, w, _ptr(y), _stream())
        if prof is not None:
            e1.record()
            prof.append(dict(e0=e0, e1=e1, flops=self.flops(n, h, w), variant=0, nblocks=0, vec=True, kind="rgbconv", k=self.k, s=self.stride,
                             cin=self.cin, cout=self.cout, n=n, h=h, w=w))
        return y


SMALL_OUTPUT_LAYER = not os.environ.get("SNTC_NO_UPSMALL")


class UpSmallPlan:

    @staticmethod
    def supported(kind, k, stride, cin, cout):
        return kind in ("convT", "sigup") and bool(capi.load().sntc_upsmall_supported(KINDS[kind], int(k), int(stride), int(cin), int(cout)))

    def __init__(self, kind, weight, bias, stride):
        capi.require_gpu()
        self.kind, self.stride = kind, int(stride)
        self.k = int(weight.shape[0])
        self.cout, self.cin = (int(weight.shape[2]), int(weight.shape[3])) if kind == "convT" else (int(weight.shape[3]), int(weight.shape[2]))
        w = weight.contiguous()
        b = None if bias is None else bias.contiguous()
        self._h = C.c_void_p()
        capi.call("sntc_upsmall_plan_create", KINDS[kind], self.k, self.stride, self.cin, self.cout, _ptr(w), _ptr(b), _stream(), C.byref(self._h))
        torch.cuda.current_stream().synchronize()

    def __del__(self):
        h = getattr(self, "_h", None)
        if h is not None and h.value:
            try:
                capi.load().sntc_upsmall_plan_destroy(h)
            except Exception:
                pass
            self._h = None

    def update(self, weight, bias=None):
        capi.call("sntc_upsmall_plan_update", self._h, _ptr(weight), _ptr(bias), _stream())

    def out_hw(self, h, w):
        return h * self.stride, w * self.stride

    def flops(self, n, h, w):
        return int(capi.load().sntc_upsmall_flops(self._h, n, h, w))

    def __call__(self, x, res=None, aux=None):
        if res is not None or aux is not None:
            raise ValueError("the small-output transposed convolution has no epilogue operands")
        _check_nhwc(x, self.cin)
        n, h, w, _ = x.shape
        y = torch.empty((n, self.stride * h, self.stride * w, self.cout), dtype=torch.float32, device=x.device)
        prof = PROFILE
        if prof is not None:
            e0, e1 = torch.cuda.Event(enable_timing=True), torch.cuda.Event(enable_timing=True)
            e0.record()
        capi.call("sntc_upsmall_forward", self._h, _ptr(x), n, h, w, _ptr(y), _stream())
        if prof is not None:
            e1.record()
            prof.append(dict(e0=e0, e1=e1, flops=self.flops(n, h, w), variant=0, nblocks=0, vec=True, kind="upsmall", k=self.k, s=self.stride,
                             cin=self.cin, cout=self.cout, n=n, h=h, w=w))
        return y


def pad_reflect(x, hp, wp):
    _check_nhwc(x)
    n, h, w, c = x.shape
    if (hp, wp) == (h, w):
        return x
    y = torch.empty((n, hp, wp, c), dtype=torch.float32, device=x.device)
    capi.call("sntc_pad_reflect", _ptr(x), n, h, w, c, hp, wp, _ptr(y), _stream())
    return y


def concat_channels(a, b=None, extra=16):
    _check_nhwc(a)
    n, h, w, ca = a.shape
    if b is not None:
        _check_nhwc(b)
        if tuple(b.shape[:3]) != (n, h, w):
            raise ValueError(f"concat_channels: {tuple(a.shape)} vs {tuple(b.shape)}")
    cb = int(b.shape[-1]) if b is not None else int(extra)
    y = torch.empty((n, h, w, ca + cb), dtype=torch.float32, device=a.device)
    capi.call("sntc_concat_channels", _ptr(a), ca, _ptr(b), cb, n * h * w, _ptr(y), _stream())
    return y


def depth_to_space(x, block=2):
    _check_nhwc(x)
    n, h, w, c = x.shape
    if c % (block * block):
        raise ValueError(f"depth_to_space: {c} channels are not a multiple of {block * block}")
    y = torch.empty((n, h * block, w * block, c // (block * block)), dtype=torch.float32, device=x.device)
    capi.call("sntc_depth_to_space", _ptr(x), n, h, w, c, int(block), _ptr(y), _stream())
    return y


def crop(x, h, w):
    _check_nhwc(x)
    n, hp, wp, c = x.shape
    if (hp, wp) == (h, w):
        return x
    y = torch.empty((n, h, w, c), dtype=torch.float32, device=x.device)
    capi.call("sntc_crop", _ptr(x), n, hp, wp, c, h, w, _ptr(y), _stream())
    return y


def to_pixels(x_hat, h, w):
    _check_nhwc(x_hat)
    n, hs, ws, c = x_hat.shape
    px = torch.empty((n, h, w, c), dtype=torch.uint8, device=x_hat.device)
    capi.call("sntc_pixels_sse", _ptr(None), _ptr(x_hat), n, h, w, c, hs, ws, _ptr(px), _ptr(None), _stream())
    return px


def pixels_sse(x, x_hat, want_pixels=False):
    _check_nhwc(x)
    _check_nhwc(x_hat, x.shape[-1])
    n, h, w, c = x.shape
    hs, ws = x_hat.shape[1], x_hat.shape[2]
    sse = torch.empty((n,), dtype=torch.int64, device=x.device)
    px = torch.empty((n, h, w, c), dtype=torch.uint8, device=x.device) if want_pixels else None
    capi.call("sntc_pixels_sse", _ptr(x), _ptr(x_hat), n, h, w, c, hs, ws, _ptr(px), _ptr(sse), _stream())
    return sse, px


def block_sse(x, pixels, block):
    _check_nhwc(x)
    n, h, w, c = x.shape
    block = int(block)
    if not (isinstance(pixels, torch.Tensor) and pixels.dtype == torch.uint8 and tuple(pixels.shape) == (n, h, w, c)
            and pixels.is_contiguous() and pixels.device == x.device):
        raise ValueError(f"block_sse: pixels uint8 {(n, h, w, c)} on the images' device")
    if block < 1:
        raise ValueError("block_sse: block >= 1")
# ... 640 lines not shown
```

Measured before the change: 3955.

## Add in-register split-K execution for gather-GEMM conv to skip slab reduction

```diff
diff --git a/include/sntc.h b/include/sntc.h
--- a/include/sntc.h
+++ b/include/sntc.h
@@ -135,6 +135,8 @@
 int sntc_conv_status_inject(int flags, void* stream);
 int sntc_conv_set_stream_k(int enabled);
 int sntc_conv_get_stream_k(void);
+int sntc_conv_set_split_k_exec(int mode);
+int sntc_conv_get_split_k_exec(void);
 int sntc_conv_launch_info(const sntc_conv_plan* plan, int n, int h, int w, int* variant, int* nblocks);
 int sntc_conv_launch_order(const sntc_conv_plan* plan, int n, int h, int w, int* column_major);
 int64_t sntc_conv_tune_workspace_bytes(const sntc_conv_plan* plan, int n, int h, int w);
diff --git a/shallow-ntc_amd/_capi.py b/shallow-ntc_amd/_capi.py
--- a/shallow-ntc_amd/_capi.py
+++ b/shallow-ntc_amd/_capi.py
@@ -94,6 +94,8 @@
     "sntc_conv_status_inject": (C.c_int, [C.c_int, _P]),
     "sntc_conv_set_stream_k": (C.c_int, [C.c_int]),
     "sntc_conv_get_stream_k": (C.c_int, []),
+    "sntc_conv_set_split_k_exec": (C.c_int, [C.c_int]),
+    "sntc_conv_get_split_k_exec": (C.c_int, []),
     "sntc_conv_launch_info": (C.c_int, [_P, C.c_int, C.c_int, C.c_int, C.POINTER(C.c_int), C.POINTER(C.c_int)]),
     "sntc_conv_launch_order": (C.c_int, [_P, C.c_int, C.c_int, C.c_int, C.POINTER(C.c_int)]),
     "sntc_conv_tune_workspace_bytes": (C.c_int64, [_P, C.c_int, C.c_int, C.c_int]),
@@ -230,6 +232,8 @@
     _lib = lib
     if os.environ.get("SNTC_STATIC_SCHEDULES", "") not in ("", "0"):
         lib.sntc_conv_set_stream_k(0)
+    if os.environ.get("SNTC_SPLIT_K_EXEC", "") in ("0", "1", "2"):
+        lib.sntc_conv_set_split_k_exec(int(os.environ["SNTC_SPLIT_K_EXEC"]))
     return lib
 
 
diff --git a/shallow-ntc_amd/csrc/conv_plan.hip b/shallow-ntc_amd/csrc/conv_plan.hip
--- a/shallow-ntc_amd/csrc/conv_plan.hip
+++ b/shallow-ntc_amd/csrc/conv_plan.hip
@@ -500,6 +500,7 @@
 struct Sched {
   const GGInstance* inst = nullptr;
   int ksplit = 1;
+  bool inreg = false;
   bool sk = false;
   int workers = 0;
   int64_t units = 0;
@@ -552,12 +553,12 @@
   double padded_macs = 0;
 };
 
-static Work work_of(const sntc_conv_plan* p, const GGInstance& inst, int64_t M, int ncols) {
+static Work work_of(const sntc_conv_plan* p, const GGInstance& inst, int64_t M, int ncols, int ranges = 0) {
   Work wk;
   const int bm = inst.bm, bn = inst.bn;
   wk.ntm = (int)((M + bm - 1) / bm);
   for (int gi = 0; gi < p->ngroups; ++gi) {
-    const int steps = p->g[gi].K / kStage;
+    const int steps = ranges > 0 ? ranges : p->g[gi].K / kStage;
     wk.ntn[gi] = (launch_cols(p, gi, ncols) + bn - 1) / bn;
     wk.tile0[gi] = wk.tps;
     wk.unit0[gi] = wk.ups;
@@ -574,6 +575,8 @@
 constexpr double kDeepCost = 0.6;
 
 static std::atomic<int> g_stream_k_enabled{1};
+
+static std::atomic<int> g_split_k_exec{1};
 
 static Sched schedule_s3(const sntc_conv_plan* p, const Geo& g, int64_t n, const TuneChoice* force) {
   Sched best;
@@ -620,10 +623,11 @@
 
 static const GGInstance* column_major(const sntc_conv_plan* p, const Sched& sc, int ncols) {
   const GGInstance* strip = sc.inst;
-  if (!sc.sk || strip->load != kLoadVec || strip->stage != kStageRing || strip->form != kFormPlain || p->ngroups != 1 || p->colm == 0 ||
+  if (!sc.sk || strip->load != kLoadVec || strip->stage != kStageRing || (strip->form != kFormPlain && strip->form != kFormSplit) ||
+      p->ngroups != 1 || p->colm == 0 ||
       (p->colm != 1 && (size_t)launch_cols(p, 0, ncols) * p->g[0].K * sizeof(float) <= ((size_t)4 << 20)))
     return nullptr;
-  const GGInstance* twin = gg_find(strip->variant, kLoadVec, kStageRing, kFormColm);
+  const GGInstance* twin = gg_find(strip->variant, kLoadVec, kStageRing, strip->form == kFormSplit ? kFormSplitColm : kFormColm);
   return twin && gg_resident(*twin) >= gg_resident(*strip) ? twin : nullptr;
 }
 
@@ -646,23 +650,29 @@
     if (!ring) continue;
     const GGInstance* dma = !fused && plan_dma(p) ? gg_find(v, load, kStageDma, kFormPlain) : nullptr;
     const Work wk = work_of(p, *ring, M, ncols);
-    const int64_t tiles = wk.tiles, units = wk.units;
+    const int64_t tiles = wk.tiles;
     const double macs = wk.padded_macs;
     Sched s;
     s.inst = dma ? dma : ring;
+    const int exec = g_split_k_exec.load(std::memory_order_relaxed);
+    const GGInstance* split = ksplit > 1 && exec != 0 && load == kLoadVec && form == kFormPlain ? gg_find(v, load, kStageRing, kFormSplit) : nullptr;
+    if (split && exec != 2 && tiles < (int64_t)std::max(1, gg_resident(*split))) split = nullptr;
+    if (split) { s.inst = split; s.inreg = true; }
     const int resident = std::max(1, gg_resident(*s.inst));
     s.ksplit = ksplit;
+    const int64_t units = s.inreg ? tiles * ksplit : wk.units;
     s.units = units;
-    const int64_t fit = msteps > 0 ? units / msteps : 0;
+    const int64_t fit = s.inreg ? tiles : msteps > 0 ? units / msteps : 0;
     const int workers = (int)(std::min<int64_t>(resident, fit) & ~7LL);
-    const bool short_tiles = (units < 64 * tiles || tiles * ksplit >= 4 * (int64_t)resident) && !p->force_stream_k;
-    const bool can_sk = ksplit == 1 && g_stream_k_enabled.load(std::memory_order_relaxed) && units < (1LL << 31) && workers >= 8 &&
+    const int64_t bpt = s.inreg ? 1 : ksplit;
+    const bool short_tiles = (wk.units < 64 * tiles || tiles * bpt >= 4 * (int64_t)resident) && !p->force_stream_k;
+    const bool can_sk = (ksplit == 1 || s.inreg) && g_stream_k_enabled.load(std::memory_order_relaxed) && units < (1LL << 31) && workers >= 8 &&
                         2 * workers >= resident;
     s.sk = force ? (force->sk != 0 && can_sk) : (can_sk && !p->no_stream_k && !short_tiles);
     s.workers = s.sk ? workers : 0;
-    s.blocks = s.sk ? workers : tiles * ksplit;
+    s.blocks = s.sk ? workers : tiles * bpt;
     double cost = macs;
-    const bool deep_ok = !fused && !s.sk && p->dma != 0 && p->vec && !p->rowpack && !pro && !p->bf3 &&
+    const bool deep_ok = !fused && !s.sk && !s.inreg && p->dma != 0 && p->vec && !p->rowpack && !pro && !p->bf3 &&
                          tiles * ksplit <= (int64_t)kDeepBlocksPerCU * gg_num_cus();
     const GGInstance* deep = deep_ok ? gg_find(v, kLoadVec, kStageDeep, kFormPlain) : nullptr;
     if (deep) s.inst = deep;
@@ -671,9 +681,9 @@
     } else if (deep) {
       cost *= std::max(1.0, (double)gg_num_cus() / (double)(tiles * ksplit)) * kDeepCost;
     } else {
-      const double rounds = (double)(tiles * ksplit) / resident;
+      const double rounds = (double)(tiles * bpt) / resident;
       cost *= rounds < 1.0 ? 1.0 / rounds : std::ceil(rounds) / rounds;
-      if (tiles * ksplit < 768) cost *= 1.0 + 0.5 * (double)(768 - tiles * ksplit) / 768.0;
+      if (tiles * bpt < 768) cost *= 1.0 + 0.5 * (double)(768 - tiles * bpt) / 768.0;
     }
     static const double kRate[kNumVariants + 1] = {0, 0.86, 0.93, 1.00, 1.00, 0.97, 0.90, 0.85, 0.90, 1.02, 0.40};
     cost /= kRate[v];
@@ -709,7 +719,7 @@
 static int64_t workspace_floats(const sntc_conv_plan* p, int64_t M, const Sched& s, int ncols = 0) {
   if (s.sk)
     return (int64_t)s.workers * (int64_t)s.inst->slab_floats + s.workers;
-  if (s.ksplit <= 1) return 0;
+  if (s.ksplit <= 1 || s.inreg) return 0;
   int64_t cols = 0;
   for (int gi = 0; gi < p->ngroups; ++gi) cols += launch_cols(p, gi, ncols);
   return (int64_t)s.ksplit * M * cols;
@@ -731,7 +741,7 @@
   const Sched s = plan_schedule(p, g, n, h, w, false, ncols);
   if (variant) *variant = s.inst ? s.inst->variant : 0;
   if (nblocks) *nblocks = (int)s.blocks;
-  if (column_major_out) *column_major_out = s.inst && s.inst->form == kFormColm ? 1 : 0;
+  if (column_major_out) *column_major_out = s.inst && (s.inst->form == kFormColm || s.inst->form == kFormSplitColm) ? 1 : 0;
   return SNTC_OK;
 }
 
@@ -773,7 +783,7 @@
     return fail(SNTC_ERR_BAD_SHAPE, "sntc_conv_forward: this call needs sntc_conv_workspace_bytes() of workspace "
                                     "(split-K slabs / stream-K hand-off)");
   const GGInstance& inst = *sc.inst;
-  const Work wk = work_of(p, inst, M, ncols);
+  const Work wk = work_of(p, inst, M, ncols, sc.inreg ? sc.ksplit : 0);
   if (sc.sk && wk.units != sc.units) return fail(SNTC_ERR_HIP, "sntc_conv_forward: schedule and launch disagree about the work units");
   GGArgs a{};
   a.ksplit = sc.ksplit;
@@ -810,7 +820,7 @@
     G.blk0 = nb;
     G.tile0 = wk.tile0[gi];
     G.unit0 = wk.unit0[gi];
-    nb += G.ntn * a.ntm * sc.ksplit;
+    nb += G.ntn * a.ntm * (sc.inreg ? 1 : sc.ksplit);
     G.slab_off = slab_off;
     G.q0y = p->g[gi].q0y; G.q0x = p->g[gi].q0x;
     slab_off += (size_t)sc.ksplit * M * G.Ncol;
@@ -819,7 +829,7 @@
   a.ups = (int)wk.ups;
   if (p->s3) a.order = p->dma == 0 ? 0 : 1;
   rc = gg_launch(inst, a, sc.sk ? sc.workers : nb, (hipStream_t)stream);
-  if (rc || sc.sk || sc.ksplit <= 1) return rc;
+  if (rc || sc.sk || sc.ksplit <= 1 || sc.inreg) return rc;
   return gg_reduce_launch(a, (hipStream_t)stream);
 }
 
@@ -1037,6 +1047,14 @@
 
 extern "C" int sntc_conv_get_stream_k(void) { return g_stream_k_enabled.load(std::memory_order_relaxed); }
 
+extern "C" int sntc_conv_set_split_k_exec(int mode) {
+  if (mode < 0 || mode > 2) return fail(SNTC_ERR_BAD_SHAPE, "sntc_conv_set_split_k_exec: 0 slabs, 1 auto, 2 in registers where a twin exists");
+  g_split_k_exec.store(mode, std::memory_order_relaxed);
+  return SNTC_OK;
+}
+
+extern "C" int sntc_conv_get_split_k_exec(void) { return g_split_k_exec.load(std::memory_order_relaxed); }
+
 __global__ void status_exchange_kernel(int* word, int* out) { *out = atomicExch(word, 0); }
 __global__ void status_or_kernel(int* word, int flags) { atomicOr(word, flags); }
 
diff --git a/shallow-ntc_amd/csrc/gather_gemm.hip b/shallow-ntc_amd/csrc/gather_gemm.hip
--- a/shallow-ntc_amd/csrc/gather_gemm.hip
+++ b/shallow-ntc_amd/csrc/gather_gemm.hip
@@ -14,6 +14,9 @@
 extern template __global__ void gg_kernel<1, 3, 4, 1, true, false, false, false, 0, true>(const GGArgs);
 extern template __global__ void gg_kernel<2, 2, 2, 2, true, false, false, false, 0, false, true>(const GGArgs);
 extern template __global__ void gg_kernel<1, 2, 4, 1, true, false, true>(const GGArgs);
+#define SNTC_GG_DECL_SPLIT(TM, TN, WM, WN) extern template __global__ void gg_split_kernel<TM, TN, WM, WN>(const GGArgs);
+SNTC_GG_SPLIT_SHAPES(SNTC_GG_DECL_SPLIT)
+extern template __global__ void gg_split_kernel<2, 2, 2, 2, true>(const GGArgs);
 extern template __global__ void gg_kernel<1, 4, 4, 1, true, false, true>(const GGArgs);
 
 __global__ void __launch_bounds__(256) gg_reduce_kernel(const GGArgs a) {
@@ -68,6 +71,8 @@
   GG(v, kLoadVecPro, kStageRing, kFormPlain, TM, TN, WM, WN, true, true),    \
   GG(v, kLoadGather, kStageRing, kFormPlain, TM, TN, WM, WN, false, true)
 #define GG_DMA(v, TM, TN, WM, WN) GG(v, kLoadVec, kStageDma, kFormPlain, TM, TN, WM, WN, true, false, false, true)
+#define GG_SPLIT(v, TM, TN, WM, WN) \
+  row(v, kLoadVec, kStageRing, kFormSplit, TM, TN, WM, WN, reinterpret_cast<const void*>(&gg_split_kernel<TM, TN, WM, WN>))
 #define BF3P(v, TN, form) row(v, kLoadVec, kStageDma, form, 2, TN, 4, 2, bf3p_kernel(v, form == kFormPresplitHalo))
 
 static const GGInstance kInstances[] = {
@@ -78,6 +83,8 @@
     GG(8, kLoadVec, kStageDeep, kFormPlain, 1, 1, 2, 2, true, false, false, true, kDeepRing),
     GG(3, kLoadVec, kStageRing, kFormFuse2, 1, 3, 4, 1, true, false, false, false, 0, true),
     GG(9, kLoadVec, kStageRing, kFormColm, 2, 2, 2, 2, true, false, false, false, 0, false, true),
+    GG_SPLIT(1, 1, 1, 4, 1), GG_SPLIT(2, 1, 2, 4, 1), GG_SPLIT(4, 1, 4, 4, 1), GG_SPLIT(8, 1, 1, 2, 2), GG_SPLIT(9, 2, 2, 2, 2),
+    row(9, kLoadVec, kStageRing, kFormSplitColm, 2, 2, 2, 2, reinterpret_cast<const void*>(&gg_split_kernel<2, 2, 2, 2, true>)),
     GG(2, kLoadVec, kStageRing, kFormBf3, 1, 2, 4, 1, true, false, true),
     GG(4, kLoadVec, kStageRing, kFormBf3, 1, 4, 4, 1, true, false, true),
     BF3P(11, 4, kFormPresplit), BF3P(11, 4, kFormPresplitHalo), BF3P(12, 2, kFormPresplit), BF3P(12, 2, kFormPresplitHalo),
@@ -86,6 +93,7 @@
 #undef GG
 #undef GG_LOADERS
 #undef GG_DMA
+#undef GG_SPLIT
 #undef BF3P
 constexpr int kNumInstances = sizeof(kInstances) / sizeof(kInstances[0]);
 
@@ -165,7 +173,7 @@
   a.dma = inst.stage;
   a.bf3 = inst.form == kFormBf3 || presplit(inst) ? 1 : 0;
   a.halo = inst.form == kFormPresplitHalo ? 1 : 0;
-  if (!presplit(inst)) a.order = inst.form == kFormColm ? 0 : 1;
+  if (!presplit(inst)) a.order = inst.form == kFormColm || inst.form == kFormSplitColm ? 0 : 1;
 #ifdef SNTC_DIAG
   if (const char* e = getenv("SNTC_GG_DBG")) a.dbg = atoi(e);
 #endif
diff --git a/shallow-ntc_amd/csrc/gather_gemm_kernel.h b/shallow-ntc_amd/csrc/gather_gemm_kernel.h
--- a/shallow-ntc_amd/csrc/gather_gemm_kernel.h
+++ b/shallow-ntc_amd/csrc/gather_gemm_kernel.h
@@ -98,6 +98,8 @@
   int consume;
   int publish;
   int split;
+  int first;
+  int last;
 };
 
 constexpr int gg_waves(int tiles) { return tiles == 1 ? 4 : (tiles <= 3 ? 3 : 2); }
@@ -113,9 +115,9 @@
   *hi = h; *mid = m; *lo = (__bf16)r2;
 }
 
-template <int TM, int TN, int WM, int WN, bool VEC, bool PRO, bool BF3 = false, bool DMA = false, int DEEP = 0, bool FUSE2 = false,
-          bool COLM = false>
-__global__ void __launch_bounds__(256, FUSE2 ? 2 : gg_waves(TM * TN)) gg_kernel(const GGArgs a) {
+template <int TM, int TN, int WM, int WN, bool VEC, bool PRO, bool BF3, bool DMA, int DEEP, bool FUSE2, bool COLM, bool SPLITR>
+__device__ __forceinline__ void gg_body(const GGArgs& a) {
+  static_assert(!SPLITR || (VEC && !PRO && !BF3 && !DMA && !FUSE2), "in-register split-K: the register-staged fp32 vector instances");
   static_assert(!BF3 || (VEC && !PRO), "the bf16 x 3 experiment covers the vector path without prologue");
   static_assert(!DMA || (VEC && !PRO && !BF3), "direct-to-LDS staging: vector path, no prologue (nothing can touch the data on the way)");
   static_assert(!FUSE2 || (TM == 1 && TN == 3 && WM == 4 && WN == 1 && VEC && !PRO && !BF3 && !DMA),
@@ -156,7 +158,7 @@
     const int u_hi = (int)(a.units * (wl + 1) / a.nworkers);
     auto locate = [&](int u, int* t, int* k, int* steps) {
       if constexpr (COLM) {
-        const int st = a.g[0].steps;
+        const int st = SPLITR ? a.ksplit : a.g[0].steps;
         const int per = a.ntm * st;
         const int nt = u / per;
         const int r2 = u - nt * per;
@@ -172,10 +174,11 @@
         for (int i = 1; i < kMaxGroups; ++i)
           if (i < a.ngroups && r >= (int)a.g[i].unit0) gi = i;
         const int r2 = r - (int)a.g[gi].unit0;
-        const int nt = r2 / a.g[gi].steps;
+        const int st = SPLITR ? a.ksplit : a.g[gi].steps;
+        const int nt = r2 / st;
         *t = mt * a.tps + a.g[gi].tile0 + nt;
-        *k = r2 - nt * a.g[gi].steps;
-        *steps = a.g[gi].steps;
+        *k = r2 - nt * st;
+        *steps = st;
       }
     };
     if (u_hi > u_lo) {
@@ -211,21 +214,55 @@
     }
   };
 
+  Piece sp_tile{};
+  int sp_r = 0, sp_first = 0, sp_end = 0, sp_consume = -1, sp_publish = 0;
+  auto range_piece = [&](Piece* p) {
+    KArgs& a = fresh_args();
+    const int steps = a.g[sp_tile.gi].steps;
+    *p = sp_tile;
+    p->k0 = (int)(((long long)sp_r * steps) / a.ksplit);
+    p->k1 = (int)(((long long)(sp_r + 1) * steps) / a.ksplit);
+    p->first = sp_r == sp_first ? 1 : 0;
+    p->last = sp_r + 1 == sp_end ? 1 : 0;
+    p->consume = p->first ? sp_consume : -1;
+    p->publish = p->last ? sp_publish : 0;
+    p->split = sp_r;
+    ++sp_r;
+  };
+  auto open_tile = [&](int r0, int r1, int consume, int publish) {
+    sp_r = sp_first = r0; sp_end = r1; sp_consume = consume; sp_publish = publish;
+  };
+
   auto next_piece = [&](Piece* p) -> bool {
     KArgs& a = fresh_args();
+    if constexpr (SPLITR) {
+      if (sp_r < sp_end) { range_piece(p); return true; }
+    }
     if (!a.sk) return false;
     if (sk_phase == 0) {
       sk_phase = 1;
       if (sk_head_t >= 0) {
+        if constexpr (SPLITR) {
+          tile_of(sk_head_t, &sp_tile);
+          open_tile(0, sk_head_k1, -1, 1);
+          range_piece(p);
+          return true;
+        }
         tile_of(sk_head_t, p);
-        p->k0 = 0; p->k1 = sk_head_k1; p->consume = -1; p->publish = 1; p->split = 0;
+        p->k0 = 0; p->k1 = sk_head_k1; p->consume = -1; p->publish = 1; p->split = 0; p->first = 1; p->last = 1;
         return true;
       }
     }
     if (sk_phase == 1) {
       if (sk_cur <= sk_last) {
+        if constexpr (SPLITR) {
+          tile_of(sk_cur++, &sp_tile);
+          open_tile(0, a.ksplit, -1, 0);
+          range_piece(p);
+          return true;
+        }
         tile_of(sk_cur++, p);
-        p->k0 = 0; p->k1 = a.g[p->gi].steps; p->consume = -1; p->publish = 0; p->split = 0;
+        p->k0 = 0; p->k1 = a.g[p->gi].steps; p->consume = -1; p->publish = 0; p->split = 0; p->first = 1; p->last = 1;
         return true;
       }
       sk_phase = 2;
@@ -233,8 +270,14 @@
     if (sk_phase == 2) {
       sk_phase = 3;
       if (sk_tail_t >= 0) {
+        if constexpr (SPLITR) {
+          tile_of(sk_tail_t, &sp_tile);
+          open_tile(sk_tail_k0, a.ksplit, wl - 1, 0);
+          range_piece(p);
+          return true;
+        }
         tile_of(sk_tail_t, p);
-        p->k0 = sk_tail_k0; p->k1 = a.g[p->gi].steps; p->consume = wl - 1; p->publish = 0; p->split = 0;
+        p->k0 = sk_tail_k0; p->k1 = a.g[p->gi].steps; p->consume = wl - 1; p->publish = 0; p->split = 0; p->first = 1; p->last = 1;
         return true;
       }
     }
@@ -251,8 +294,9 @@
     for (int i = 1; i < kMaxGroups; ++i)
       if (i < a.ngroups && (int)blockIdx.x >= a.g[i].blk0) gi = i;
     const int lb0 = blockIdx.x - a.g[gi].blk0;
-    const int split = lb0 % a.ksplit;
-    const int lb = lb0 / a.ksplit;
+    const int bpt = SPLITR ? 1 : a.ksplit;
+    const int split = lb0 % bpt;
+    const int lb = lb0 / bpt;
     const int ntn = a.g[gi].ntn;
     const int full = a.ntm & ~7;
     if (lb < full * ntn) {
@@ -268,7 +312,12 @@
     P.gi = gi;
     P.k0 = (int)(((long long)split * steps) / a.ksplit);
     P.k1 = (int)(((long long)(split + 1) * steps) / a.ksplit);
-    P.consume = -1; P.publish = 0; P.split = split;
+    P.consume = -1; P.publish = 0; P.split = split; P.first = 1; P.last = 1;
+    if constexpr (SPLITR) {
+      sp_tile = P;
+      open_tile(0, a.ksplit, -1, 0);
+      range_piece(&P);
+    }
     have = true;
   }
   if (!have) return;
@@ -549,6 +598,7 @@
   };
 
   f32x16 acc[TM][TN];
+  f32x16 sum[TM][TN];
   auto mfma3 = [&](const Frag3& F) {
     constexpr int PA[6] = {2, 0, 1, 1, 0, 0};
     constexpr int PB[6] = {0, 2, 1, 0, 1, 0};
@@ -612,9 +662,18 @@
 #pragma unroll
           for (int q = 0; q < 4; ++q) {
             const f32x4 v = buf_load(sr, (unsigned)tid * 16u, (unsigned)((i * TN + j) * 4 + q) * 4096u);
-            acc[i][j][4 * q] = v[0]; acc[i][j][4 * q + 1] = v[1]; acc[i][j][4 * q + 2] = v[2]; acc[i][j][4 * q + 3] = v[3];
+            f32x16& d = SPLITR ? sum[i][j] : acc[i][j];
+            d[4 * q] = v[0]; d[4 * q + 1] = v[1]; d[4 * q + 2] = v[2]; d[4 * q + 3] = v[3];
           }
-    } else {
+    } else if (!SPLITR || P.first) {
+#pragma unroll
+      for (int i = 0; i < TM; ++i)
+#pragma unroll
+        for (int j = 0; j < TN; ++j)
+#pragma unroll
+          for (int e = 0; e < 16; ++e) (SPLITR ? sum[i][j] : acc[i][j])[e] = 0.0f;
+    }
+    if constexpr (SPLITR) {
 #pragma unroll
       for (int i = 0; i < TM; ++i)
 #pragma unroll
@@ -757,7 +816,17 @@
     const int wm = wave / WN, wn = wave % WN;
     KArgs& a = fresh_args();
     const auto& Gd = a.g[P.gi];
-    if (P.publish) {
+    if constexpr (SPLITR) {
+#pragma unroll
+      for (int i = 0; i < TM; ++i)
+#pragma unroll
+        for (int j = 0; j < TN; ++j) {
+          sum[i][j] = sum[i][j] + acc[i][j];
+          acc[i][j] = sum[i][j];
+        }
+    }
+    if (SPLITR && !P.last) {
+    } else if (P.publish) {
       const __amdgpu_buffer_rsrc_t sr = __builtin_amdgcn_make_buffer_rsrc(
           a.sk_slab + (size_t)wl * (TM * TN * 16 * 256), 0, TM * TN * 16 * 256 * 4, 0x00020000);
 #pragma unroll
@@ -776,7 +845,7 @@
         asm volatile("s_waitcnt vmcnt(0)" ::: "memory");
         __hip_atomic_store(a.sk_flags + wl, 1, __ATOMIC_RELAXED, __HIP_MEMORY_SCOPE_AGENT);
       }
-    } else if (a.ksplit > 1) {
+    } else if (!SPLITR && a.ksplit > 1) {
       float* slab = a.slab + Gd.slab_off + (size_t)P.split * a.M * Gd.Ncol;
 #pragma unroll
       for (int j = 0; j < TN; ++j) {
@@ -931,8 +1000,20 @@
   }
 }
 
+template <int TM, int TN, int WM, int WN, bool VEC, bool PRO, bool BF3 = false, bool DMA = false, int DEEP = 0, bool FUSE2 = false,
+          bool COLM = false>
+__global__ void __launch_bounds__(256, FUSE2 ? 2 : gg_waves(TM * TN)) gg_kernel(const GGArgs a) {
+  gg_body<TM, TN, WM, WN, VEC, PRO, BF3, DMA, DEEP, FUSE2, COLM, false>(a);
+}
+
+template <int TM, int TN, int WM, int WN, bool COLM = false>
+__global__ void __launch_bounds__(256, gg_waves(TM * TN)) gg_split_kernel(const GGArgs a) {
+  gg_body<TM, TN, WM, WN, true, false, false, false, 0, false, COLM, true>(a);
+}
+
 #define SNTC_GG_SHAPES(X) X(1, 1, 4, 1) X(1, 2, 4, 1) X(1, 3, 4, 1) X(1, 4, 4, 1) X(1, 5, 4, 1) X(1, 6, 4, 1) X(1, 7, 4, 1) X(1, 1, 2, 2) X(2, 2, 2, 2) X(2, 4, 4, 1)
 #define SNTC_GG_DMA_SHAPES(X) X(1, 1, 4, 1) X(1, 2, 4, 1) X(1, 3, 4, 1) X(1, 4, 4, 1) X(1, 5, 4, 1) X(1, 1, 2, 2) X(2, 2, 2, 2)
+#define SNTC_GG_SPLIT_SHAPES(X) X(1, 1, 4, 1) X(1, 2, 4, 1) X(1, 4, 4, 1) X(1, 1, 2, 2) X(2, 2, 2, 2)
 constexpr int kDeepRing = 8;
 
 }
diff --git a/shallow-ntc_amd/csrc/gg_inst_split.hip b/shallow-ntc_amd/csrc/gg_inst_split.hip
--- /dev/null
+++ b/shallow-ntc_amd/csrc/gg_inst_split.hip
@@ -0,0 +1,9 @@
+#include "gather_gemm_kernel.h"
+
+namespace sntc {
+
+#define SPLIT_INST(TM, TN, WM, WN) template __global__ void gg_split_kernel<TM, TN, WM, WN>(const GGArgs);
+SNTC_GG_SPLIT_SHAPES(SPLIT_INST)
+template __global__ void gg_split_kernel<2, 2, 2, 2, true>(const GGArgs);
+
+}
diff --git a/shallow-ntc_amd/csrc/sntc_internal.h b/shallow-ntc_amd/csrc/sntc_internal.h
--- a/shallow-ntc_amd/csrc/sntc_internal.h
+++ b/shallow-ntc_amd/csrc/sntc_internal.h
@@ -82,7 +82,7 @@
 
 enum GGLoad { kLoadVec, kLoadVecPro, kLoadGather };
 enum GGStage { kStageRing, kStageDma, kStageDeep };
-enum GGForm { kFormPlain, kFormFuse2, kFormColm, kFormBf3, kFormPresplit, kFormPresplitHalo };
+enum GGForm { kFormPlain, kFormFuse2, kFormColm, kFormBf3, kFormPresplit, kFormPresplitHalo, kFormSplit, kFormSplitColm };
 struct GGInstance {
   int variant;
   GGLoad load;
diff --git a/shallow-ntc_amd/ops.py b/shallow-ntc_amd/ops.py
--- a/shallow-ntc_amd/ops.py
+++ b/shallow-ntc_amd/ops.py
@@ -731,6 +731,14 @@
     return bool(capi.load().sntc_conv_get_stream_k())
 
 
+def set_split_k_exec(mode):
+    capi.call("sntc_conv_set_split_k_exec", int(mode))
+
+
+def split_k_exec():
+    return int(capi.load().sntc_conv_get_split_k_exec())
+
+
 class static_schedules:
 
     def __init__(self, active=True):
```

Result: no change. 3951, median of 2 (-0.1%).
